# BradMcDanel/term-quantization

Measured on NVIDIA B200. Metric: resnet18_tq_g8_a12_images_per_sec, higher is better.
Workload: dtype int term codes (TR encode) -> exact int32 accumulators on tcgen05 (kind::f16 with statically proven fp32 K-chunk accumulators summed in int32, or kind::i8 planes with s32 accumulators)

## Files before the change

include/tq_b200.h:

```cpp
#ifndef TQ_B200_H
#define TQ_B200_H

#include <stdint.h>

#ifdef __cplusplus
extern "C" {
#endif

#define TQ_VERSION 201

#define TQ_OK               0
#define TQ_ERR_INVALID      1
#define TQ_ERR_UNSUPPORTED  2
#define TQ_ERR_CUDA         3

#define TQ_F32   0
#define TQ_F64   1
#define TQ_BF16  2
#define TQ_F16   3

#define TQ_I8    0
#define TQ_I16   1
#define TQ_I32   2
#define TQ_U8    3
#define TQ_F16C  4

#define TQ_ENC_HESE    0
#define TQ_ENC_BINARY  1
#define TQ_ENC_BOOTH   2

#define TQ_FLAG_RELU       1u
#define TQ_FLAG_RECIP_DIV  2u

#define TQ_FLAG_EXACT_DIV  4u

#define TQ_MAX_GROUP   32
#define TQ_MAX_BITS    16

int         tq_version(void);
const char *tq_last_error(void);
uint64_t    tq_launch_count(void);

int tq_tr_encode(const void *in, void *out, int dtype,
                 int64_t B, int64_t C, int64_t WH,
                 float sf, int bits, int g, int alpha,
                 int encoding, unsigned flags, void *stream);

int tq_tr_encode_codes(const void *in, void *codes, int dtype, int code_dtype,
                       int64_t B, int64_t C, int64_t WH,
                       float sf, int bits, int g, int alpha,
                       int encoding, unsigned flags, int *overflow, void *stream);

int tq_hist_accumulate(const void *x, int dtype, int64_t n,
                       float *hist, uint32_t *counts_scratch ,
                       int nbins, float lo, float hi, void *stream);

int tq_mse_profile(const float *hist, const float *x, int nbins,
                   const float *sfs, int nsf, int bits, int terms,
                   double *errs, int *argmin, void *stream);

int tq_hese_term_count(const void *w, int dtype, int64_t n, float sf, unsigned flags,
                       unsigned long long *count, void *stream);

int tq_conv2d_codes_f16(const void *act, const void *wgt, const float *bias, float *out,
                        int N, int H, int W, int C, int Cout, int R, int S, int stride, int pad,
                        float scale, int acc_groups, void *stream);

int tq_conv2d_codes_fused(const void *act, const void *wgt, float *out_f32, void *out_codes,
                          const float *bias, const float *bn_a, const float *bn_b, const float *residual,
                          int N, int H, int W, int C, int Cout, int R, int S, int stride, int pad,
                          float scale, int relu, float next_sf, int next_bits, int next_terms,
                          int acc_groups, void *stream);

int tq_conv2d_planes_i8(const void *act_planes, const void *wgt_planes, int planes_a, int planes_w,
                        float *out_f32, void *out_codes, const float *bias, const float *bn_a,
                        const float *bn_b, const float *residual, int N, int H, int W, int C, int Cout,
                        int R, int S, int stride, int pad, float scale, int relu, float next_sf,
                        int next_bits, int next_terms, int act_max, int wgt_max, void *stream);

int tq_codes_to_planes(const void *codes_f16, void *planes_s8, int64_t n, int planes, int *overflow, void *stream);

int tq_conv_weight_l1(const void *wgt_f16, int RS, int Cout, int C, long long *pos, long long *neg, void *stream);

int tq_bn_relu_maxpool_encode(const float *x, const float *bn_a, const float *bn_b, float *out,
                              void *out_codes, int N, int H, int W, int C, int relu,
                              float next_sf, int next_bits, int next_terms, void *stream);

int tq_stem_conv7x7s2(const float *x, void *x2_scratch, const void *w2, float *out,
                      int N, int H, int W, int Cout, void *stream);
int tq_stem_conv7x7s2_dt(const void *x, int x_dtype, void *x2_scratch, const void *w2, float *out,
                         int N, int H, int W, int Cout, void *stream);

int tq_stem_conv7x7s2_u8(const void *x_u8, const float *mean3, const float *std3, void *x2_scratch, const void *w2,
                         float *out, int N, int H, int W, int Cout, void *stream);
int tq_stem_conv7x7s2_pool(const void *x, int x_dtype, void *x2_scratch, const void *w2,
                           const float *bn_a, const float *bn_b, int relu, float *out, void *out_codes,
                           int N, int H, int W, int Cout, float next_sf, int next_bits, int next_terms,
                           void *stream);

int tq_depthwise3x3_codes(const void *act_codes, const int32_t *wgt_codes, float *out_f32, void *out_codes,
                          const float *bias, const float *bn_a, const float *bn_b, int N, int H, int W, int C,
                          int stride, float scale, int relu, int act_unsigned, float next_sf, int next_bits,
                          int next_terms, void *stream);

int tq_bn_act_encode(const float *x, const float *bias, const float *bn_a, const float *bn_b, float *out_f32,
                     void *out_codes, int64_t npix, int C, int relu, float next_sf, int next_bits, int next_terms,
                     void *stream);

int tq_first_conv3x3_fused(const float *x, const float *wgt, const float *bias, const float *bn_a, const float *bn_b,
                           float *out_f32, void *out_codes, int N, int H, int W, int Cout, int stride, int relu,
                           float next_sf, int next_bits, int next_terms, void *stream);

int tq_maxpool2d_f16(const void *x_f16, void *y_f16, int N, int H, int W, int C, int k, int stride, int pad,
                     void *stream);

int tq_u8_normalize_bf16(const void *x_u8, void *y_bf16, int64_t npix, const float *mean3, const float *std3,
                         void *stream);

int tq_selftest_division(uint64_t n, uint32_t seed, unsigned long long *mismatch, void *stream);

#ifdef __cplusplus
}
#endif
#endif
```

term_quantization_b200/_lib.py:

```python
import ctypes as C
import os

_HERE = os.path.dirname(os.path.abspath(__file__))
LIB_PATH = os.environ.get("TQ_B200_LIB") or os.path.join(_HERE, "libtq_b200.so")

TQ_OK, TQ_ERR_INVALID, TQ_ERR_UNSUPPORTED, TQ_ERR_CUDA = 0, 1, 2, 3
TQ_F32, TQ_F64, TQ_BF16, TQ_F16 = 0, 1, 2, 3
TQ_I8, TQ_I16, TQ_I32, TQ_U8, TQ_F16C = 0, 1, 2, 3, 4
ENC_HESE, ENC_BINARY, ENC_BOOTH = 0, 1, 2
FLAG_RELU, FLAG_RECIP_DIV, FLAG_EXACT_DIV = 1, 2, 4

_i64, _i, _f, _p, _u = C.c_int64, C.c_int, C.c_float, C.c_void_p, C.c_uint
SYMBOLS = {
    "tq_version": (_i, []),
    "tq_last_error": (C.c_char_p, []),
    "tq_launch_count": (C.c_uint64, []),
    "tq_tr_encode": (_i, [_p, _p, _i, _i64, _i64, _i64, _f, _i, _i, _i, _i, _u, _p]),
    "tq_tr_encode_codes": (_i, [_p, _p, _i, _i, _i64, _i64, _i64, _f, _i, _i, _i, _i, _u, _p, _p]),
    "tq_hist_accumulate": (_i, [_p, _i, _i64, _p, _p, _i, _f, _f, _p]),
    "tq_mse_profile": (_i, [_p, _p, _i, _p, _i, _i, _i, _p, _p, _p]),
    "tq_hese_term_count": (_i, [_p, _i, _i64, _f, _u, _p, _p]),
    "tq_conv2d_codes_f16": (_i, [_p, _p, _p, _p] + [_i] * 9 + [_f, _i, _p]),
    "tq_conv2d_codes_fused": (_i, [_p] * 8 + [_i] * 9 + [_f, _i, _f, _i, _i, _i, _p]),
    "tq_conv2d_planes_i8": (_i, [_p, _p, _i, _i] + [_p] * 6 + [_i] * 9 + [_f, _i, _f, _i, _i, _i, _i, _p]),
    "tq_codes_to_planes": (_i, [_p, _p, _i64, _i, _p, _p]),
    "tq_conv_weight_l1": (_i, [_p, _i, _i, _i, _p, _p, _p]),
    "tq_depthwise3x3_codes": (_i, [_p] * 7 + [_i] * 5 + [_f, _i, _i, _f, _i, _i, _p]),
    "tq_bn_act_encode": (_i, [_p] * 6 + [_i64, _i, _i, _f, _i, _i, _p]),
    "tq_maxpool2d_f16": (_i, [_p, _p, _i, _i, _i, _i, _i, _i, _i, _p]),
    "tq_first_conv3x3_fused": (_i, [_p] * 7 + [_i, _i, _i, _i, _i, _i, _f, _i, _i, _p]),
    "tq_u8_normalize_bf16": (_i, [_p, _p, _i64, _p, _p, _p]),
    "tq_bn_relu_maxpool_encode": (_i, [_p] * 5 + [_i] * 5 + [_f, _i, _i, _p]),
    "tq_stem_conv7x7s2": (_i, [_p, _p, _p, _p, _i, _i, _i, _i, _p]),
    "tq_stem_conv7x7s2_dt": (_i, [_p, _i, _p, _p, _p, _i, _i, _i, _i, _p]),
    "tq_stem_conv7x7s2_u8": (_i, [_p, _p, _p, _p, _p, _p, _i, _i, _i, _i, _p]),
    "tq_stem_conv7x7s2_pool": (_i, [_p, _i, _p, _p, _p, _p, _i, _p, _p, _i, _i, _i, _i, _f, _i, _i, _p]),
    "tq_selftest_division": (_i, [C.c_uint64, C.c_uint32, _p, _p]),
}

_lib = None


class TQError(RuntimeError):
    pass


def build(verbose=False):
    import subprocess
    subprocess.run(["make", "-C", os.path.join(_HERE, "csrc"), "-j4", "--no-print-directory"],
                   check=True, stdout=None if verbose else subprocess.DEVNULL)


def lib():
    global _lib
    if _lib is None:
        if not os.path.exists(LIB_PATH):
            raise TQError(
                f"{LIB_PATH} is missing: build it with `python -c 'import __graft_entry__ as g; "
                "g.build()'` or `make -C term_quantization_b200/csrc`. There is no CPU fallback.")
        L = C.CDLL(LIB_PATH)
        for name, (res, args) in SYMBOLS.items():
            fn = getattr(L, name)
            fn.restype = res
            fn.argtypes = args
        _lib = L
    return _lib


def check(rc):
    if rc != TQ_OK:
        msg = lib().tq_last_error().decode("utf-8", "replace")
        if rc == TQ_ERR_INVALID:
            raise ValueError(f"tq_b200: {msg}")
        if rc == TQ_ERR_UNSUPPORTED:
            raise NotImplementedError(f"tq_b200: {msg}")
        raise TQError(f"tq_b200: {msg}")


def launch_count():
    return int(lib().tq_launch_count())
```

term_quantization_b200/conv_codes.py:

```python
import torch

from . import _lib
from . import tr_cuda


def pack_conv_weight(w, w_sf, weight_bits, group_size, num_terms):
    codes = tr_cuda.tr_codes(w.detach().contiguous(), w_sf, weight_bits, group_size, num_terms,
                             dtype=torch.int16)
    O, I, kh, kw = codes.shape
    return codes.permute(2, 3, 0, 1).reshape(kh * kw, O, I).to(torch.float16).contiguous()



EXACT_LIMIT = 1 << 24


def _relu_code(relu):
    if relu in ("relu6", 2):
        return 2
    return 1 if relu else 0


class WeightPlan:

    def __init__(self, engine, groups, bound, act_max, signed, wgt, planes=None, planes_w=0, wgt_max=0):
        self.engine, self.groups, self.bound, self.act_max, self.signed = engine, groups, bound, act_max, signed
        self.wgt, self.planes, self.planes_w, self.wgt_max = wgt, planes, planes_w, wgt_max

    def __repr__(self):
        return (f"WeightPlan({self.engine}, groups={self.groups}, bound={self.bound:.3e}, act_max={self.act_max}, "
                f"signed={self.signed}, planes_w={self.planes_w})")


def weight_l1(wgt):
    RS, Cout, C = wgt.shape
    kcb = (C + 63) // 64
    pos = torch.empty((Cout, kcb), dtype=torch.int64, device=wgt.device)
    neg = torch.empty_like(pos)
    with torch.cuda.device(wgt.device):
        rc = _lib.lib().tq_conv_weight_l1(wgt.data_ptr(), RS, Cout, C, pos.data_ptr(), neg.data_ptr(),
                                          torch.cuda.current_stream(wgt.device).cuda_stream)
    _lib.check(rc)
    return pos, neg


def codes_to_planes(codes, planes):
    if codes.dtype != torch.float16 or not codes.is_contiguous() or not codes.is_cuda:
        raise RuntimeError("codes_to_planes expects a contiguous fp16 CUDA tensor")
    out = torch.empty((planes,) + tuple(codes.shape), dtype=torch.int8, device=codes.device)
    ovf = torch.zeros(1, dtype=torch.int32, device=codes.device)
    with torch.cuda.device(codes.device):
        rc = _lib.lib().tq_codes_to_planes(codes.data_ptr(), out.data_ptr(), codes.numel(), planes, ovf.data_ptr(),
                                           torch.cuda.current_stream(codes.device).cuda_stream)
    _lib.check(rc)
    return out, ovf


def _planes_needed(max_abs_code):
    if max_abs_code <= 127:
        return 1
    if max_abs_code <= 2047:
        return 2
    raise NotImplementedError(f"codes up to {max_abs_code} do not fit two signed 8-bit planes")


def plan_weight(wgt, act_max, signed_act=False, engine="auto"):
    if wgt.dtype != torch.float16 or wgt.dim() != 3 or not wgt.is_contiguous():
        raise RuntimeError("plan_weight expects a contiguous fp16 [R*S, Cout, C] code tensor")
    RS, Cout, C = wgt.shape
    bound = float("inf")
    if engine in ("auto", "f16"):
        pos, neg = weight_l1(wgt)
        kcb = pos.shape[1]
        block_n = 64 if Cout <= 64 else 128
        for groups in (1, 2, 4, 8):
            if kcb % groups or groups * block_n > (512 if block_n == 128 else 256):
                continue
            p = pos.view(Cout, groups, kcb // groups).sum(2)
            n = neg.view(Cout, groups, kcb // groups).sum(2)
            worst = (p + n) if signed_act else torch.maximum(p, n)
            b = float(act_max) * float(worst.max().item())
            bound = min(bound, b)
            if b < EXACT_LIMIT:
                return WeightPlan("f16", groups, b, act_max, signed_act, wgt)
        if engine == "f16":
            raise NotImplementedError(
                f"kind::f16 conv: cannot prove exact fp32 accumulation for this weight (best bound {bound:.3e} >= 2^24 "
                f"with act_max = {act_max}); use the kind::i8 plane engine (engine='i8' / 'auto')")
    if C % 16:
        raise NotImplementedError("kind::i8 plane engine needs C % 16 == 0")
    wmax = int(wgt.abs().max().item())
    pw = _planes_needed(wmax)
    planes, ovf = codes_to_planes(wgt, pw)
    if int(ovf.item()):
        raise RuntimeError("weight codes do not fit their planes")
    return WeightPlan("i8", 1, bound, act_max, signed_act, wgt, planes=planes, planes_w=pw, wgt_max=max(wmax, 1))


_PLANS = {}


def _cached_plan(wgt, act_max, signed_act, engine):
    key = (wgt.data_ptr(), wgt._version, tuple(wgt.shape), int(act_max), bool(signed_act), engine)
    plan = _PLANS.get(key)
    if plan is None or plan.wgt is not wgt:
        if len(_PLANS) > 256:
            _PLANS.clear()
        plan = _PLANS[key] = plan_weight(wgt, act_max, signed_act, engine)
    return plan


def _run_conv(act, plan, out, codes, bias, bn, residual, N, H, W, C, Cout, R, S, stride, pad, scale, relu, sf, bits,
              terms, act_planes=None):
    ptr = lambda t: t.data_ptr() if t is not None else None
    L = _lib.lib()
    stream = torch.cuda.current_stream(act.device).cuda_stream
    with torch.cuda.device(act.device):
        if plan.engine == "f16":
            rc = L.tq_conv2d_codes_fused(
                act.data_ptr(), plan.wgt.data_ptr(), ptr(out), ptr(codes), ptr(bias),
                ptr(bn[0]) if bn else None, ptr(bn[1]) if bn else None, ptr(residual),
                N, H, W, C, Cout, R, S, stride, pad, float(scale), _relu_code(relu), float(sf), int(bits),
                int(terms), int(plan.groups), stream)
        else:
            if act_planes is None:
                pa = _planes_needed(plan.act_max)
                act_planes, _ = codes_to_planes(act, pa)
            rc = L.tq_conv2d_planes_i8(
                act_planes.data_ptr(), plan.planes.data_ptr(), act_planes.shape[0], plan.planes_w, ptr(out), ptr(codes),
                ptr(bias), ptr(bn[0]) if bn else None, ptr(bn[1]) if bn else None, ptr(residual),
                N, H, W, C, Cout, R, S, stride, pad, float(scale), _relu_code(relu), float(sf), int(bits), int(terms),
                int(plan.act_max), int(plan.wgt_max), stream)
    _lib.check(rc)


def conv2d_codes(act, wgt, bias, kernel_size, stride, pad, scale, out=None, *, act_max=512, signed_act=False,
                 engine="auto", plan=None):
    if not (act.is_cuda and wgt.is_cuda and act.dtype == torch.float16 and wgt.dtype == torch.float16):
        raise RuntimeError("conv2d_codes expects fp16 CUDA code tensors")
    if not (act.is_contiguous() and wgt.is_contiguous()):
        raise RuntimeError("conv2d_codes expects contiguous NHWC activations and packed weights")
    N, H, W, C = act.shape
    R, S = kernel_size
    RS, Cout, C2 = wgt.shape
    if RS != R * S or C2 != C:
        raise RuntimeError("weight / activation shape mismatch")
    Ho = (H + 2 * pad - R) // stride + 1
    Wo = (W + 2 * pad - S) // stride + 1
    if out is None:
        out = torch.empty((N, Ho, Wo, Cout), dtype=torch.float32, device=act.device)
    if plan is None:
        plan = _cached_plan(wgt, act_max, signed_act, engine)
    _run_conv(act, plan, out, None, bias, None, None, N, H, W, C, Cout, R, S, stride, pad, scale, False, 1.0, 1, 0)
    return out


def conv2d_codes_fused(act, wgt, kernel_size, stride, pad, scale, *, bias=None, bn=None, residual=None,
                       relu=False, want_f32=True, next_quant=None, act_max=512, signed_act=False, engine="auto",
                       plan=None):
    N, H, W, C = act.shape
    R, S = kernel_size
    RS, Cout, C2 = wgt.shape
    if act.dtype != torch.float16 or wgt.dtype != torch.float16 or RS != R * S or C2 != C:
        raise RuntimeError("conv2d_codes_fused: bad operands")
    Ho = (H + 2 * pad - R) // stride + 1
    Wo = (W + 2 * pad - S) // stride + 1
    out = torch.empty((N, Ho, Wo, Cout), dtype=torch.float32, device=act.device) if want_f32 else None
    codes = torch.empty((N, Ho, Wo, Cout), dtype=torch.float16, device=act.device) if next_quant else None
    if residual is not None and (residual.shape != (N, Ho, Wo, Cout) or not residual.is_contiguous()
                                 or residual.dtype != torch.float32):
        raise RuntimeError("residual must be a contiguous fp32 [N, Ho, Wo, Cout] tensor")
    sf, bits, terms = next_quant if next_quant else (1.0, 1, 0)
    if plan is None:
        plan = _cached_plan(wgt, act_max, signed_act, engine)
    _run_conv(act, plan, out, codes, bias, bn, residual, N, H, W, C, Cout, R, S, stride, pad, scale, relu, sf, bits, terms)
    return out, codes


def pack_linear_weight(w, w_sf):
    sf32 = torch.tensor(w_sf, dtype=torch.float32).item()
    codes = torch.round(w.detach() / sf32)
    if not torch.equal(codes * sf32, w.detach()):
        raise RuntimeError("weight is not an integer multiple of w_sf any more")
    O, I = codes.shape
    Op, Ip = (O + 3) // 4 * 4, (I + 15) // 16 * 16
    packed = torch.zeros((1, Op, Ip), dtype=torch.float16, device=w.device)
    packed[0, :O, :I] = codes.to(torch.float16)
    return packed, sf32


def linear_codes(x_codes, wgt, scale, *, bias=None, out_features=None, plan=None, act_max=512, signed_act=True,
                 engine="auto"):
    if x_codes.dtype != torch.float16 or x_codes.dim() != 2:
        raise RuntimeError("linear_codes expects fp16 [M, K] codes")
    M, K = x_codes.shape
    _, Op, Kp = wgt.shape
    if K > Kp:
        raise RuntimeError("weight / activation shape mismatch")
    if K != Kp:
        xp = torch.zeros((M, Kp), dtype=torch.float16, device=x_codes.device)
        xp[:, :K] = x_codes
        x_codes = xp
    bias_p = bias
    if bias is not None and bias.numel() != Op:
        bias_p = torch.zeros(Op, dtype=torch.float32, device=wgt.device)
        bias_p[:bias.numel()] = bias.detach().float()
    out = conv2d_codes(x_codes.contiguous().view(1, 1, M, Kp), wgt, bias_p, (1, 1), 1, 0, scale, plan=plan, act_max=act_max,
                       signed_act=signed_act, engine=engine).view(M, Op)
    n = out_features if out_features is not None else Op
    return out if n == Op else out[:, :n]


def pack_depthwise_weight(w, w_sf):
    if w.dim() != 4 or w.shape[1] != 1 or tuple(w.shape[2:]) != (3, 3):
        raise NotImplementedError("depthwise packing expects a (C, 1, 3, 3) weight")
    sf32 = torch.tensor(w_sf, dtype=torch.float32).item()
    codes = torch.round(w.detach() / sf32)
    if not torch.equal(codes * sf32, w.detach()):
        raise RuntimeError("depthwise weight is not an integer multiple of w_sf any more")
    return codes.view(w.shape[0], 9).t().contiguous().to(torch.int32), sf32


def depthwise3x3_codes(act, wgt, stride, scale, *, bias=None, bn=None, relu=False, want_f32=False, next_quant=None,
                       act_unsigned=False):
    if act.dtype != torch.float16 or not act.is_contiguous() or wgt.dtype != torch.int32 or not wgt.is_contiguous():
        raise RuntimeError("depthwise3x3_codes expects contiguous fp16 NHWC codes and int32 [9, C] weights")
    N, H, W, C = act.shape
    if tuple(wgt.shape) != (9, C):
        raise RuntimeError("weight / activation shape mismatch")
    Ho, Wo = (H - 1) // stride + 1, (W - 1) // stride + 1
    out = torch.empty((N, Ho, Wo, C), dtype=torch.float32, device=act.device) if want_f32 else None
    codes = torch.empty((N, Ho, Wo, C), dtype=torch.float16, device=act.device) if next_quant else None
    sf, bits, terms = next_quant if next_quant else (1.0, 1, 0)
    ptr = lambda t: t.data_ptr() if t is not None else None
    with torch.cuda.device(act.device):
        rc = _lib.lib().tq_depthwise3x3_codes(
            act.data_ptr(), wgt.data_ptr(), ptr(out), ptr(codes), ptr(bias), ptr(bn[0]) if bn else None,
            ptr(bn[1]) if bn else None, N, H, W, C, stride, float(scale), _relu_code(relu), int(bool(act_unsigned)),
            float(sf), int(bits), int(terms), torch.cuda.current_stream(act.device).cuda_stream)
    _lib.check(rc)
    return out, codes


def pack_first_conv_weight(w_oihw):
    if w_oihw.dim() != 4 or w_oihw.shape[1:] != (3, 3, 3):
        raise RuntimeError("pack_first_conv_weight expects a (Cout, 3, 3, 3) weight")
    return w_oihw.detach().float().permute(2, 3, 1, 0).contiguous()


def first_conv3x3_fused(x_nhwc, w_packed, stride=1, bias=None, bn=None, relu=False, want_f32=False, next_quant=None):
    if x_nhwc.dtype != torch.float32 or not x_nhwc.is_contiguous() or not x_nhwc.is_cuda or x_nhwc.shape[-1] != 3:
        raise RuntimeError("first_conv3x3_fused expects a contiguous fp32 CUDA [N, H, W, 3] tensor")
    N, H, W, _ = x_nhwc.shape
    Cout = w_packed.shape[-1]
    Ho, Wo = (H - 1) // stride + 1, (W - 1) // stride + 1
    out = torch.empty((N, Ho, Wo, Cout), dtype=torch.float32, device=x_nhwc.device) if want_f32 else None
    codes = torch.empty((N, Ho, Wo, Cout), dtype=torch.float16, device=x_nhwc.device) if next_quant else None
    if out is None and codes is None:
        raise RuntimeError("first_conv3x3_fused: nothing to compute (want_f32 or next_quant)")
    sf, bits, terms = next_quant if next_quant else (1.0, 1, 0)
    ptr = lambda t: t.data_ptr() if t is not None else None
    for t in (bias, bn[0] if bn else None, bn[1] if bn else None):
        if t is not None and (t.dtype != torch.float32 or t.numel() != Cout or not t.is_contiguous() or t.device != x_nhwc.device):
            raise RuntimeError("first_conv3x3_fused: bias / bn must be contiguous fp32 [Cout] tensors on the input's device")
    with torch.cuda.device(x_nhwc.device):
        rc = _lib.lib().tq_first_conv3x3_fused(
            x_nhwc.data_ptr(), w_packed.data_ptr(), ptr(bias), ptr(bn[0]) if bn else None, ptr(bn[1]) if bn else None,
            ptr(out), ptr(codes), N, H, W, Cout, int(stride), _relu_code(relu), float(sf), int(bits), int(terms),
            torch.cuda.current_stream(x_nhwc.device).cuda_stream)
    _lib.check(rc)
    return out, codes


def maxpool_codes(codes_nhwc, kernel_size, stride=None, padding=0):
    k = kernel_size if isinstance(kernel_size, int) else kernel_size[0]
    st = k if stride is None else (stride if isinstance(stride, int) else stride[0])
    pd = padding if isinstance(padding, int) else padding[0]
    if codes_nhwc.dtype != torch.float16 or not codes_nhwc.is_contiguous() or not codes_nhwc.is_cuda:
        raise RuntimeError("maxpool_codes expects a contiguous fp16 CUDA [N, H, W, C] tensor")
    N, H, W, C = codes_nhwc.shape
    Ho, Wo = (H + 2 * pd - k) // st + 1, (W + 2 * pd - k) // st + 1
    out = torch.empty((N, Ho, Wo, C), dtype=torch.float16, device=codes_nhwc.device)
    with torch.cuda.device(codes_nhwc.device):
        rc = _lib.lib().tq_maxpool2d_f16(codes_nhwc.data_ptr(), out.data_ptr(), N, H, W, C, k, st, pd,
                                         torch.cuda.current_stream(codes_nhwc.device).cuda_stream)
    _lib.check(rc)
    return out


def bn_act_encode(x_nhwc, bn=None, relu=False, want_f32=False, next_quant=None, bias=None):
    if x_nhwc.dtype != torch.float32 or not x_nhwc.is_contiguous() or not x_nhwc.is_cuda:
        raise RuntimeError("bn_act_encode expects a contiguous fp32 CUDA tensor with channels last")
    C = x_nhwc.shape[-1]
    out = torch.empty_like(x_nhwc) if want_f32 else None
    codes = torch.empty(x_nhwc.shape, dtype=torch.float16, device=x_nhwc.device) if next_quant else None
    sf, bits, terms = next_quant if next_quant else (1.0, 1, 0)
    ptr = lambda t: t.data_ptr() if t is not None else None
    with torch.cuda.device(x_nhwc.device):
        if bias is not None and (bias.dtype != torch.float32 or bias.numel() != C or not bias.is_contiguous() or bias.device != x_nhwc.device):
            raise RuntimeError("bn_act_encode: bias must be a contiguous fp32 [C] tensor on the input's device")
        rc = _lib.lib().tq_bn_act_encode(
            x_nhwc.data_ptr(), ptr(bias), ptr(bn[0]) if bn else None, ptr(bn[1]) if bn else None, ptr(out), ptr(codes),
            x_nhwc.numel() // C, C, _relu_code(relu), float(sf), int(bits), int(terms),
            torch.cuda.current_stream(x_nhwc.device).cuda_stream)
    _lib.check(rc)
    return out, codes


def bn_relu_maxpool_encode(x_nhwc, bn, relu=True, next_quant=None):
    if x_nhwc.dtype != torch.float32 or not x_nhwc.is_contiguous() or not x_nhwc.is_cuda:
        raise RuntimeError("bn_relu_maxpool_encode expects a contiguous fp32 CUDA [N, H, W, C] tensor")
    N, H, W, C = x_nhwc.shape
    Ho, Wo = (H - 1) // 2 + 1, (W - 1) // 2 + 1
    out = torch.empty((N, Ho, Wo, C), dtype=torch.float32, device=x_nhwc.device)
    codes = torch.empty((N, Ho, Wo, C), dtype=torch.float16, device=x_nhwc.device) if next_quant else None
    sf, bits, terms = next_quant if next_quant else (1.0, 1, 0)
    with torch.cuda.device(x_nhwc.device):
        rc = _lib.lib().tq_bn_relu_maxpool_encode(
            x_nhwc.data_ptr(), bn[0].data_ptr(), bn[1].data_ptr(), out.data_ptr(),
            codes.data_ptr() if codes is not None else None, N, H, W, C, int(bool(relu)),
            float(sf), int(bits), int(terms), torch.cuda.current_stream(x_nhwc.device).cuda_stream)
    _lib.check(rc)
    return out, codes


def pack_stem_weight(w, channel_sign=None):
    Cout, Cin, kh, kw = w.shape
    if (Cin, kh, kw) != (3, 7, 7) or Cout > 64:
        raise NotImplementedError("stem conv packing expects a (Cout <= 64, 3, 7, 7) weight")
    w8 = torch.zeros(Cout, 4, 8, 8, dtype=torch.float32, device=w.device)
    w8[:, :3, :7, :7] = w.detach().float()
    if channel_sign is not None:
        w8 = w8 * channel_sign.view(-1, 1, 1, 1).to(w8)
    w2 = w8.view(Cout, 4, 4, 2, 4, 2).permute(2, 0, 4, 3, 5, 1).reshape(4, Cout, 64)
    hi = w2.half()
    lo = (w2 - hi.float()).half()
    out = torch.zeros(4, 128, 64, dtype=torch.float16, device=w.device)
    out[:, :Cout] = hi
    out[:, 64:64 + Cout] = lo
    return out.contiguous()


_STEM_DTYPES = {torch.float32: _lib.TQ_F32, torch.bfloat16: _lib.TQ_BF16, torch.float16: _lib.TQ_F16}


def stem_conv7x7s2(x_nhwc, w2, scratch=None, cout=None):
    if x_nhwc.dtype not in _STEM_DTYPES or not x_nhwc.is_contiguous() or x_nhwc.shape[-1] != 3:
        raise RuntimeError("stem_conv7x7s2 expects a contiguous fp32 / bf16 / fp16 [N, H, W, 3] tensor")
    N, H, W, _ = x_nhwc.shape
    Cout = cout if cout is not None else 64
    need = (2 if x_nhwc.dtype == torch.float32 else 1) * N * (H // 2 + 3) * (W // 2 + 3) * 16
    if scratch is None or scratch.numel() < need:
        scratch = torch.empty(need, dtype=torch.float16, device=x_nhwc.device)
    out = torch.empty((N, H // 2, W // 2, Cout), dtype=torch.float32, device=x_nhwc.device)
    with torch.cuda.device(x_nhwc.device):
        rc = _lib.lib().tq_stem_conv7x7s2_dt(x_nhwc.data_ptr(), _STEM_DTYPES[x_nhwc.dtype], scratch.data_ptr(),
                                             w2.data_ptr(), out.data_ptr(), N, H, W, Cout,
                                             torch.cuda.current_stream(x_nhwc.device).cuda_stream)
    _lib.check(rc)
    return out, scratch


def stem_conv7x7s2_u8(x_u8_nhwc, mean, std, w2, scratch=None, cout=None):
    import ctypes
    if x_u8_nhwc.dtype != torch.uint8 or not x_u8_nhwc.is_contiguous() or not x_u8_nhwc.is_cuda or x_u8_nhwc.shape[-1] != 3:
        raise RuntimeError("stem_conv7x7s2_u8 expects a contiguous uint8 CUDA [N, H, W, 3] tensor")
    N, H, W, _ = x_u8_nhwc.shape
    Cout = cout if cout is not None else 64
    need = N * (H // 2 + 3) * (W // 2 + 3) * 16
    if scratch is None or scratch.numel() < need:
        scratch = torch.empty(need, dtype=torch.float16, device=x_u8_nhwc.device)
    out = torch.empty((N, H // 2, W // 2, Cout), dtype=torch.float32, device=x_u8_nhwc.device)
    m = (ctypes.c_float * 3)(*mean)
    s = (ctypes.c_float * 3)(*std)
    with torch.cuda.device(x_u8_nhwc.device):
        rc = _lib.lib().tq_stem_conv7x7s2_u8(x_u8_nhwc.data_ptr(), ctypes.cast(m, ctypes.c_void_p), ctypes.cast(s, ctypes.c_void_p),
                                             scratch.data_ptr(), w2.data_ptr(), out.data_ptr(), N, H, W, Cout,
                                             torch.cuda.current_stream(x_u8_nhwc.device).cuda_stream)
    _lib.check(rc)
    return out, scratch


def stem_pool_operands(w, bn):
    a, b = bn
    sign = torch.where(a < 0, -torch.ones_like(a), torch.ones_like(a))
    return pack_stem_weight(w, sign), (a.abs().contiguous(), b.contiguous())


def stem_conv_pool(x_nhwc, w2, bn, relu=True, next_quant=None, scratch=None):
    if x_nhwc.dtype not in _STEM_DTYPES or not x_nhwc.is_contiguous() or x_nhwc.shape[-1] != 3:
        raise RuntimeError("stem_conv_pool expects a contiguous fp32 / bf16 / fp16 [N, H, W, 3] tensor")
    N, H, W, _ = x_nhwc.shape
    Cout = bn[0].numel()
    need = (2 if x_nhwc.dtype == torch.float32 else 1) * N * (H // 2 + 3) * (W // 2 + 3) * 16
    if scratch is None or scratch.numel() < need:
        scratch = torch.empty(need, dtype=torch.float16, device=x_nhwc.device)
    Hp, Wp = (H // 2 - 1) // 2 + 1, (W // 2 - 1) // 2 + 1
    out = torch.empty((N, Hp, Wp, Cout), dtype=torch.float32, device=x_nhwc.device)
    codes = torch.empty((N, Hp, Wp, Cout), dtype=torch.float16, device=x_nhwc.device) if next_quant else None
    sf, bits, terms = next_quant if next_quant else (1.0, 1, 0)
    with torch.cuda.device(x_nhwc.device):
        rc = _lib.lib().tq_stem_conv7x7s2_pool(
            x_nhwc.data_ptr(), _STEM_DTYPES[x_nhwc.dtype], scratch.data_ptr(), w2.data_ptr(),
            bn[0].data_ptr(), bn[1].data_ptr(), int(bool(relu)), out.data_ptr(),
            codes.data_ptr() if codes is not None else None, N, H, W, Cout, float(sf), int(bits), int(terms),
            torch.cuda.current_stream(x_nhwc.device).cuda_stream)
    _lib.check(rc)
    return out, codes, scratch
```

term_quantization_b200/csrc/tq_gemm.cu:

```cuda
#ifdef TQ_CONV_TRACE
#include <cstdio>
#endif
#include <cuda.h>

#include <cstdlib>
#include <cstring>
#include <mutex>
#include <type_traits>
#include <vector>

#include "tq_common.cuh"

namespace tq {

constexpr int GM_BLOCK_M = 128;
constexpr int GM_ROW_BYTES = 128;
constexpr int GM_BLOCK_K = 64;
constexpr int GM_THREADS = 640;
constexpr int GM_A_BYTES = GM_BLOCK_M * GM_ROW_BYTES;
constexpr int GM_I8_SHIFT = 4;

struct ConvGeom {
    int N, H, W, C, Cout, R, S, stride, pad, Ho, Wo;
    int wbox, hbox, nbox;
    int hw;
    int step_w, step_h, off_w, off_h;
    int pool, pool_p, pool_q;
    int halo, halo_baseoff;
    int img_h1;
    int pair;
    int tiles_w, tiles_h, tiles_n;
    int m_tiles, n_tiles, kc_blocks;
    int a_tx_bytes;
    float scale;
    int a_stages, a_stage_bytes;
    int stages, stage_bytes, ring_off, bstat_off, epi_off, epi_group_bytes, epi_codes_off, lut_off, bar_off, smem_total;
    int prog_steps, nb_tiles, n_groups;
    int kcpg, acc_int, planes_a, planes_w, kblk;
    int b_rows;
    int dbg_skip_epilogue;
    int dbg_skip_mma, dbg_skip_tma;
    uint32_t prog_mma[16];
    const float *bias, *bn_a, *bn_b, *residual;
    int relu, relu6, write_f32, write_codes;
    float next_sf;
    int next_bits, next_terms, next_fastdiv;
};

__device__ __forceinline__ uint32_t smem_u32(const void *p) { return (uint32_t)__cvta_generic_to_shared(p); }

__device__ __forceinline__ void mbar_init(uint64_t *bar, uint32_t count)
{
    asm volatile("mbarrier.init.shared::cta.b64 [%0], %1;" ::"r"(smem_u32(bar)), "r"(count));
}
__device__ __forceinline__ void mbar_expect_tx(uint64_t *bar, uint32_t bytes)
{
    asm volatile("mbarrier.arrive.expect_tx.shared::cta.b64 _, [%0], %1;" ::"r"(smem_u32(bar)), "r"(bytes) : "memory");
}
__device__ __forceinline__ void mbar_arrive(uint64_t *bar)
{
    asm volatile("mbarrier.arrive.shared::cta.b64 _, [%0];" ::"r"(smem_u32(bar)) : "memory");
}
__device__ __forceinline__ void mbar_wait(uint64_t *bar, uint32_t parity)
{
    asm volatile(
        "{\n\t"
        ".reg .pred P1;\n\t"
        "WAIT_LOOP:\n\t"
        "mbarrier.try_wait.parity.shared::cta.b64 P1, [%0], %1;\n\t"
        "@P1 bra DONE;\n\t"
        "bra WAIT_LOOP;\n\t"
        "DONE:\n\t"
        "}" ::"r"(smem_u32(bar)), "r"(parity) : "memory");
}
__device__ __forceinline__ void tma_load_4d(const CUtensorMap *map, uint64_t *bar, void *dst, int c0, int c1, int c2, int c3)
{
    asm volatile(
        "cp.async.bulk.tensor.4d.shared::cluster.global.mbarrier::complete_tx::bytes [%0], [%1, {%3, %4, %5, %6}], [%2];"
        ::"r"(smem_u32(dst)), "l"(map), "r"(smem_u32(bar)), "r"(c0), "r"(c1), "r"(c2), "r"(c3) : "memory");
}
__device__ __forceinline__ void tma_load_3d(const CUtensorMap *map, uint64_t *bar, void *dst, int c0, int c1, int c2)
{
    asm volatile(
        "cp.async.bulk.tensor.3d.shared::cluster.global.mbarrier::complete_tx::bytes [%0], [%1, {%3, %4, %5}], [%2];"
        ::"r"(smem_u32(dst)), "l"(map), "r"(smem_u32(bar)), "r"(c0), "r"(c1), "r"(c2) : "memory");
}
__device__ __forceinline__ bool elect_one()
{
    uint32_t pred = 0;
    asm volatile(
        "{\n\t"
        ".reg .pred P;\n\t"
        "elect.sync _|P, 0xFFFFFFFF;\n\t"
        "selp.u32 %0, 1, 0, P;\n\t"
        "}" : "=r"(pred));
    return pred != 0;
}
__device__ __forceinline__ void tc_fence_before() { asm volatile("tcgen05.fence::before_thread_sync;" ::: "memory"); }
__device__ __forceinline__ void tc_fence_after() { asm volatile("tcgen05.fence::after_thread_sync;" ::: "memory"); }
__device__ __forceinline__ void umma_f16(uint32_t tmem_d, uint64_t desc_a, uint64_t desc_b, uint32_t idesc, uint32_t accumulate)
{
    asm volatile(
        "{\n\t"
        ".reg .pred p;\n\t"
        "setp.ne.b32 p, %4, 0;\n\t"
        "tcgen05.mma.cta_group::1.kind::f16 [%0], %1, %2, %3, p;\n\t"
        "}" ::"r"(tmem_d), "l"(desc_a), "l"(desc_b), "r"(idesc), "r"(accumulate) : "memory");
}
__device__ __forceinline__ void umma_i8(uint32_t tmem_d, uint64_t desc_a, uint64_t desc_b, uint32_t idesc, uint32_t accumulate)
{
    asm volatile(
        "{\n\t"
        ".reg .pred p;\n\t"
        "setp.ne.b32 p, %4, 0;\n\t"
        "tcgen05.mma.cta_group::1.kind::i8 [%0], %1, %2, %3, p;\n\t"
        "}" ::"r"(tmem_d), "l"(desc_a), "l"(desc_b), "r"(idesc), "r"(accumulate) : "memory");
}
template <int KIND>
__device__ __forceinline__ void umma(uint32_t tmem_d, uint64_t desc_a, uint64_t desc_b, uint32_t idesc, uint32_t accumulate)
{
    if constexpr (KIND == 1) umma_i8(tmem_d, desc_a, desc_b, idesc, accumulate);
    else umma_f16(tmem_d, desc_a, desc_b, idesc, accumulate);
}
__device__ __forceinline__ uint32_t cluster_ctarank()
{
    uint32_t r;
    asm volatile("mov.u32 %0, %%cluster_ctarank;" : "=r"(r));
    return r;
}
__device__ __forceinline__ void cluster_sync_all()
{
    asm volatile("barrier.cluster.arrive.release.aligned;\n\tbarrier.cluster.wait.acquire.aligned;" ::: "memory");
}
__device__ __forceinline__ uint32_t mapa_u32(uint32_t addr, uint32_t rank)
{
    uint32_t r;
    asm volatile("mapa.shared::cluster.u32 %0, %1, %2;" : "=r"(r) : "r"(addr), "r"(rank));
    return r;
}
__device__ __forceinline__ void mbar_arrive_cluster(uint32_t cluster_addr)
{
    asm volatile("mbarrier.arrive.shared::cluster.b64 _, [%0];" ::"r"(cluster_addr) : "memory");
}
__device__ __forceinline__ void tma_load_4d_pair(const CUtensorMap *map, uint32_t bar_cluster, void *dst, int c0, int c1, int c2, int c3)
{
    asm volatile(
        "cp.async.bulk.tensor.4d.cta_group::2.shared::cluster.global.mbarrier::complete_tx::bytes [%0], [%1, {%3, %4, %5, %6}], [%2];"
        ::"r"(smem_u32(dst)), "l"(map), "r"(bar_cluster), "r"(c0), "r"(c1), "r"(c2), "r"(c3) : "memory");
}
__device__ __forceinline__ void tma_load_3d_pair(const CUtensorMap *map, uint32_t bar_cluster, void *dst, int c0, int c1, int c2)
{
    asm volatile(
        "cp.async.bulk.tensor.3d.cta_group::2.shared::cluster.global.mbarrier::complete_tx::bytes [%0], [%1, {%3, %4, %5}], [%2];"
        ::"r"(smem_u32(dst)), "l"(map), "r"(bar_cluster), "r"(c0), "r"(c1), "r"(c2) : "memory");
}
__device__ __forceinline__ void umma_f16_pair(uint32_t tmem_d, uint64_t desc_a, uint64_t desc_b, uint32_t idesc, uint32_t accumulate)
{
    asm volatile(
        "{\n\t"
        ".reg .pred p;\n\t"
        "setp.ne.b32 p, %4, 0;\n\t"
        "tcgen05.mma.cta_group::2.kind::f16 [%0], %1, %2, %3, p;\n\t"
        "}" ::"r"(tmem_d), "l"(desc_a), "l"(desc_b), "r"(idesc), "r"(accumulate) : "memory");
}
__device__ __forceinline__ void umma_commit_pair(uint64_t *bar)
{
    asm volatile("tcgen05.commit.cta_group::2.mbarrier::arrive::one.shared::cluster.multicast::cluster.b64 [%0], %1;"
                 ::"r"(smem_u32(bar)), "h"((uint16_t)3) : "memory");
}
__device__ __forceinline__ void umma_commit(uint64_t *bar)
{
    asm volatile("tcgen05.commit.cta_group::1.mbarrier::arrive::one.shared::cluster.b64 [%0];" ::"r"(smem_u32(bar)) : "memory");
}
#ifdef TQ_CONV_TRACE
#define TR_DECL(n) long long trc[n] = {}
#define TR(slot, ...) do { const long long _t = clock64(); __VA_ARGS__; trc[slot] += clock64() - _t; } while (0)
#define TR_T0(name) const long long name = clock64()
#define TR_SINCE(slot, name) trc[slot] += clock64() - name
#else
#define TR_DECL(n)
#define TR(slot, ...) do { __VA_ARGS__; } while (0)
#define TR_T0(name)
#define TR_SINCE(slot, name)
#endif

__device__ __forceinline__ void tmem_ld_32x32b_x32(uint32_t taddr, uint32_t (&r)[32])
{
    asm volatile(
        "tcgen05.ld.sync.aligned.32x32b.x32.b32 "
        "{%0, %1, %2, %3, %4, %5, %6, %7, %8, %9, %10, %11, %12, %13, %14, %15, "
        "%16, %17, %18, %19, %20, %21, %22, %23, %24, %25, %26, %27, %28, %29, %30, %31}, [%32];"
        : "=r"(r[0]), "=r"(r[1]), "=r"(r[2]), "=r"(r[3]), "=r"(r[4]), "=r"(r[5]), "=r"(r[6]), "=r"(r[7]),
          "=r"(r[8]), "=r"(r[9]), "=r"(r[10]), "=r"(r[11]), "=r"(r[12]), "=r"(r[13]), "=r"(r[14]), "=r"(r[15]),
          "=r"(r[16]), "=r"(r[17]), "=r"(r[18]), "=r"(r[19]), "=r"(r[20]), "=r"(r[21]), "=r"(r[22]), "=r"(r[23]),
          "=r"(r[24]), "=r"(r[25]), "=r"(r[26]), "=r"(r[27]), "=r"(r[28]), "=r"(r[29]), "=r"(r[30]), "=r"(r[31])
        : "r"(taddr));
    asm volatile("tcgen05.wait::ld.sync.aligned;" ::: "memory");
}

__device__ __forceinline__ void tmem_ld_32x32b_x16(uint32_t taddr, uint32_t (&r)[16])
{
    asm volatile(
        "tcgen05.ld.sync.aligned.32x32b.x16.b32 "
        "{%0, %1, %2, %3, %4, %5, %6, %7, %8, %9, %10, %11, %12, %13, %14, %15}, [%16];"
        : "=r"(r[0]), "=r"(r[1]), "=r"(r[2]), "=r"(r[3]), "=r"(r[4]), "=r"(r[5]), "=r"(r[6]), "=r"(r[7]),
          "=r"(r[8]), "=r"(r[9]), "=r"(r[10]), "=r"(r[11]), "=r"(r[12]), "=r"(r[13]), "=r"(r[14]), "=r"(r[15])
        : "r"(taddr));
    asm volatile("tcgen05.wait::ld.sync.aligned;" ::: "memory");
}

__device__ __forceinline__ void tma_store_4d(const CUtensorMap *map, const void *src, int c0, int c1, int c2, int c3)
{
    asm volatile("cp.async.bulk.tensor.4d.global.shared::cta.bulk_group [%0, {%2, %3, %4, %5}], [%1];"
                 ::"l"(map), "r"(smem_u32(src)), "r"(c0), "r"(c1), "r"(c2), "r"(c3) : "memory");
}
__device__ __forceinline__ void bulk_commit() { asm volatile("cp.async.bulk.commit_group;" ::: "memory"); }
__device__ __forceinline__ void bulk_wait_read0() { asm volatile("cp.async.bulk.wait_group.read 0;" ::: "memory"); }
__device__ __forceinline__ void bulk_wait0() { asm volatile("cp.async.bulk.wait_group 0;" ::: "memory"); }
__device__ __forceinline__ void fence_proxy_async() { asm volatile("fence.proxy.async.shared::cta;" ::: "memory"); }
__device__ __forceinline__ void epi_bar_sync(int id) { asm volatile("bar.sync %0, 128;" ::"r"(id) : "memory"); }
__device__ __forceinline__ void cp_async16(void *dst, const void *src)
{
    asm volatile("cp.async.ca.shared.global [%0], [%1], 16;" ::"r"(smem_u32(dst)), "l"(src) : "memory");
}
__device__ __forceinline__ void cp_async_wait_all() { asm volatile("cp.async.wait_all;" ::: "memory"); }

__device__ __forceinline__ uint64_t smem_desc_sw128(uint32_t saddr)
{
    return (uint64_t)((saddr & 0x3FFFFu) >> 4) | (1ull << 16) | ((uint64_t)(1024 >> 4) << 32) | (1ull << 46) | (2ull << 61);
}

constexpr int GM_LUT_MAX_BITS = 10;
constexpr int GM_MAX_STAGES = 8;
constexpr int GM_EPI_GROUPS = 4;
constexpr int GM_EPI_F32_BYTES = 16384;
constexpr int GM_EPI_CODE_BYTES = 8192;
constexpr int GM_SMEM_BUDGET = 227 * 1024;

template <bool FULL>
__device__ __forceinline__ void epi_affine(float (&t)[32], const ConvGeom &g, int c0)
{
    if (g.bias) {
        const float4 *bp = reinterpret_cast<const float4 *>(g.bias + c0);
#pragma unroll
        for (int j = 0; j < 32; j += 4) {
            if (FULL || c0 + j < g.Cout) {
                const float4 b = __ldg(bp + (j >> 2));
                t[j] = __fadd_rn(t[j], b.x); t[j + 1] = __fadd_rn(t[j + 1], b.y);
                t[j + 2] = __fadd_rn(t[j + 2], b.z); t[j + 3] = __fadd_rn(t[j + 3], b.w);
            }
        }
    }
    if (g.bn_a) {
        const float4 *ap = reinterpret_cast<const float4 *>(g.bn_a + c0);
        const float4 *bp = reinterpret_cast<const float4 *>(g.bn_b + c0);
#pragma unroll
        for (int j = 0; j < 32; j += 4) {
            if (FULL || c0 + j < g.Cout) {
                const float4 a = __ldg(ap + (j >> 2));
                const float4 b = __ldg(bp + (j >> 2));
                t[j] = __fmaf_rn(t[j], a.x, b.x); t[j + 1] = __fmaf_rn(t[j + 1], a.y, b.y);
                t[j + 2] = __fmaf_rn(t[j + 2], a.z, b.z); t[j + 3] = __fmaf_rn(t[j + 3], a.w, b.w);
            }
        }
    }
}

__device__ __forceinline__ uint32_t lds_u16(uint32_t saddr)
{
    uint16_t v;
    asm("ld.shared.u16 %0, [%1];" : "=h"(v) : "r"(saddr));
    return v;
}

template <bool RELU>
__device__ __forceinline__ void epi_stage(float (&t)[32], const ConvGeom &g, uint8_t *st_f32, uint8_t *st_codes, int row,
                                          bool has_res, const __half *lut, const Quant &nq)
{
    const uint32_t sw128 = (uint32_t)(row & 7);
    const uint32_t sw64 = (uint32_t)((row >> 1) & 3);
    uint8_t *frow = st_f32 + row * 128, *crow = st_codes + row * 64;
    if (has_res) {
#pragma unroll
        for (int j = 0; j < 32; j += 4) {
            const float4 r = *reinterpret_cast<const float4 *>(frow + (((uint32_t)(j >> 2) ^ sw128) << 4));
            t[j] = __fadd_rn(t[j], r.x); t[j + 1] = __fadd_rn(t[j + 1], r.y);
            t[j + 2] = __fadd_rn(t[j + 2], r.z); t[j + 3] = __fadd_rn(t[j + 3], r.w);
        }
    }
    if (RELU) {
#pragma unroll
        for (int j = 0; j < 32; ++j) t[j] = fmaxf(t[j], 0.0f);
        if (g.relu6) {
#pragma unroll
            for (int j = 0; j < 32; ++j) t[j] = fminf(t[j], 6.0f);
        }
    }
    if (g.write_f32) {
#pragma unroll
        for (int j = 0; j < 32; j += 4)
            *reinterpret_cast<float4 *>(frow + (((uint32_t)(j >> 2) ^ sw128) << 4)) = make_float4(t[j], t[j + 1], t[j + 2], t[j + 3]);
    }
    if (g.write_codes) {
        const uint32_t lut_s = smem_u32(lut) - 2u * 0x4B000000u;
        const uint32_t sign_off = 2u << g.next_bits;
#pragma unroll
        for (int j = 0; j < 32; j += 8) {
            uint32_t hc[8];
#pragma unroll
            for (int e = 0; e < 8; ++e) {
                const float x = t[j + e];
                float r;
                if (RELU) r = div_rn_nonneg<true>(x, nq);
                else r = div_rn_nonneg<true>(fmaxf(fabsf(x), 0.0f), nq);
                r = fminf(r, nq.maxv);
                float q = __fadd_rd(r, 0.5f);
                q = __fadd_rd(q, 8388608.0f);
                uint32_t addr = __float_as_uint(q) * 2u + lut_s;
                if (!RELU) addr += (__float_as_uint(x) >> 31) * sign_off;
                hc[e] = lds_u16(addr);
            }
            *reinterpret_cast<uint4 *>(crow + (((uint32_t)(j >> 3) ^ sw64) << 4)) =
                make_uint4(hc[0] | (hc[1] << 16), hc[2] | (hc[3] << 16), hc[4] | (hc[5] << 16), hc[6] | (hc[7] << 16));
        }
    }
}

template <int BLOCK_N, int MODE, bool RELU, int KIND, int CG = 1>
__global__ void __launch_bounds__(GM_THREADS, 1)
conv_igemm_kernel(const __grid_constant__ CUtensorMap tmA, const __grid_constant__ CUtensorMap tmB,
                      const __grid_constant__ CUtensorMap tmC, const __grid_constant__ CUtensorMap tmD,
                      const __grid_constant__ CUtensorMap tmR, const __grid_constant__ ConvGeom g)
{
    static_assert(KIND == 0 || MODE == 0, "the s8-plane engine streams both operands (MODE 0)");
    static_assert(CG == 1 || ((MODE == 4 || MODE == 3) && KIND == 0), "the CTA pair runs the halo modes");
    constexpr int MMA_N = MODE == 2 ? 2 * BLOCK_N : BLOCK_N;
    constexpr int B_BYTES = MMA_N * GM_ROW_BYTES;
    const int STAGES = g.stages;
    extern __shared__ uint8_t smem_raw[];
    uint8_t *smem = reinterpret_cast<uint8_t *>((reinterpret_cast<uintptr_t>(smem_raw) + 1023) & ~uintptr_t(1023));
    uint8_t *ring = smem + g.ring_off;
    uint8_t *bstat = smem + g.bstat_off;
    uint64_t *full_bar = reinterpret_cast<uint64_t *>(smem + g.bar_off);
    uint64_t *empty_bar = full_bar + GM_MAX_STAGES;
    uint64_t *tfull_bar = empty_bar + GM_MAX_STAGES;
    uint64_t *tempty_bar = tfull_bar + 3;
    uint64_t *bfull_bar = tempty_bar + 3;
    uint64_t *res_bar = bfull_bar + 1;
    uint64_t *afull_bar = res_bar + GM_EPI_GROUPS;
    uint64_t *aempty_bar = afull_bar + 4;
    uint32_t *tmem_slot = reinterpret_cast<uint32_t *>(aempty_bar + 4);
    constexpr bool prog = MODE >= 1 && MODE <= 3;
    const int acc_cols = g.n_groups * BLOCK_N;

    const int warp = threadIdx.x >> 5, lane = threadIdx.x & 31;
    const uint32_t cta_rank = CG == 2 ? cluster_ctarank() : 0u;
    const int tile_first = CG == 2 ? (int)(blockIdx.x >> 1) : (int)blockIdx.x;
    const int tile_step = CG == 2 ? (int)(gridDim.x >> 1) : (int)gridDim.x;
    const int total_tiles = CG == 2 ? ((g.m_tiles + 1) / 2) * g.n_tiles : g.m_tiles * g.n_tiles;
    auto m_tile_of = [&](int tile) { return CG == 2 ? 2 * (tile / g.n_tiles) + (int)cta_rank : tile / g.n_tiles; };
    const int kblocks = g.R * g.S * g.kc_blocks * (KIND == 1 ? g.planes_a * g.planes_w : 1);
    const int ACC_STAGES = 3 * acc_cols <= 512 ? 3 : (2 * acc_cols <= 512 ? 2 : 1);
    uint32_t TMEM_COLS = 32;
    while (TMEM_COLS < (uint32_t)(ACC_STAGES * acc_cols)) TMEM_COLS <<= 1;

    if (warp == 0 && lane == 0) {
        asm volatile("prefetch.tensormap [%0];" ::"l"(&tmA) : "memory");
        asm volatile("prefetch.tensormap [%0];" ::"l"(&tmB) : "memory");
        if (g.write_f32) asm volatile("prefetch.tensormap [%0];" ::"l"(&tmC) : "memory");
        if (g.write_codes) asm volatile("prefetch.tensormap [%0];" ::"l"(&tmD) : "memory");
        if (g.residual) asm volatile("prefetch.tensormap [%0];" ::"l"(&tmR) : "memory");
    }
    __half *lut = reinterpret_cast<__half *>(smem + g.lut_off);
    if (g.write_codes) {
        for (uint32_t i = threadIdx.x; i < (2u << g.next_bits); i += GM_THREADS) {
            int code = elem_code(i & ((1u << g.next_bits) - 1u), TQ_ENC_HESE, g.next_terms);
            lut[i] = __int2half_rn((i >> g.next_bits) ? -code : code);
        }
    }
    if (MODE == 4 && g.img_h1) {
        const int tail = g.a_stage_bytes - g.a_tx_bytes;
        for (int i = threadIdx.x * 16; i < g.a_stages * tail; i += GM_THREADS * 16)
            *reinterpret_cast<uint4 *>(bstat + (i / tail) * g.a_stage_bytes + g.a_tx_bytes + (i % tail)) = make_uint4(0u, 0u, 0u, 0u);
        fence_proxy_async();
    }
    if (warp == 1 && lane == 0) {
        for (int i = 0; i < STAGES; ++i) { mbar_init(&full_bar[i], 1); mbar_init(&empty_bar[i], 1); }
        mbar_init(bfull_bar, 1);
        for (int i = 0; i < 3; ++i) { mbar_init(&tfull_bar[i], 1); mbar_init(&tempty_bar[i], (ACC_STAGES == 1 ? 512 : 256) * CG); }
        for (int i = 0; i < GM_EPI_GROUPS; ++i) mbar_init(&res_bar[i], 1);
        for (int i = 0; i < 4; ++i) { mbar_init(&afull_bar[i], 1); mbar_init(&aempty_bar[i], 1); }
        asm volatile("fence.mbarrier_init.release.cluster;" ::: "memory");
    }
    if (warp == 2) {
        if constexpr (CG == 2) {
            asm volatile("tcgen05.alloc.cta_group::2.sync.aligned.shared::cta.b32 [%0], %1;" ::"r"(smem_u32(tmem_slot)), "r"(TMEM_COLS) : "memory");
            asm volatile("tcgen05.relinquish_alloc_permit.cta_group::2.sync.aligned;" ::: "memory");
        } else {
            asm volatile("tcgen05.alloc.cta_group::1.sync.aligned.shared::cta.b32 [%0], %1;" ::"r"(smem_u32(tmem_slot)), "r"(TMEM_COLS) : "memory");
            asm volatile("tcgen05.relinquish_alloc_permit.cta_group::1.sync.aligned;" ::: "memory");
        }
    }
    tc_fence_before();
    if constexpr (CG == 2) cluster_sync_all();
    else __syncthreads();
    tc_fence_after();
    const uint32_t tmem_base = *tmem_slot;

    if (warp == 0) {
        if (elect_one()) {
            int stage = 0;
            uint32_t phase = 0;
            uint8_t *sdst = ring;
            if constexpr (prog && CG == 2) {
                const uint32_t bfull0 = mapa_u32(smem_u32(bfull_bar), 0);
                if (cta_rank == 0) mbar_expect_tx(bfull_bar, (uint32_t)(g.nb_tiles * B_BYTES));
                for (int t = 0; t < g.nb_tiles; ++t)
                    tma_load_3d_pair(&tmB, bfull0, bstat + t * (B_BYTES / 2), 0, (int)cta_rank * (BLOCK_N / 2), t);
            } else if constexpr (prog) {
                mbar_expect_tx(bfull_bar, (uint32_t)(g.nb_tiles * B_BYTES));
                for (int t = 0; t < g.nb_tiles; ++t) tma_load_3d(&tmB, bfull_bar, bstat + t * B_BYTES, 0, 0, t);
            }
            if constexpr (MODE == 4 && CG == 2) {
                constexpr uint32_t B_HALF = (uint32_t)B_BYTES / 2;
                const int kcb = g.kc_blocks, taps = g.R * g.S, a_stages = g.a_stages;
                const uint32_t full0 = mapa_u32(smem_u32(full_bar), 0), afull0 = mapa_u32(smem_u32(afull_bar), 0);
                int as = 0, bs = 0;
                uint32_t aph = 0, bph = 0;
                TR_DECL(4);
                TR_T0(tp0);
                auto load_halo = [&](int tile, int kc) {
                    const int m_tile = m_tile_of(tile);
                    const int tw = m_tile % g.tiles_w, th = (m_tile / g.tiles_w) % g.tiles_h, tn = m_tile / (g.tiles_w * g.tiles_h);
                    TR(0, mbar_wait(&aempty_bar[as], aph ^ 1u));
                    if (cta_rank == 0) mbar_expect_tx(&afull_bar[as], 2u * (uint32_t)g.a_tx_bytes);
                    tma_load_4d_pair(&tmA, afull0 + 8u * (uint32_t)as, bstat + as * g.a_stage_bytes, kc * GM_BLOCK_K,
                                     tw * g.step_w - g.pad, th * g.step_h - g.pad, tn * g.nbox);
                    if (++as == a_stages) { as = 0; aph ^= 1u; }
                };
                const bool ahead = a_stages >= 3;
                if (ahead && tile_first < total_tiles) load_halo(tile_first, 0);
                for (int tile = tile_first; tile < total_tiles; tile += tile_step) {
                    const int n_tile = tile % g.n_tiles;
                    const int nb0 = n_tile * BLOCK_N + (int)cta_rank * (BLOCK_N / 2);
                    for (int kc = 0; kc < kcb; ++kc) {
                        if (!ahead) load_halo(tile, kc);
                        else if (kc + 1 < kcb) load_halo(tile, kc + 1);
                        else if (tile + tile_step < total_tiles) load_halo(tile + tile_step, 0);
                        for (int tap = 0; tap < taps; tap += 2) {
                            const int nt = taps - tap >= 2 ? 2 : 1;
                            TR(1, mbar_wait(&empty_bar[bs], bph ^ 1u));
                            if (cta_rank == 0) mbar_expect_tx(&full_bar[bs], 2u * (uint32_t)nt * B_HALF);
                            for (int j = 0; j < nt; ++j)
                                tma_load_3d_pair(&tmB, full0 + 8u * (uint32_t)bs, ring + bs * g.stage_bytes + j * (int)B_HALF,
                                                 kc * GM_BLOCK_K, nb0, tap + j);
                            if (++bs == STAGES) { bs = 0; bph ^= 1u; }
                        }
                    }
                }
#ifdef TQ_CONV_TRACE
                TR_SINCE(2, tp0);
                if (blockIdx.x == 0 || blockIdx.x == 101)
                    printf("cta %3d producer (pair): total %lld, wait halo-empty %lld, wait weight-empty %lld\n", blockIdx.x, trc[2], trc[0], trc[1]);
#endif
            } else if constexpr (MODE == 4) {
                const int kcb = g.kc_blocks, taps = g.R * g.S, a_stages = g.a_stages;
                int as = 0, bs = 0;
                uint32_t aph = 0, bph = 0;
                TR_DECL(4);
                TR_T0(tp0);
                for (int tile = tile_first; tile < total_tiles; tile += tile_step) {
                    const int n_tile = tile % g.n_tiles, m_tile = m_tile_of(tile);
                    const int tw = m_tile % g.tiles_w, th = (m_tile / g.tiles_w) % g.tiles_h, tn = m_tile / (g.tiles_w * g.tiles_h);
                    const int w_in0 = tw * g.step_w - g.pad, h_in0 = th * g.step_h - g.pad;
                    const int nb0 = n_tile * BLOCK_N;
                    for (int kc = 0; kc < kcb; ++kc) {
                        TR(0, mbar_wait(&aempty_bar[as], aph ^ 1u));
                        if (g.dbg_skip_tma == 4) {
                            mbar_arrive(&afull_bar[as]);
                        } else {
                        mbar_expect_tx(&afull_bar[as], (uint32_t)g.a_tx_bytes);
                        tma_load_4d(&tmA, &afull_bar[as], bstat + as * g.a_stage_bytes, kc * GM_BLOCK_K, w_in0, h_in0, tn * g.nbox);
                        }
                        if (++as == a_stages) { as = 0; aph ^= 1u; }
                        for (int tap = 0; tap < taps; ++tap) {
                            TR(1, mbar_wait(&empty_bar[bs], bph ^ 1u));
                            if (g.dbg_skip_tma == 2) {
                                mbar_arrive(&full_bar[bs]);
                            } else {
                            mbar_expect_tx(&full_bar[bs], (uint32_t)B_BYTES);
                            tma_load_3d(&tmB, &full_bar[bs], ring + bs * B_BYTES, kc * GM_BLOCK_K, nb0, tap);
                            }
                            if (++bs == STAGES) { bs = 0; bph ^= 1u; }
                        }
                    }
                }
#ifdef TQ_CONV_TRACE
                TR_SINCE(2, tp0);
                if (blockIdx.x == 0 || blockIdx.x == 100)
                    printf("cta %3d producer: total %lld, wait halo-empty %lld, wait weight-empty %lld\n", blockIdx.x, trc[2], trc[0], trc[1]);
#endif
            } else if constexpr (MODE == 3 && CG == 2) {
                const uint32_t full0 = mapa_u32(smem_u32(full_bar), 0);
                for (int tile = tile_first; tile < total_tiles; tile += tile_step) {
                    const int m_tile = m_tile_of(tile);
                    const int tw = m_tile % g.tiles_w, th = (m_tile / g.tiles_w) % g.tiles_h, tn = m_tile / (g.tiles_w * g.tiles_h);
                    mbar_wait(&empty_bar[stage], phase ^ 1u);
                    if (cta_rank == 0) mbar_expect_tx(&full_bar[stage], 2u * (uint32_t)g.a_tx_bytes);
                    tma_load_4d_pair(&tmA, full0 + 8u * (uint32_t)stage, sdst, 0, tw * g.step_w - g.pad, th * g.step_h - g.pad, tn * g.nbox);
                    sdst += g.stage_bytes;
                    if (++stage == STAGES) { stage = 0; phase ^= 1u; sdst = ring; }
                }
            } else {
            const int steps = MODE == 3 ? g.kc_blocks : (MODE == 2 ? g.prog_steps / g.R : (prog ? g.prog_steps : kblocks));
            const int S = MODE == 3 ? 1 : g.S, kc_blocks = g.kc_blocks, stage_bytes = g.stage_bytes;
            const uint32_t tx_bytes = (uint32_t)g.a_tx_bytes + (prog ? 0u : (uint32_t)B_BYTES);
            const bool skip_tma = g.dbg_skip_tma != 0;
            for (int tile = tile_first; tile < total_tiles; tile += tile_step) {
                const int n_tile = tile % g.n_tiles, m_tile = m_tile_of(tile);
                const int tw = m_tile % g.tiles_w, th = (m_tile / g.tiles_w) % g.tiles_h, tn = m_tile / (g.tiles_w * g.tiles_h);
                const int w_in0 = (tw * g.step_w + g.off_w) * g.stride - g.pad, h_in0 = (th * g.step_h + g.off_h) * g.stride - g.pad, n0 = tn * g.nbox;
                const int nb0 = n_tile * BLOCK_N;
                int r = 0, sx = 0, kc = 0;
                int pa = 0, pw = 0;
                const int kblk = g.kblk, taps_all = g.R * g.S;
                for (int st = 0; st < steps; ++st) {
                    int cc, cw, ch, cn, bt;
                    if constexpr (MODE == 2) {
                        cw = w_in0; ch = h_in0; cc = 0; cn = n0 + st * g.N;
                        bt = 0;
                    } else {
                        cw = w_in0 + sx; ch = h_in0 + r; cc = kc * kblk; cn = n0; bt = r * S + sx;
                        if constexpr (KIND == 1) { cn += pa * g.N; bt += pw * taps_all; }
                    }
                    mbar_wait(&empty_bar[stage], phase ^ 1u);
                    if (skip_tma) mbar_arrive(&full_bar[stage]);
                    else {
                        mbar_expect_tx(&full_bar[stage], tx_bytes);
                        tma_load_4d(&tmA, &full_bar[stage], sdst, cc, cw, ch, cn);
                        if constexpr (!prog) tma_load_3d(&tmB, &full_bar[stage], sdst + GM_A_BYTES, cc, nb0, bt);
                    }
                    sdst += stage_bytes;
                    if (++stage == STAGES) { stage = 0; phase ^= 1u; sdst = ring; }
                    if (++kc == kc_blocks) {
                        kc = 0;
                        if constexpr (KIND == 1) {
                            if (++pw == g.planes_w) { pw = 0; if (++pa == g.planes_a) { pa = 0; if (++sx == S) { sx = 0; ++r; } } }
                        } else {
                            if (++sx == S) { sx = 0; ++r; }
                        }
                    }
                }
            }
            }
        }
        __syncwarp();
    } else if (warp == 1) {
        constexpr uint32_t IDESC = (KIND == 1 ? ((2u << 4) | (1u << 7) | (1u << 10)) : (1u << 4)) |
                                   ((uint32_t)(MMA_N >> 3) << 17) | ((uint32_t)(GM_BLOCK_M >> 4) << 24);
        constexpr uint64_t DESC_HI = ((uint64_t)(1024 >> 4) << 32) | (1ull << 46) | (2ull << 61);
        if (elect_one() && cta_rank == 0) {
            int stage = 0;
            uint32_t phase = 0;
            int acc = 0;
            uint32_t acc_phase = 0;
            const uint32_t a_lo0 = ((smem_u32(ring) & 0x3FFFFu) >> 4) | (1u << 16);
            const uint32_t b_lo0 = ((smem_u32(bstat) & 0x3FFFFu) >> 4) | (1u << 16);
            const uint32_t a_step = (uint32_t)g.stage_bytes >> 4;
            uint32_t a_lo = a_lo0;
            const int steps = prog ? g.prog_steps : kblocks;
            const bool skip_mma = g.dbg_skip_mma != 0;
            uint32_t pw = MODE == 2 ? g.prog_mma[0] : 0u;
            int as4 = 0;
            uint32_t aph4 = 0;
            if constexpr (prog) {
                mbar_wait(bfull_bar, 0);
                tc_fence_after();
            }
            TR_DECL(6);
            TR_T0(ti0);
            for (int tile = tile_first; tile < total_tiles; tile += tile_step) {
                TR(0, mbar_wait(&tempty_bar[acc], acc_phase ^ 1u));
                tc_fence_after();
                const uint32_t tmem_d = tmem_base + (uint32_t)(acc * acc_cols);
                if constexpr (MODE == 4 && CG == 2) {
                    constexpr uint32_t IDESC2 = (1u << 4) | ((uint32_t)(MMA_N >> 3) << 17) | ((uint32_t)(256 >> 4) << 24);
                    constexpr uint32_t B_HALF16 = (uint32_t)(B_BYTES / 2) >> 4;
                    const int taps = g.R * g.S, S = g.S, kcb = g.kc_blocks;
                    const uint32_t row_step = (uint32_t)g.hw * 8u;
                    int kin = 0;
                    uint32_t td = tmem_d;
                    for (int kc = 0; kc < kcb; ++kc) {
                        TR(1, mbar_wait(&afull_bar[as4], aph4));
                        tc_fence_after();
                        uint32_t a_row = b_lo0 + (uint32_t)as4 * ((uint32_t)g.a_stage_bytes >> 4);
                        int sx = 0;
                        for (int tap = 0; tap < taps; tap += 2) {
                            const int nt = taps - tap >= 2 ? 2 : 1;
                            TR(2, mbar_wait(&full_bar[stage], phase));
                            tc_fence_after();
                            for (int j = 0; j < nt; ++j) {
                                const uint64_t da = DESC_HI | (a_row + (uint32_t)sx * 8u);
                                const uint64_t db = DESC_HI | (a_lo + (uint32_t)j * B_HALF16);
#pragma unroll
                                for (int k = 0; k < GM_ROW_BYTES / 32; ++k)
                                    umma_f16_pair(td, da + (uint64_t)(2 * k), db + (uint64_t)(2 * k), IDESC2, (kin | (tap + j) | k) != 0 ? 1u : 0u);
                                if (++sx == S) { sx = 0; a_row += row_step; }
                            }
                            umma_commit_pair(&empty_bar[stage]);
                            a_lo += a_step;
                            if (++stage == STAGES) { stage = 0; phase ^= 1u; a_lo = a_lo0; }
                        }
                        umma_commit_pair(&aempty_bar[as4]);
                        if (++as4 == g.a_stages) { as4 = 0; aph4 ^= 1u; }
                        if (++kin == g.kcpg) { kin = 0; td += BLOCK_N; }
                    }
                } else if constexpr (MODE == 4) {
                    const int taps = g.R * g.S, S = g.S, kcb = g.kc_blocks;
                    const uint32_t row_step = (uint32_t)g.hw * 8u;
                    int kin = 0;
                    uint32_t td = tmem_d;
                    for (int kc = 0; kc < kcb; ++kc) {
                        TR(1, mbar_wait(&afull_bar[as4], aph4));
                        tc_fence_after();
                        uint32_t a_row = b_lo0 + (uint32_t)as4 * ((uint32_t)g.a_stage_bytes >> 4);
                        int sx = 0;
                        for (int tap = 0; tap < taps; ++tap) {
                            TR(2, mbar_wait(&full_bar[stage], phase));
                            tc_fence_after();
                            const uint64_t da = DESC_HI | (a_row + (uint32_t)sx * 8u);
                            const uint64_t db = DESC_HI | a_lo;
                            if (!skip_mma) {
#pragma unroll
                                for (int k = 0; k < GM_ROW_BYTES / 32; ++k)
                                    umma<KIND>(td, da + (uint64_t)(2 * k), db + (uint64_t)(2 * k), IDESC, (kin | tap | k) != 0 ? 1u : 0u);
                            }
                            umma_commit(&empty_bar[stage]);
                            a_lo += a_step;
                            if (++stage == STAGES) { stage = 0; phase ^= 1u; a_lo = a_lo0; }
                            if (++sx == S) { sx = 0; a_row += row_step; }
                        }
                        umma_commit(&aempty_bar[as4]);
                        if (++as4 == g.a_stages) { as4 = 0; aph4 ^= 1u; }
                        if (++kin == g.kcpg) { kin = 0; td += BLOCK_N; }
                    }
                } else if constexpr (MODE == 3 && CG == 2) {
                    constexpr uint32_t IDESC2 = (1u << 4) | ((uint32_t)(MMA_N >> 3) << 17) | ((uint32_t)(256 >> 4) << 24);
                    const int taps = g.R * g.S, S = g.S;
                    const uint32_t row_step = (uint32_t)g.hw * 8u;
                    TR(2, mbar_wait(&full_bar[stage], phase));
                    tc_fence_after();
                    uint32_t a_row = a_lo, b_lo = b_lo0;
                    int s = 0;
                    for (int tap = 0; tap < taps; ++tap) {
                        const uint64_t da = DESC_HI | (a_row + (uint32_t)s * 8u);
                        const uint64_t db = DESC_HI | b_lo;
#pragma unroll
                        for (int k = 0; k < GM_ROW_BYTES / 32; ++k)
                            umma_f16_pair(tmem_d, da + (uint64_t)(2 * k), db + (uint64_t)(2 * k), IDESC2, (tap | k) != 0 ? 1u : 0u);
                        b_lo += (uint32_t)(B_BYTES / 2) >> 4;
                        if (++s == S) { s = 0; a_row += row_step; }
                    }
                    umma_commit_pair(&empty_bar[stage]);
                    a_lo += a_step;
                    if (++stage == STAGES) { stage = 0; phase ^= 1u; a_lo = a_lo0; }
                } else if constexpr (MODE == 3) {
                    const int taps = g.R * g.S, S = g.S, kcb = g.kc_blocks;
                    const uint32_t row_step = (uint32_t)g.hw * 8u;
                    for (int kc = 0; kc < kcb; ++kc) {
                        TR(2, mbar_wait(&full_bar[stage], phase));
                        tc_fence_after();
                        uint32_t a_row = a_lo, b_lo = b_lo0 + (uint32_t)kc * (uint32_t)(B_BYTES >> 4);
                        int s = 0;
                        for (int tap = 0; tap < taps; ++tap) {
                            const uint32_t a_tap = a_row + (uint32_t)s * 8u;
                            uint64_t da = DESC_HI | a_tap;
                            if (g.halo_baseoff) da |= (uint64_t)((a_tap >> 3) & 7u) << 49;
                            const uint64_t db = DESC_HI | b_lo;
                            if (!skip_mma) {
#pragma unroll
                                for (int k = 0; k < GM_ROW_BYTES / 32; ++k)
                                    umma<KIND>(tmem_d, da + (uint64_t)(2 * k), db + (uint64_t)(2 * k), IDESC, (kc | tap | k) != 0 ? 1u : 0u);
                            }
                            b_lo += (uint32_t)kcb * (uint32_t)(B_BYTES >> 4);
                            if (++s == S) { s = 0; a_row += row_step; }
                        }
                        umma_commit(&empty_bar[stage]);
                        a_lo += a_step;
                        if (++stage == STAGES) { stage = 0; phase ^= 1u; a_lo = a_lo0; }
                    }
                } else if constexpr (MODE != 2) {
                    uint32_t b_lo = b_lo0;
                    int kc = 0, kin = 0, tap0 = 1, pa = 0, pw = 0;
                    uint32_t grp = 0;
                    for (int st = 0; st < steps; ++st) {
                        TR(2, mbar_wait(&full_bar[stage], phase));
                        tc_fence_after();
                        const uint64_t da = DESC_HI | a_lo;
                        const uint64_t db = DESC_HI | (MODE == 1 ? b_lo : a_lo + (uint32_t)(GM_A_BYTES >> 4));
                        uint32_t fresh;
                        if constexpr (KIND == 1) {
                            grp = (uint32_t)(pa + pw);
                            fresh = (tap0 && kc == 0 && (pa == 0 || pw == g.planes_w - 1)) ? 1u : 0u;
                        } else {
                            fresh = (tap0 && kin == 0) ? 1u : 0u;
                        }
                        const uint32_t td = tmem_d + grp * BLOCK_N;
                        if (!skip_mma) {
#pragma unroll
                            for (int k = 0; k < GM_ROW_BYTES / 32; ++k)
                                umma<KIND>(td, da + (uint64_t)(2 * k), db + (uint64_t)(2 * k), IDESC, (k != 0 || !fresh) ? 1u : 0u);
                        }
                        umma_commit(&empty_bar[stage]);
                        a_lo += a_step;
                        b_lo += (uint32_t)(B_BYTES >> 4);
                        if (++stage == STAGES) { stage = 0; phase ^= 1u; a_lo = a_lo0; }
                        if constexpr (KIND == 1) {
                            if (++kc == g.kc_blocks) {
                                kc = 0;
                                if (++pw == g.planes_w) { pw = 0; if (++pa == g.planes_a) { pa = 0; tap0 = 0; } }
                            }
                        } else {
                            ++kin; ++kc;
                            if (kin == g.kcpg) { kin = 0; ++grp; }
                            if (kc == g.kc_blocks) { kc = 0; kin = 0; grp = 0; tap0 = 0; }
                        }
                    }
                } else {
                    uint32_t started = 0;
                    const int R = g.R, planes = steps / R;
                    const uint32_t row_step = (uint32_t)g.hw * 8u;
                    int st = 0;
                    for (int pl = 0; pl < planes; ++pl) {
                        TR(2, mbar_wait(&full_bar[stage], phase));
                        tc_fence_after();
                        uint32_t a_row = a_lo;
                        for (int r = 0; r < R; ++r, ++st, a_row += row_step) {
                            const uint32_t cur = pw;
                            pw = g.prog_mma[st + 1 < steps ? st + 1 : 0];
                            const uint64_t da = DESC_HI | a_row;
                            const uint32_t g0 = (cur >> 8) & 0xFu;
                            const uint64_t db = DESC_HI | (b_lo0 + ((cur >> 4) & 0xFu) * (uint32_t)(B_BYTES >> 4));
                            const uint32_t first = ((started >> g0) & 1u) ^ 1u;
                            started |= 1u << g0;
                            if (!skip_mma) {
#pragma unroll
                                for (int k = 0; k < GM_BLOCK_K / 16; ++k)
                                    umma_f16(tmem_d + g0 * BLOCK_N, da + (uint64_t)(2 * k), db + (uint64_t)(2 * k), IDESC,
                                             (k != 0 || !first) ? 1u : 0u);
                            }
                            if ((cur & 0xFu) == 2u) {
                                const uint32_t g1 = (cur >> 16) & 0xFu;
                                const uint64_t db1 = DESC_HI | (b_lo0 + ((cur >> 12) & 0xFu) * (uint32_t)(B_BYTES >> 4));
                                const uint32_t first1 = ((started >> g1) & 1u) ^ 1u;
                                started |= 1u << g1;
                                if (!skip_mma) {
#pragma unroll
                                    for (int k = 0; k < GM_BLOCK_K / 16; ++k)
                                        umma_f16(tmem_d + g1 * BLOCK_N, da + (uint64_t)(2 * k), db1 + (uint64_t)(2 * k), IDESC,
                                                 (k != 0 || !first1) ? 1u : 0u);
                                }
                            }
                        }
                        umma_commit(&empty_bar[stage]);
                        a_lo += a_step;
                        if (++stage == STAGES) { stage = 0; phase ^= 1u; a_lo = a_lo0; }
                    }
                }
                if constexpr (CG == 2) umma_commit_pair(&tfull_bar[acc]);
                else umma_commit(&tfull_bar[acc]);
                if (++acc == ACC_STAGES) { acc = 0; acc_phase ^= 1u; }
            }
#ifdef TQ_CONV_TRACE
            TR_SINCE(3, ti0);
            if (blockIdx.x == 0 || blockIdx.x == 100)
                printf("cta %3d issuer: total %lld, wait acc-empty %lld, wait halo-full %lld, wait stage-full %lld\n", blockIdx.x, trc[3], trc[0], trc[1], trc[2]);
#endif
        }
        __syncwarp();
    } else if (warp >= 4) {
        const int grp = (warp - 4) >> 2;
        const int pair = grp >> 1, half = grp & 1;
        const int ew = warp & 3;
        const int mrow = ew * 32 + lane;
        const int my = mrow / g.hw, mx = mrow % g.hw;
        const int row = g.img_h1 ? (my / g.img_h1) * (g.wbox * g.hbox) + (my % g.img_h1) * g.wbox + mx : my * g.wbox + mx;
        const bool row_live = g.img_h1 ? (mx < g.wbox && (my % g.img_h1) < g.hbox && (my / g.img_h1) < g.nbox) : (mx < g.wbox && row < 128);
        const bool store_thread = (ew == 0 && lane == 0);
        uint8_t *st_f32 = smem + g.epi_off + grp * g.epi_group_bytes;
        uint8_t *st_codes = st_f32 + g.epi_codes_off;
        const Quant nq = make_quant(g.write_codes ? g.next_sf : 1.0f, (float)((1u << g.next_bits) - 1u));
        const bool has_res = g.residual != nullptr;
        const bool single = ACC_STAGES == 1;
        const int CHUNKS = single ? BLOCK_N / 128 : BLOCK_N / 64;
        const uint32_t res_bytes = (uint32_t)(g.wbox * g.hbox * g.nbox) * 128u;
        uint32_t res_phase = 0;
        int it = 0;
        const uint32_t tempty0 = CG == 2 ? mapa_u32(smem_u32(tempty_bar), 0) : 0u;
        auto release_acc = [&](int a) {
            if (CG == 2 && cta_rank != 0) mbar_arrive_cluster(tempty0 + 8u * (uint32_t)a);
            else mbar_arrive(&tempty_bar[a]);
        };
        TR_DECL(8);
        TR_T0(te0);
        const int n_tiles = g.n_tiles, tiles_w = g.tiles_w, tiles_h = g.tiles_h;
        int n_tile = tile_first % n_tiles;
        int tw, th, tn;
        {
            const int m0 = m_tile_of(tile_first);
            tw = m0 % tiles_w; th = (m0 / tiles_w) % tiles_h; tn = m0 / (tiles_w * tiles_h);
        }
        const int step_n = tile_step % n_tiles, step_m = (tile_step / n_tiles) * CG;
        const int s_w = step_m % tiles_w, s_h = (step_m / tiles_w) % tiles_h, s_n = step_m / (tiles_w * tiles_h);
        const int u_w = CG % tiles_w, u_h = (CG / tiles_w) % tiles_h, u_n = CG / (tiles_w * tiles_h);
        auto add_m = [&](int dw, int dh, int dn) {
            tw += dw;
            int c = tw >= tiles_w ? 1 : 0;
            tw -= c ? tiles_w : 0;
            th += dh + c;
            c = th >= tiles_h ? 1 : 0;
            th -= c ? tiles_h : 0;
            tn += dn + c;
        };
        int acc = 0;
        uint32_t acc_phase = 0;
        auto next_tile = [&]() {
            n_tile += step_n;
            const bool carry = n_tile >= n_tiles;
            n_tile -= carry ? n_tiles : 0;
            add_m(s_w, s_h, s_n);
            if (carry) add_m(u_w, u_h, u_n);
            if (++acc == ACC_STAGES) { acc = 0; acc_phase ^= 1u; }
        };
        for (int tile = tile_first; tile < total_tiles; tile += tile_step, ++it, next_tile()) {
            if (!single && (it & 1) != pair) continue;
            const int w0 = tw * g.wbox, h0 = th * g.hbox, n0 = tn * g.nbox;

            if (g.dbg_skip_epilogue) {
                mbar_wait(&tfull_bar[acc], acc_phase);
                tc_fence_after();
                tc_fence_before();
                release_acc(acc);
                continue;
            }
#pragma unroll 1
            for (int cc = 0; cc < CHUNKS; ++cc) {
                const int col0 = (single ? grp * (BLOCK_N / 4) : half * (BLOCK_N / 2)) + cc * 32;
                const int c0 = n_tile * BLOCK_N + col0;
                const bool chunk_live = c0 < g.Cout;
                if (has_res && store_thread && chunk_live) {
                    bulk_wait_read0();
                    mbar_expect_tx(&res_bar[grp], res_bytes);
                    tma_load_4d(&tmR, &res_bar[grp], st_f32, c0, w0, h0, n0);
                }
                if (cc == 0) {
                    TR(0, mbar_wait(&tfull_bar[acc], acc_phase));
                    tc_fence_after();
                }
                if (!chunk_live) {
                    if (cc == CHUNKS - 1) {
                        tc_fence_before();
                        release_acc(acc);
                    }
                    continue;
                }
                float t[32];
                TR_T0(tl0);
#pragma unroll
                for (int hh = 0; hh < 2; ++hh) {
                    uint32_t v[16];
                    const uint32_t tcol = tmem_base + ((uint32_t)(ew * 32) << 16) + (uint32_t)(acc * acc_cols + col0 + hh * 16);
                    tmem_ld_32x32b_x16(tcol, v);
                    const bool as_int = KIND == 1 || g.acc_int != 0;
                    if (g.n_groups > 1) {
                        if (KIND == 0 && as_int) {
#pragma unroll
                            for (int e = 0; e < 16; ++e) v[e] = (uint32_t)__float2int_rn(__uint_as_float(v[e]));
                        }
                        for (int gi = 1; gi < g.n_groups; ++gi) {
                            uint32_t u[16];
                            tmem_ld_32x32b_x16(tcol + (uint32_t)(gi * BLOCK_N), u);
#pragma unroll
                            for (int e = 0; e < 16; ++e) {
                                if (KIND == 1) v[e] = (v[e] << GM_I8_SHIFT) + u[e];
                                else if (as_int) v[e] += (uint32_t)__float2int_rn(__uint_as_float(u[e]));
                                else v[e] = __float_as_uint(__fadd_rn(__uint_as_float(v[e]), __uint_as_float(u[e])));
                            }
                        }
                    }
                    if (KIND == 1 || (as_int && g.n_groups > 1)) {
#pragma unroll
                        for (int e = 0; e < 16; ++e) v[e] = __float_as_uint(__int2float_rn((int)v[e]));
                    }
#pragma unroll
                    for (int e = 0; e < 16; ++e) t[hh * 16 + e] = __fmul_rn(__uint_as_float(v[e]), g.scale);
                }
                if (cc == CHUNKS - 1) {
                    tc_fence_before();
                    release_acc(acc);
                }
                TR_SINCE(1, tl0);
                TR_T0(tq0);
                if constexpr (MODE == 2) {
                    if (g.pool) {
                        {
                            uint8_t *frow = st_f32 + mrow * 128;
                            const uint32_t sw = (uint32_t)(mrow & 7);
#pragma unroll
                            for (int j = 0; j < 32; j += 4)
                                *reinterpret_cast<float4 *>(frow + (((uint32_t)(j >> 2) ^ sw) << 4)) =
                                    make_float4(t[j], t[j + 1], t[j + 2], t[j + 3]);
                        }
                        epi_bar_sync(1 + grp);
                        TR_SINCE(2, tq0);
                        TR_T0(tq1);
                        uint8_t *st_pool = st_codes, *st_pcodes = st_codes + 4096;
                        const int pp = mrow >> 2, cb = mrow & 3;
                        float pv[8];
                        const bool pool_thread = pp < g.pool_p * g.pool_q;
                        if (pool_thread) {
                            const int pl = pp / g.pool_q, ql = pp % g.pool_q;
                            const int oh0 = 2 * (th * g.pool_p + pl) - 1, ow0 = 2 * (tw * g.pool_q + ql) - 1;
                            int rowoff[3], coloff[3];
#pragma unroll
                            for (int d = 0; d < 3; ++d) {
                                rowoff[d] = (2 * pl + (((unsigned)(oh0 + d) < (unsigned)g.Ho) ? d : 1)) * g.hw;
                                coloff[d] = 2 * ql + (((unsigned)(ow0 + d) < (unsigned)g.Wo) ? d : 1);
                            }
                            float4 m0 = make_float4(-INFINITY, -INFINITY, -INFINITY, -INFINITY), m1 = m0;
#pragma unroll
                            for (int dy = 0; dy < 3; ++dy)
#pragma unroll
                                for (int dx = 0; dx < 3; ++dx) {
                                    const int mm = rowoff[dy] + coloff[dx];
                                    const uint32_t sw = (uint32_t)(mm & 7);
                                    const float4 a = *reinterpret_cast<const float4 *>(st_f32 + mm * 128 + (((uint32_t)(2 * cb) ^ sw) << 4));
                                    const float4 b = *reinterpret_cast<const float4 *>(st_f32 + mm * 128 + (((uint32_t)(2 * cb + 1) ^ sw) << 4));
                                    m0.x = fmaxf(m0.x, a.x); m0.y = fmaxf(m0.y, a.y); m0.z = fmaxf(m0.z, a.z); m0.w = fmaxf(m0.w, a.w);
                                    m1.x = fmaxf(m1.x, b.x); m1.y = fmaxf(m1.y, b.y); m1.z = fmaxf(m1.z, b.z); m1.w = fmaxf(m1.w, b.w);
                                }
                            pv[0] = m0.x; pv[1] = m0.y; pv[2] = m0.z; pv[3] = m0.w; pv[4] = m1.x; pv[5] = m1.y; pv[6] = m1.z; pv[7] = m1.w;
                            const int c8 = c0 + 8 * cb;
                            if (c8 < g.Cout) {
                                const float4 a0 = __ldg(reinterpret_cast<const float4 *>(g.bn_a + c8));
                                const float4 a1 = __ldg(reinterpret_cast<const float4 *>(g.bn_a + c8 + 4));
                                const float4 b0 = __ldg(reinterpret_cast<const float4 *>(g.bn_b + c8));
                                const float4 b1 = __ldg(reinterpret_cast<const float4 *>(g.bn_b + c8 + 4));
                                const float av[8] = {a0.x, a0.y, a0.z, a0.w, a1.x, a1.y, a1.z, a1.w};
                                const float bv[8] = {b0.x, b0.y, b0.z, b0.w, b1.x, b1.y, b1.z, b1.w};
#pragma unroll
                                for (int e = 0; e < 8; ++e) {
                                    pv[e] = __fmaf_rn(pv[e], av[e], bv[e]);
                                    if (RELU) pv[e] = fmaxf(pv[e], 0.0f);
                                }
                            }
                        }
                        TR_SINCE(3, tq1);
                        TR_T0(tq2);
                        if (store_thread) bulk_wait_read0();
                        epi_bar_sync(1 + grp);
                        TR_SINCE(4, tq2);
                        TR_T0(tq3);
                        if (pool_thread) {
                            const uint32_t psw = (uint32_t)(pp & 7);
                            *reinterpret_cast<float4 *>(st_pool + pp * 128 + (((uint32_t)(2 * cb) ^ psw) << 4)) = make_float4(pv[0], pv[1], pv[2], pv[3]);
                            *reinterpret_cast<float4 *>(st_pool + pp * 128 + (((uint32_t)(2 * cb + 1) ^ psw) << 4)) = make_float4(pv[4], pv[5], pv[6], pv[7]);
                            if (g.write_codes) {
                                uint32_t hc[8];
#pragma unroll
                                for (int e = 0; e < 8; ++e) {
                                    uint32_t idx;
                                    if (RELU) idx = g.next_fastdiv ? quantize_f32_nonneg<true>(pv[e], nq) : quantize_f32_nonneg<false>(pv[e], nq);
                                    else idx = (g.next_fastdiv ? quantize_f32<true>(pv[e], nq) : quantize_f32<false>(pv[e], nq)) |
                                               ((__float_as_uint(pv[e]) >> 31) << g.next_bits);
                                    hc[e] = __half_as_ushort(lut[idx]);
                                }
                                *reinterpret_cast<uint4 *>(st_pcodes + pp * 64 + (((uint32_t)cb ^ (uint32_t)((pp >> 1) & 3)) << 4)) =
                                    make_uint4(hc[0] | (hc[1] << 16), hc[2] | (hc[3] << 16), hc[4] | (hc[5] << 16), hc[6] | (hc[7] << 16));
                            }
                        }
                        TR_SINCE(5, tq3);
                        fence_proxy_async();
                        epi_bar_sync(1 + grp);
                        if (store_thread) {
                            tma_store_4d(&tmC, st_pool, c0, tw * g.pool_q, th * g.pool_p, n0);
                            if (g.write_codes) tma_store_4d(&tmD, st_pcodes, c0, tw * g.pool_q, th * g.pool_p, n0);
                            bulk_commit();
                        }
                        TR_SINCE(6, tq0);
                        continue;
                    }
                }
                TR(2, if (c0 + 32 <= g.Cout) epi_affine<true>(t, g, c0); else epi_affine<false>(t, g, c0));
                TR_T0(tw0);
                if (has_res) {
                    mbar_wait(&res_bar[grp], res_phase);
                } else {
                    if (store_thread) bulk_wait_read0();
                    epi_bar_sync(1 + grp);
                }
                TR_SINCE(3, tw0);
                TR(4, if (row_live) epi_stage<RELU>(t, g, st_f32, st_codes, row, has_res, lut, nq));
                if (has_res) res_phase ^= 1u;
                TR_T0(ts0);
                fence_proxy_async();
                epi_bar_sync(1 + grp);
                if (store_thread) {
                    if (g.write_f32) tma_store_4d(&tmC, st_f32, c0, w0, h0, n0);
                    if (g.write_codes) tma_store_4d(&tmD, st_codes, c0, w0, h0, n0);
                    bulk_commit();
                }
                TR_SINCE(5, ts0);
            }
        }
#ifdef TQ_CONV_TRACE
        TR_SINCE(7, te0);
        if ((blockIdx.x == 0 || blockIdx.x == 100) && store_thread && grp < 2)
            printf("cta %3d epilogue group %d: total %lld, wait acc-full %lld, tmem+combine %lld, affine %lld, wait staging %lld, stage %lld, "
                   "sync+store %lld, pooled tail %lld  (pooled stem: the four middle slots are raw staging + sync, window max + affine, store wait + sync, "
                   "pooled tile + encode)\n", blockIdx.x, grp, trc[7], trc[0], trc[1], trc[2], trc[3], trc[4], trc[5], trc[6]);
#endif
        if (store_thread) bulk_wait0();
    }

    tc_fence_before();
    if constexpr (CG == 2) cluster_sync_all();
    else __syncthreads();
    if (warp == 2) {
        if constexpr (CG == 2) asm volatile("tcgen05.dealloc.cta_group::2.sync.aligned.b32 %0, %1;" ::"r"(tmem_base), "r"(TMEM_COLS) : "memory");
        else asm volatile("tcgen05.dealloc.cta_group::1.sync.aligned.b32 %0, %1;" ::"r"(tmem_base), "r"(TMEM_COLS) : "memory");
    }
}

typedef CUresult (*EncodeTiledFn)(CUtensorMap *, CUtensorMapDataType, cuuint32_t, void *, const cuuint64_t *,
                                  const cuuint64_t *, const cuuint32_t *, const cuuint32_t *, CUtensorMapInterleave,
                                  CUtensorMapSwizzle, CUtensorMapL2promotion, CUtensorMapFloatOOBfill);

EncodeTiledFn encode_tiled()
{
    static EncodeTiledFn fn = nullptr;
    static std::once_flag once;
    std::call_once(once, [] {
        void *p = nullptr;
        cudaDriverEntryPointQueryResult q;
        if (cudaGetDriverEntryPoint("cuTensorMapEncodeTiled", &p, cudaEnableDefault, &q) == cudaSuccess &&
            q == cudaDriverEntryPointSuccess)
            fn = (EncodeTiledFn)p;
    });
    return fn;
}

static void pick_box(ConvGeom &g)
{
    long best = -1;
    static const int force_w = getenv("TQ_CONV_WBOX") ? atoi(getenv("TQ_CONV_WBOX")) : 0;
    static const int force_h = getenv("TQ_CONV_HBOX") ? atoi(getenv("TQ_CONV_HBOX")) : 0;
    for (int wb = 1; wb <= g.Wo && wb <= 128; ++wb) {
        if (wb * g.stride > 256) break;
        if (force_w && wb != force_w && force_w <= g.Wo) continue;
        for (int hb = 1; hb <= g.Ho && wb * hb <= 128; ++hb) {
            if (hb * g.stride > 256) break;
            if (force_h && hb != force_h && force_h <= g.Ho && force_w * force_h <= 128) continue;
            int nb = 1;
            if (wb == g.Wo && hb == g.Ho) nb = 128 / (wb * hb) < g.N ? 128 / (wb * hb) : g.N;
            if (nb < 1) nb = 1;
            const long tiles = (long)((g.Wo + wb - 1) / wb) * ((g.Ho + hb - 1) / hb) * ((g.N + nb - 1) / nb);
            if (best < 0 || tiles < best || (tiles == best && wb > g.wbox)) {
                best = tiles;
                g.wbox = wb; g.hbox = hb; g.nbox = nb;
            }
        }
    }
    g.tiles_w = (g.Wo + g.wbox - 1) / g.wbox;
    g.tiles_h = (g.Ho + g.hbox - 1) / g.hbox;
    g.tiles_n = (g.N + g.nbox - 1) / g.nbox;
    g.m_tiles = g.tiles_w * g.tiles_h * g.tiles_n;
    g.a_tx_bytes = g.wbox * g.hbox * g.nbox * GM_ROW_BYTES;
}

static bool pick_box_halo(ConvGeom &g)
{
    long best = -1, best_halo = 0;
    int bw = 0, bh = 0;
    for (int wb = 1; wb <= g.Wo; ++wb) {
        const int hw = wb + g.S - 1;
        if (hw > 128 || hw > 256) break;
        int hb = 128 / hw;
        if (hb > g.Ho) hb = g.Ho;
        if (hb < 1 || hb + g.R - 1 > 256) continue;
        const long tiles = (long)((g.Wo + wb - 1) / wb) * ((g.Ho + hb - 1) / hb) * g.N;
        const long halo = (long)hw * (hb + g.R - 1);
        if (best < 0 || tiles < best || (tiles == best && halo < best_halo)) { best = tiles; best_halo = halo; bw = wb; bh = hb; }
    }
    if (best < 0) return false;
    g.wbox = bw; g.hbox = bh; g.nbox = 1;
    g.hw = bw + g.S - 1;
    g.tiles_w = (g.Wo + bw - 1) / bw;
    g.tiles_h = (g.Ho + bh - 1) / bh;
    g.tiles_n = g.N;
    g.m_tiles = g.tiles_w * g.tiles_h * g.tiles_n;
    g.a_tx_bytes = g.hw * (bh + g.R - 1) * GM_ROW_BYTES;
    return true;
}

static int plan_smem(ConvGeom &g, int block_n)
{
    const int b_bytes = (g.b_rows > 0 ? g.b_rows : block_n) * GM_ROW_BYTES;
    const bool prog = g.prog_steps > 0;
    g.stage_bytes = GM_A_BYTES + (prog ? 0 : b_bytes);
    if (g.halo) g.stage_bytes = (g.a_tx_bytes + 1023) & ~1023;
    g.bstat_off = 0;
    g.ring_off = prog ? g.nb_tiles * (g.pair ? b_bytes / 2 : b_bytes) : 0;
    if (g.halo && !prog) {
        g.a_stage_bytes = (g.a_tx_bytes + 1023) & ~1023;
        if (g.img_h1) g.a_stage_bytes = (g.a_tx_bytes + ((g.R - 1) * g.hw + g.S) * GM_ROW_BYTES + 1023) & ~1023;
        static const int a_stages_env = getenv("TQ_CONV_ASTAGES") ? atoi(getenv("TQ_CONV_ASTAGES")) : 0;
        g.a_stages = a_stages_env >= 2 && a_stages_env <= 4 ? a_stages_env : (g.pair ? 3 : 2);
        g.stage_bytes = b_bytes;
        g.ring_off = g.a_stages * g.a_stage_bytes;
    }
    g.epi_codes_off = (g.write_f32 || g.residual) ? GM_EPI_F32_BYTES : 0;
    g.epi_group_bytes = g.epi_codes_off + ((g.write_codes || g.pool) ? GM_EPI_CODE_BYTES : 0);
    const int epi_bytes = GM_EPI_GROUPS * g.epi_group_bytes;
    const int fixed = g.ring_off + epi_bytes + (2 << GM_LUT_MAX_BITS) * 2 + 1024  + 1024 ;
    int stages = (GM_SMEM_BUDGET - fixed) / g.stage_bytes;
    if (stages > GM_MAX_STAGES) stages = GM_MAX_STAGES;
    static const int cap = getenv("TQ_CONV_STAGES") ? atoi(getenv("TQ_CONV_STAGES")) : GM_MAX_STAGES;
    if (stages > cap && cap >= 2) stages = cap;
    if (stages < 2) return fail(TQ_ERR_UNSUPPORTED, "shared memory budget: %d resident weight tiles do not fit", g.nb_tiles);
    g.stages = stages;
    g.epi_off = g.ring_off + stages * g.stage_bytes;
    g.lut_off = g.epi_off + epi_bytes;
    g.bar_off = g.lut_off + (2 << GM_LUT_MAX_BITS) * 2;
    g.smem_total = g.bar_off + 1024 + 1024;
    return TQ_OK;
}

template <int BLOCK_N, int MODE, int KIND = 0, int CG = 1>
static int launch_conv_mode(const CUtensorMap &tmA, const CUtensorMap &tmB, const CUtensorMap &tmC,
                            const CUtensorMap &tmD, const CUtensorMap &tmR, ConvGeom &g, cudaStream_t s)
{
    static const bool skip_epi = getenv("TQ_CONV_SKIP_EPI") != nullptr;
    g.dbg_skip_epilogue = skip_epi ? 1 : 0;
    static const bool skip_mma = getenv("TQ_CONV_SKIP_MMA") != nullptr;
    static const int skip_tma = getenv("TQ_CONV_SKIP_TMA") ? atoi(getenv("TQ_CONV_SKIP_TMA")) : 0;
    g.dbg_skip_mma = skip_mma ? 1 : 0;
    g.dbg_skip_tma = skip_tma;
    auto kern = g.relu ? conv_igemm_kernel<BLOCK_N, MODE, true, KIND, CG> : conv_igemm_kernel<BLOCK_N, MODE, false, KIND, CG>;
    static bool attr_set[2][64] = {{false}};
    int dev = 0;
    cudaGetDevice(&dev);
    if (dev >= 0 && dev < 64 && !attr_set[g.relu ? 1 : 0][dev]) {
        if (cudaFuncSetAttribute(kern, cudaFuncAttributeMaxDynamicSharedMemorySize, GM_SMEM_BUDGET) != cudaSuccess)
            return check_launch("cudaFuncSetAttribute(conv_igemm_kernel)");
        attr_set[g.relu ? 1 : 0][dev] = true;
    }
    if constexpr (CG == 2) {
        const int supers = ((g.m_tiles + 1) / 2) * g.n_tiles;
        cudaLaunchConfig_t cfg = {};
        cudaLaunchAttribute attr[1];
        attr[0].id = cudaLaunchAttributeClusterDimension;
        attr[0].val.clusterDim.x = 2; attr[0].val.clusterDim.y = 1; attr[0].val.clusterDim.z = 1;
        cfg.blockDim = dim3(GM_THREADS); cfg.dynamicSmemBytes = (size_t)g.smem_total; cfg.stream = s;
        cfg.attrs = attr; cfg.numAttrs = 1;
        static int max_pairs[2][64] = {{0}};
        int &mp = max_pairs[g.relu ? 1 : 0][dev >= 0 && dev < 64 ? dev : 0];
        if (mp == 0) {
            cfg.gridDim = dim3((unsigned)(num_sms() & ~1));
            int n = 0;
            if (cudaOccupancyMaxActiveClusters(&n, kern, &cfg) != cudaSuccess || n < 1) { (void)cudaGetLastError(); n = num_sms() / 2; }
            mp = n < num_sms() / 2 ? n : num_sms() / 2;
        }
        const int pairs = supers < mp ? supers : mp;
        cfg.gridDim = dim3((unsigned)(2 * pairs));
        cudaError_t e = cudaLaunchKernelEx(&cfg, kern, tmA, tmB, tmC, tmD, tmR, g);
        count_launch();
        if (e != cudaSuccess) return fail(TQ_ERR_CUDA, "conv_igemm_kernel (CTA pairs): %s", cudaGetErrorString(e));
        return check_launch("conv_igemm_kernel");
    } else {
        const int total = g.m_tiles * g.n_tiles;
        const int grid = total < num_sms() ? total : num_sms();
        kern<<<grid, GM_THREADS, g.smem_total, s>>>(tmA, tmB, tmC, tmD, tmR, g);
        count_launch();
        return check_launch("conv_igemm_kernel");
    }
}

enum ConvVariant { CV_NONE = 0, CV_64_M0, CV_64_M1, CV_64_M2, CV_64_M3, CV_64_M3_PAIR, CV_128_M0, CV_128_M4, CV_128_M4_PAIR, CV_256_M0, CV_I8_64, CV_I8_128 };

static int pick_variant(ConvGeom &g, int block_n, int kind, bool general_prog, ConvVariant &v)
{
    if (g.n_groups < 1) g.n_groups = 1;
    if (g.n_groups * block_n > 512) return fail(TQ_ERR_UNSUPPORTED, "accumulator groups exceed tensor memory");
    if (g.kcpg < 1) g.kcpg = g.kc_blocks;
    int rc = plan_smem(g, block_n);
    if (rc != TQ_OK) return rc;
    if (kind == 1) {
        if (g.prog_steps != 0 || g.halo || block_n == 256) return fail(TQ_ERR_UNSUPPORTED, "s8-plane engine: streaming mode only");
        v = block_n == 64 ? CV_I8_64 : CV_I8_128;
        return TQ_OK;
    }
    if (g.prog_steps == 0 && g.halo) {
        if (block_n != 128) return fail(TQ_ERR_UNSUPPORTED, "streamed-weight halo mode is built for BLOCK_N = 128 only");
        v = g.pair ? CV_128_M4_PAIR : CV_128_M4;
        return TQ_OK;
    }
    if (g.prog_steps == 0) { v = block_n == 64 ? CV_64_M0 : (block_n == 128 ? CV_128_M0 : CV_256_M0); return TQ_OK; }
    if (block_n != 64) return fail(TQ_ERR_UNSUPPORTED, "resident-weight mode is built for BLOCK_N = 64 only");
    v = general_prog ? CV_64_M2 : (g.halo ? (g.pair ? CV_64_M3_PAIR : CV_64_M3) : CV_64_M1);
    return TQ_OK;
}

static int launch_variant(ConvVariant v, const CUtensorMap &tmA, const CUtensorMap &tmB, const CUtensorMap &tmC,
                          const CUtensorMap &tmD, const CUtensorMap &tmR, ConvGeom &g, cudaStream_t s)
{
    switch (v) {
    case CV_64_M0: return launch_conv_mode<64, 0>(tmA, tmB, tmC, tmD, tmR, g, s);
    case CV_64_M1: return launch_conv_mode<64, 1>(tmA, tmB, tmC, tmD, tmR, g, s);
    case CV_64_M2: return launch_conv_mode<64, 2>(tmA, tmB, tmC, tmD, tmR, g, s);
    case CV_64_M3: return launch_conv_mode<64, 3>(tmA, tmB, tmC, tmD, tmR, g, s);
    case CV_64_M3_PAIR: return launch_conv_mode<64, 3, 0, 2>(tmA, tmB, tmC, tmD, tmR, g, s);
    case CV_128_M0: return launch_conv_mode<128, 0>(tmA, tmB, tmC, tmD, tmR, g, s);
    case CV_128_M4: return launch_conv_mode<128, 4>(tmA, tmB, tmC, tmD, tmR, g, s);
    case CV_128_M4_PAIR: return launch_conv_mode<128, 4, 0, 2>(tmA, tmB, tmC, tmD, tmR, g, s);
    case CV_256_M0: return launch_conv_mode<256, 0>(tmA, tmB, tmC, tmD, tmR, g, s);
    case CV_I8_64: return launch_conv_mode<64, 0, 1>(tmA, tmB, tmC, tmD, tmR, g, s);
    case CV_I8_128: return launch_conv_mode<128, 0, 1>(tmA, tmB, tmC, tmD, tmR, g, s);
    default: return fail(TQ_ERR_UNSUPPORTED, "no kernel variant");
    }
}

struct ConvArgs {
    const void *act, *wgt, *out_f32, *out_codes, *bias, *bn_a, *bn_b, *residual;
    int kind, N, H, W, C, Cout, R, S, stride, pad, relu, next_bits, next_terms, acc_groups, planes_a, planes_w, device;
    float scale, next_sf;
};
struct ConvPlan {
    ConvArgs key;
    ConvGeom g;
    CUtensorMap tmA, tmB, tmC, tmD, tmR;
    ConvVariant variant;
};
static std::mutex g_plan_mu;
static std::vector<ConvPlan> g_plans[64];
static size_t g_plan_count = 0;

static uint64_t hash_args(const ConvArgs &a)
{
    const unsigned char *p = reinterpret_cast<const unsigned char *>(&a);
    uint64_t h = 1469598103934665603ull;
    for (size_t i = 0; i < sizeof(ConvArgs); ++i) { h ^= p[i]; h *= 1099511628211ull; }
    return h;
}

static int encode_map(EncodeTiledFn enc, CUtensorMap *tm, CUtensorMapDataType dt, int esize, const void *base,
                      int rank, const cuuint64_t *dims, const cuuint32_t *box, const cuuint32_t *estr, const char *what,
                      CUtensorMapSwizzle swz = CU_TENSOR_MAP_SWIZZLE_128B)
{
    cuuint64_t strides[4];
    cuuint64_t acc = (cuuint64_t)esize;
    for (int i = 0; i < rank - 1; ++i) { acc *= dims[i]; strides[i] = acc; }
    CUresult r = enc(tm, dt, (cuuint32_t)rank, const_cast<void *>(base), dims, strides, box, estr,
                     CU_TENSOR_MAP_INTERLEAVE_NONE, swz, CU_TENSOR_MAP_L2_PROMOTION_L2_256B,
                     CU_TENSOR_MAP_FLOAT_OOB_FILL_NONE);
    if (r != CUDA_SUCCESS) return fail(TQ_ERR_CUDA, "cuTensorMapEncodeTiled(%s) failed: %d", what, (int)r);
    return TQ_OK;
}

static int plan_conv(const ConvArgs &a, ConvPlan &pl)
{
    const int N = a.N, H = a.H, W = a.W, C = a.C, Cout = a.Cout, R = a.R, S = a.S, stride = a.stride, pad = a.pad;
    const int kind = a.kind;
    EncodeTiledFn enc = encode_tiled();
    if (!enc) return fail(TQ_ERR_CUDA, "cuTensorMapEncodeTiled is not available from this driver");

    ConvGeom g{};
    g.N = N; g.H = H; g.W = W; g.C = C; g.Cout = Cout; g.R = R; g.S = S; g.stride = stride; g.pad = pad;
    g.Ho = (H + 2 * pad - R) / stride + 1;
    g.Wo = (W + 2 * pad - S) / stride + 1;
    if (g.Ho < 1 || g.Wo < 1) return fail(TQ_ERR_INVALID, "empty output");
    g.scale = a.scale;
    g.kblk = kind == 1 ? GM_ROW_BYTES : GM_BLOCK_K;
    g.kc_blocks = (C + g.kblk - 1) / g.kblk;
    g.planes_a = kind == 1 ? a.planes_a : 1;
    g.planes_w = kind == 1 ? a.planes_w : 1;
    pick_box(g);
    g.hw = g.wbox;
    static const int n256 = getenv("TQ_CONV_N256") ? atoi(getenv("TQ_CONV_N256")) : 0;
    const int block_n = Cout <= 64 ? 64 : ((n256 && kind == 0 && a.acc_groups == 1 && Cout % 256 == 0) ? 256 : 128);
    g.n_tiles = (Cout + block_n - 1) / block_n;
    g.bias = (const float *)a.bias; g.bn_a = (const float *)a.bn_a; g.bn_b = (const float *)a.bn_b;
    g.residual = (const float *)a.residual;
    g.relu = a.relu ? 1 : 0;
    g.relu6 = a.relu == 2 ? 1 : 0;
    g.write_f32 = a.out_f32 ? 1 : 0;
    g.write_codes = a.out_codes ? 1 : 0;
    g.next_sf = a.out_codes ? a.next_sf : 1.0f;
    g.next_bits = a.out_codes ? a.next_bits : 1;
    g.next_terms = a.next_terms;
    g.next_fastdiv = (g.next_sf >= 9.313225746154785e-10f && g.next_sf <= 1073741824.0f) ? 1 : 0;
    if (kind == 1) {
        g.n_groups = g.planes_a + g.planes_w - 1;
        g.kcpg = g.kc_blocks;
        g.acc_int = 1;
    } else {
        if (a.acc_groups < 1 || g.kc_blocks % a.acc_groups != 0)
            return fail(TQ_ERR_INVALID, "acc_groups = %d must divide the %d 64-channel blocks of C", a.acc_groups, g.kc_blocks);
        g.n_groups = a.acc_groups;
        g.kcpg = g.kc_blocks / a.acc_groups;
        g.acc_int = a.acc_groups > 1 ? 1 : 0;
    }
    if (g.n_groups * block_n > 512 || (2 * g.n_groups * block_n > 512 && block_n != 128))
        return fail(TQ_ERR_UNSUPPORTED, "%d accumulator groups of %d columns exceed tensor memory", g.n_groups, block_n);
    const int taps = R * S * g.kc_blocks;
    static const bool no_prog = getenv("TQ_CONV_NO_PROG") != nullptr;
    if (kind == 0 && g.n_groups == 1 && !no_prog && Cout <= 64 && taps <= 12) {
        g.prog_steps = taps;
        g.nb_tiles = taps;
        static const bool no_halo = getenv("TQ_CONV_NO_HALO") != nullptr;
        static const bool halo_baseoff = getenv("TQ_CONV_HALO_BASEOFF") ? atoi(getenv("TQ_CONV_HALO_BASEOFF")) != 0 : false;
        if (!no_halo && g.kc_blocks == 1 && stride == 1 && R * S > 1) {
            ConvGeom h = g;
            static const int slack = getenv("TQ_CONV_HALO_SLACK") ? atoi(getenv("TQ_CONV_HALO_SLACK")) : 16;
            if (pick_box_halo(h) && (long)h.m_tiles * 100 <= (long)g.m_tiles * (100 + slack)) {
                g = h;
                g.halo = 1;
                g.halo_baseoff = halo_baseoff ? 1 : 0;
                static const int pair3_env = getenv("TQ_CONV_PAIR3") ? atoi(getenv("TQ_CONV_PAIR3")) : 0;
                static const int pair_env3 = getenv("TQ_CONV_PAIR") ? atoi(getenv("TQ_CONV_PAIR")) : 1;
                if (pair3_env && pair_env3 && !g.halo_baseoff && Cout % 16 == 0 && ((g.m_tiles + 1) / 2) * g.n_tiles >= num_sms() / 2) g.pair = 1;
            }
        }
    }

    g.step_w = g.wbox; g.step_h = g.hbox; g.off_w = 0; g.off_h = 0;
    static const bool no_halo4 = getenv("TQ_CONV_NO_HALO4") != nullptr;
    static const bool no_packed = getenv("TQ_CONV_NO_PACKED") != nullptr;
    if (kind == 0 && !no_halo4 && !no_packed && g.prog_steps == 0 && !g.halo && block_n == 128 && stride == 1 && R == 3 && S == 3 &&
        pad == 1 && N >= 2 && 2 * (W + 1) * (H + 1) <= 128) {
        const int per = (W + 1) * (H + 1);
        g.wbox = W; g.hbox = H; g.nbox = 128 / per < N ? 128 / per : N;
        g.hw = W + 1; g.img_h1 = H + 1;
        g.tiles_w = g.tiles_h = 1; g.tiles_n = (N + g.nbox - 1) / g.nbox; g.m_tiles = g.tiles_n;
        g.a_tx_bytes = g.nbox * per * GM_ROW_BYTES;
        g.step_w = g.wbox; g.step_h = g.hbox;
        g.halo = 1;
        static const int pair_env = getenv("TQ_CONV_PAIR") ? atoi(getenv("TQ_CONV_PAIR")) : 1;
        if (pair_env && ((g.m_tiles + 1) / 2) * g.n_tiles >= num_sms() / 2) g.pair = 1;
    }
    if (kind == 0 && !no_halo4 && g.prog_steps == 0 && !g.halo && block_n == 128 && stride == 1 && R * S > 1) {
        ConvGeom h = g;
        static const int slack4 = getenv("TQ_CONV_HALO_SLACK") ? atoi(getenv("TQ_CONV_HALO_SLACK")) : 16;
        if (pick_box_halo(h) && (long)h.m_tiles * 100 <= (long)g.m_tiles * (100 + slack4)) {
            h.step_w = h.wbox; h.step_h = h.hbox;
            g = h;
            g.halo = 1;
            static const int pair_env = getenv("TQ_CONV_PAIR") ? atoi(getenv("TQ_CONV_PAIR")) : 1;
            if (pair_env && ((g.m_tiles + 1) / 2) * g.n_tiles >= num_sms() / 2) g.pair = 1;
        }
    }
    const CUtensorMapDataType op_dt = kind == 1 ? CU_TENSOR_MAP_DATA_TYPE_UINT8 : CU_TENSOR_MAP_DATA_TYPE_FLOAT16;
    const int op_es = kind == 1 ? 1 : 2;
    int rc;
    {
        cuuint64_t dims[4] = {(cuuint64_t)C, (cuuint64_t)W, (cuuint64_t)H, (cuuint64_t)(g.planes_a * N)};
        cuuint32_t box[4] = {(cuuint32_t)g.kblk, (cuuint32_t)(g.wbox * stride), (cuuint32_t)(g.hbox * stride), (cuuint32_t)g.nbox};
        if (g.halo) { box[1] = (cuuint32_t)g.hw; box[2] = (cuuint32_t)(g.hbox + R - 1); }
        if (g.img_h1) { box[2] = (cuuint32_t)g.img_h1; box[3] = (cuuint32_t)g.nbox; }
        cuuint32_t estr[4] = {1, (cuuint32_t)stride, (cuuint32_t)stride, 1};
        if ((rc = encode_map(enc, &pl.tmA, op_dt, op_es, a.act, 4, dims, box, estr, "activations")) != TQ_OK) return rc;
    }
    {
        if (g.prog_steps > 0 && g.kc_blocks != 1) { g.halo = 0; g.pair = 0; g.prog_steps = 0; g.nb_tiles = 0; }
        cuuint64_t dims[3] = {(cuuint64_t)C, (cuuint64_t)Cout, (cuuint64_t)(g.planes_w * R * S)};
        cuuint32_t box[3] = {(cuuint32_t)g.kblk, (cuuint32_t)(g.pair ? block_n / 2 : block_n), 1};
        cuuint32_t estr[3] = {1, 1, 1};
        if ((rc = encode_map(enc, &pl.tmB, op_dt, op_es, a.wgt, 3, dims, box, estr, "weights")) != TQ_OK) return rc;
    }
    cuuint64_t odims[4] = {(cuuint64_t)Cout, (cuuint64_t)g.Wo, (cuuint64_t)g.Ho, (cuuint64_t)N};
    cuuint32_t one[4] = {1, 1, 1, 1};
    cuuint32_t obox[4] = {32, (cuuint32_t)g.wbox, (cuuint32_t)g.hbox, (cuuint32_t)g.nbox};
    pl.tmC = pl.tmA; pl.tmD = pl.tmA; pl.tmR = pl.tmA;
    if (a.out_f32 && (rc = encode_map(enc, &pl.tmC, CU_TENSOR_MAP_DATA_TYPE_FLOAT32, 4, a.out_f32, 4, odims, obox, one, "fp32 output")) != TQ_OK) return rc;
    if (a.out_codes && (rc = encode_map(enc, &pl.tmD, CU_TENSOR_MAP_DATA_TYPE_FLOAT16, 2, a.out_codes, 4, odims, obox, one, "code output",
                                        CU_TENSOR_MAP_SWIZZLE_64B)) != TQ_OK) return rc;
    if (a.residual && (rc = encode_map(enc, &pl.tmR, CU_TENSOR_MAP_DATA_TYPE_FLOAT32, 4, a.residual, 4, odims, obox, one, "residual")) != TQ_OK) return rc;
    if ((rc = pick_variant(g, block_n, kind, false, pl.variant)) != TQ_OK) return rc;
    pl.g = g;
    pl.key = a;
    return TQ_OK;
}

static int run_conv(ConvArgs &a, cudaStream_t s)
{
    int dev = 0;
    cudaGetDevice(&dev);
    a.device = dev;
    const uint64_t h = hash_args(a);
    static const bool no_cache = getenv("TQ_CONV_NO_PLAN_CACHE") != nullptr;
    ConvPlan pl;
    bool hit = false;
    if (!no_cache) {
        std::lock_guard<std::mutex> lk(g_plan_mu);
        for (const ConvPlan &c : g_plans[h & 63])
            if (memcmp(&c.key, &a, sizeof(ConvArgs)) == 0) { pl = c; hit = true; break; }
    }
    if (!hit) {
        int rc = plan_conv(a, pl);
        if (rc != TQ_OK) return rc;
        if (!no_cache) {
            std::lock_guard<std::mutex> lk(g_plan_mu);
            if (g_plan_count >= 4096) { for (auto &b : g_plans) b.clear(); g_plan_count = 0; }
            g_plans[h & 63].push_back(pl);
            ++g_plan_count;
        }
    }
    return launch_variant(pl.variant, pl.tmA, pl.tmB, pl.tmC, pl.tmD, pl.tmR, pl.g, s);
}

static int check_conv_args(const void *act, const void *wgt, const void *out_f32, const void *out_codes, const void *bias,
                           const void *bn_a, const void *bn_b, const void *residual, int N, int H, int W, int C, int Cout,
                           int R, int S, int stride, int pad, float next_sf, int next_bits, int next_terms, int c_align)
{
    if (!act || !wgt || (!out_f32 && !out_codes)) return fail(TQ_ERR_INVALID, "NULL pointer");
    if (N < 1 || H < 1 || W < 1 || C < 1 || Cout < 1 || R < 1 || S < 1 || stride < 1 || pad < 0)
        return fail(TQ_ERR_INVALID, "bad convolution geometry");
    if (C % c_align != 0) return fail(TQ_ERR_UNSUPPORTED, "input channels must be a multiple of %d (16-byte TMA rows), got %d", c_align, C);
    if (Cout % 4 != 0) return fail(TQ_ERR_UNSUPPORTED, "output channels must be a multiple of 4, got %d", Cout);
    if (out_codes && Cout % 8 != 0) return fail(TQ_ERR_UNSUPPORTED, "code output needs Cout %% 8 == 0, got %d", Cout);
    if ((bn_a == nullptr) != (bn_b == nullptr)) return fail(TQ_ERR_INVALID, "bn_a and bn_b go together");
    if ((((uintptr_t)act | (uintptr_t)wgt | (uintptr_t)out_f32 | (uintptr_t)out_codes | (uintptr_t)bias |
          (uintptr_t)bn_a | (uintptr_t)bn_b | (uintptr_t)residual) & 15u) != 0)
        return fail(TQ_ERR_INVALID, "pointers must be 16-byte aligned");
    if (out_codes) {
        if (!(next_sf > 0.0f) || !(next_sf < INFINITY)) return fail(TQ_ERR_INVALID, "next_sf must be positive and finite");
        if (next_bits < 1 || next_bits > GM_LUT_MAX_BITS) return fail(TQ_ERR_UNSUPPORTED, "fused encode supports 1..%d bits", GM_LUT_MAX_BITS);
        if (next_terms < 0) return fail(TQ_ERR_INVALID, "next_terms must be >= 0");
        if (!(next_sf >= 9.313225746154785e-10f && next_sf <= 1073741824.0f))
            return fail(TQ_ERR_UNSUPPORTED, "fused encode needs 2^-30 <= next_sf <= 2^30 (got %g): encode with tq_tr_encode_codes instead", (double)next_sf);
    }
    return TQ_OK;
}

}

using namespace tq;

extern "C" int tq_conv2d_codes_fused(const void *act, const void *wgt, float *out_f32, void *out_codes,
                                     const float *bias, const float *bn_a, const float *bn_b,
                                     const float *residual, int N, int H, int W, int C, int Cout, int R, int S,
                                     int stride, int pad, float scale, int relu, float next_sf, int next_bits,
                                     int next_terms, int acc_groups, void *stream)
{
    int rc = check_conv_args(act, wgt, out_f32, out_codes, bias, bn_a, bn_b, residual, N, H, W, C, Cout, R, S, stride, pad,
                             next_sf, next_bits, next_terms, 8);
    if (rc != TQ_OK) return rc;
    ConvArgs a;
    memset(&a, 0, sizeof(a));
    a.act = act; a.wgt = wgt; a.out_f32 = out_f32; a.out_codes = out_codes; a.bias = bias; a.bn_a = bn_a; a.bn_b = bn_b;
    a.residual = residual;
    a.kind = 0; a.N = N; a.H = H; a.W = W; a.C = C; a.Cout = Cout; a.R = R; a.S = S; a.stride = stride; a.pad = pad;
    a.relu = relu == 2 ? 2 : (relu ? 1 : 0); a.next_bits = out_codes ? next_bits : 1; a.next_terms = next_terms;
    a.acc_groups = acc_groups < 1 ? 1 : acc_groups; a.planes_a = 1; a.planes_w = 1;
    a.scale = scale; a.next_sf = out_codes ? next_sf : 1.0f;
    return run_conv(a, (cudaStream_t)stream);
}

extern "C" int tq_conv2d_codes_f16(const void *act, const void *wgt, const float *bias, float *out,
                                   int N, int H, int W, int C, int Cout, int R, int S, int stride, int pad,
                                   float scale, int acc_groups, void *stream)
{
    if (!out) return fail(TQ_ERR_INVALID, "NULL pointer");
    return tq_conv2d_codes_fused(act, wgt, out, nullptr, bias, nullptr, nullptr, nullptr, N, H, W, C, Cout, R, S,
                                 stride, pad, scale, 0, 1.0f, 1, 0, acc_groups, stream);
}

extern "C" int tq_conv2d_planes_i8(const void *act_planes, const void *wgt_planes, int planes_a, int planes_w,
                                   float *out_f32, void *out_codes, const float *bias, const float *bn_a,
                                   const float *bn_b, const float *residual, int N, int H, int W, int C, int Cout,
                                   int R, int S, int stride, int pad, float scale, int relu, float next_sf,
                                   int next_bits, int next_terms, int act_max, int wgt_max, void *stream)
{
    int rc = check_conv_args(act_planes, wgt_planes, out_f32, out_codes, bias, bn_a, bn_b, residual, N, H, W, C, Cout, R, S,
                             stride, pad, next_sf, next_bits, next_terms, 16);
    if (rc != TQ_OK) return rc;
    if (planes_a < 1 || planes_a > 2 || planes_w < 1 || planes_w > 2) return fail(TQ_ERR_INVALID, "1 or 2 planes per operand");
    const int acap = planes_a == 2 ? 2047 : 127, wcap = planes_w == 2 ? 2047 : 127;
    if (act_max < 1 || act_max > acap || wgt_max < 1 || wgt_max > wcap)
        return fail(TQ_ERR_INVALID, "act_max / wgt_max must lie in 1..%d / 1..%d for %d / %d planes", acap, wcap, planes_a, planes_w);
    if ((double)C * R * S * (double)act_max * (double)wgt_max >= 2147483648.0)
        return fail(TQ_ERR_UNSUPPORTED, "K = %d with |a| <= %d, |w| <= %d can overflow an int32 accumulator", C * R * S, act_max, wgt_max);
    ConvArgs a;
    memset(&a, 0, sizeof(a));
    a.act = act_planes; a.wgt = wgt_planes; a.out_f32 = out_f32; a.out_codes = out_codes; a.bias = bias; a.bn_a = bn_a;
    a.bn_b = bn_b; a.residual = residual;
    a.kind = 1; a.N = N; a.H = H; a.W = W; a.C = C; a.Cout = Cout; a.R = R; a.S = S; a.stride = stride; a.pad = pad;
    a.relu = relu == 2 ? 2 : (relu ? 1 : 0); a.next_bits = out_codes ? next_bits : 1; a.next_terms = next_terms;
    a.acc_groups = 1; a.planes_a = planes_a; a.planes_w = planes_w;
    a.scale = scale; a.next_sf = out_codes ? next_sf : 1.0f;
    return run_conv(a, (cudaStream_t)stream);
}

namespace tq {

__global__ void __launch_bounds__(256)
codes_to_planes_kernel(const __half *__restrict__ codes, int8_t *__restrict__ planes, int64_t n8, int64_t plane_stride,
                       int nplanes, int *__restrict__ overflow)
{
    bool ovf = false;
    for (int64_t i = (int64_t)blockIdx.x * blockDim.x + threadIdx.x; i < n8; i += (int64_t)gridDim.x * blockDim.x) {
        const uint4 v = __ldg(reinterpret_cast<const uint4 *>(codes) + i);
        const uint32_t w[4] = {v.x, v.y, v.z, v.w};
        uint32_t hi[2] = {0u, 0u}, lo[2] = {0u, 0u};
#pragma unroll
        for (int e = 0; e < 8; ++e) {
            const int c = __half2int_rn(__ushort_as_half((unsigned short)(w[e >> 1] >> (16 * (e & 1)))));
            int h, l;
            if (nplanes == 2) { h = c >> GM_I8_SHIFT; l = c & ((1 << GM_I8_SHIFT) - 1); }
            else { h = c; l = 0; }
            ovf |= (h < -128 || h > 127);
            hi[e >> 2] |= (uint32_t)(h & 0xFF) << (8 * (e & 3));
            lo[e >> 2] |= (uint32_t)(l & 0xFF) << (8 * (e & 3));
        }
        reinterpret_cast<uint2 *>(planes)[i] = make_uint2(hi[0], hi[1]);
        if (nplanes == 2) reinterpret_cast<uint2 *>(planes + plane_stride)[i] = make_uint2(lo[0], lo[1]);
    }
    if (ovf && overflow) atomicExch(overflow, 1);
}

__global__ void __launch_bounds__(128)
weight_l1_kernel(const __half *__restrict__ wgt, int RS, int Cout, int C, int kcb, long long *__restrict__ pos, long long *__restrict__ neg)
{
    const int co = blockIdx.x, kb = blockIdx.y;
    long long p = 0, m = 0;
    const int c0 = kb * GM_BLOCK_K, c1 = min(C, c0 + GM_BLOCK_K);
    for (int t = threadIdx.x; t < RS * (c1 - c0); t += blockDim.x) {
        const int tap = t / (c1 - c0), c = c0 + t % (c1 - c0);
        const int v = __half2int_rn(wgt[((int64_t)tap * Cout + co) * C + c]);
        if (v > 0) p += v; else m -= v;
    }
    __shared__ long long sp[128], sm[128];
    sp[threadIdx.x] = p; sm[threadIdx.x] = m;
    __syncthreads();
    for (int o = 64; o > 0; o >>= 1) {
        if ((int)threadIdx.x < o) { sp[threadIdx.x] += sp[threadIdx.x + o]; sm[threadIdx.x] += sm[threadIdx.x + o]; }
        __syncthreads();
    }
    if (threadIdx.x == 0) { pos[(int64_t)co * kcb + kb] = sp[0]; neg[(int64_t)co * kcb + kb] = sm[0]; }
}

}

extern "C" int tq_codes_to_planes(const void *codes_f16, void *planes_s8, int64_t n, int planes, int *overflow, void *stream)
{
    if (!codes_f16 || !planes_s8) return fail(TQ_ERR_INVALID, "NULL pointer");
    if (n < 0 || n % 8 != 0) return fail(TQ_ERR_INVALID, "element count must be a multiple of 8");
    if (planes != 1 && planes != 2) return fail(TQ_ERR_INVALID, "1 or 2 planes");
    if ((((uintptr_t)codes_f16 | (uintptr_t)planes_s8) & 15u) != 0) return fail(TQ_ERR_INVALID, "pointers must be 16-byte aligned");
    if (n == 0) return TQ_OK;
    int64_t blocks = (n / 8 + 255) / 256;
    if (blocks > (int64_t)num_sms() * 16) blocks = (int64_t)num_sms() * 16;
    codes_to_planes_kernel<<<(int)blocks, 256, 0, (cudaStream_t)stream>>>((const __half *)codes_f16, (int8_t *)planes_s8, n / 8, n,
                                                                        planes, overflow);
    count_launch();
    return check_launch("codes_to_planes_kernel");
}

extern "C" int tq_conv_weight_l1(const void *wgt_f16, int RS, int Cout, int C, long long *pos, long long *neg, void *stream)
{
    if (!wgt_f16 || !pos || !neg) return fail(TQ_ERR_INVALID, "NULL pointer");
    if (RS < 1 || Cout < 1 || C < 1) return fail(TQ_ERR_INVALID, "bad weight shape");
    const int kcb = (C + GM_BLOCK_K - 1) / GM_BLOCK_K;
    weight_l1_kernel<<<dim3((unsigned)Cout, (unsigned)kcb), 128, 0, (cudaStream_t)stream>>>((const __half *)wgt_f16, RS, Cout, C, kcb, pos, neg);
    count_launch();
    return check_launch("weight_l1_kernel");
}


namespace tq {

struct StemNorm { float mean[3], sd[3]; };
__device__ __forceinline__ float stem_pixel(uint8_t v, int c, const StemNorm &nm)
{
    const float t = __fdiv_rn((float)v, 255.0f);
    return __bfloat162float(__float2bfloat16_rn(__fdiv_rn(__fsub_rn(t, nm.mean[c]), nm.sd[c])));
}
template <typename T> __device__ __forceinline__ float stem_pixel(T v, int, const StemNorm &) { return Elem<T>::to_f32(v); }

template <typename Tin, bool LO>
__global__ void __launch_bounds__(256)
stem_prepare_kernel(const Tin *__restrict__ x, __half *__restrict__ x2, int N, int H, int W, int Hs, int Ws, StemNorm nm)
{
    __shared__ __half norm_lut[std::is_same<Tin, uint8_t>::value ? 768 : 1];
    if constexpr (std::is_same<Tin, uint8_t>::value) {
        for (int i = threadIdx.x; i < 768; i += blockDim.x) norm_lut[i] = __float2half_rn(stem_pixel((uint8_t)(i & 255), i >> 8, nm));
        __syncthreads();
    }
    const int64_t total = (int64_t)N * Hs * Ws;
    const int64_t plane = total * 16;
    for (int64_t t = (int64_t)blockIdx.x * blockDim.x + threadIdx.x; t < total; t += (int64_t)gridDim.x * blockDim.x) {
        const int ws = (int)(t % Ws), hs = (int)((t / Ws) % Hs), n = (int)(t / ((int64_t)Ws * Hs));
        __align__(16) __half hi[16], lo[16];
#pragma unroll
        for (int d = 0; d < 4; ++d) {
            const int h = 2 * hs + (d >> 1) - 3, w = 2 * ws + (d & 1) - 3;
            const bool in = h >= 0 && h < H && w >= 0 && w < W;
#pragma unroll
            for (int c = 0; c < 4; ++c) {
                if constexpr (std::is_same<Tin, uint8_t>::value) {
                    hi[d * 4 + c] = (in && c < 3) ? norm_lut[c * 256 + (int)x[(((int64_t)n * H + h) * W + w) * 3 + c]] : __float2half_rn(0.0f);
                } else {
                    float v = 0.0f;
                    if (in && c < 3) v = stem_pixel(x[(((int64_t)n * H + h) * W + w) * 3 + c], c, nm);
                    const __half vh = __float2half_rn(v);
                    hi[d * 4 + c] = vh;
                    if (LO) lo[d * 4 + c] = __float2half_rn(v - __half2float(vh));
                }
            }
        }
        uint4 *dh = reinterpret_cast<uint4 *>(x2 + t * 16);
        dh[0] = reinterpret_cast<const uint4 *>(hi)[0]; dh[1] = reinterpret_cast<const uint4 *>(hi)[1];
        if constexpr (LO) {
            uint4 *dl = reinterpret_cast<uint4 *>(x2 + plane + t * 16);
            dl[0] = reinterpret_cast<const uint4 *>(lo)[0]; dl[1] = reinterpret_cast<const uint4 *>(lo)[1];
        }
    }
}

}

constexpr int STEM_U8 = 100;

static int stem_impl(const void *x, int x_dtype, void *x2_scratch, const void *w2, float *out, void *out_codes,
                     const float *bn_a, const float *bn_b, int relu, int pool, float next_sf, int next_bits,
                     int next_terms, int N, int H, int W, int Cout, void *stream, const float *mean3 = nullptr,
                     const float *std3 = nullptr)
{
    if (!x || !x2_scratch || !w2 || !out) return fail(TQ_ERR_INVALID, "NULL pointer");
    if (x_dtype != TQ_F32 && x_dtype != TQ_BF16 && x_dtype != TQ_F16 && x_dtype != STEM_U8)
        return fail(TQ_ERR_UNSUPPORTED, "stem conv input must be fp32, bf16, fp16 or uint8");
    StemNorm nm{};
    if (x_dtype == STEM_U8) {
        if (!mean3 || !std3) return fail(TQ_ERR_INVALID, "uint8 images need mean3 / std3");
        for (int c = 0; c < 3; ++c) {
            if (!(std3[c] > 0.0f)) return fail(TQ_ERR_INVALID, "std must be positive");
            nm.mean[c] = mean3[c]; nm.sd[c] = std3[c];
        }
    }
    const bool lo_plane = x_dtype == TQ_F32;
    if (N < 1 || H < 2 || W < 2 || (H & 1) || (W & 1)) return fail(TQ_ERR_INVALID, "H and W must be even");
    if (Cout < 4 || Cout % 4) return fail(TQ_ERR_UNSUPPORTED, "Cout must be a multiple of 4");
    if ((((uintptr_t)x2_scratch | (uintptr_t)w2 | (uintptr_t)out) & 15u) != 0)
        return fail(TQ_ERR_INVALID, "pointers must be 16-byte aligned");
    EncodeTiledFn enc = encode_tiled();
    if (!enc) return fail(TQ_ERR_CUDA, "cuTensorMapEncodeTiled is not available from this driver");
    cudaStream_t s = (cudaStream_t)stream;
    const int Ho = H / 2, Wo = W / 2, Hs = Ho + 3, Ws = Wo + 3;

    {
        const int64_t total = (int64_t)N * Hs * Ws;
        int64_t blocks = (total + 255) / 256;
        if (blocks > (int64_t)num_sms() * 16) blocks = (int64_t)num_sms() * 16;
        if (x_dtype == TQ_F32)
            stem_prepare_kernel<float, true><<<(int)blocks, 256, 0, s>>>((const float *)x, (__half *)x2_scratch, N, H, W, Hs, Ws, nm);
        else if (x_dtype == TQ_BF16)
            stem_prepare_kernel<__nv_bfloat16, false><<<(int)blocks, 256, 0, s>>>((const __nv_bfloat16 *)x, (__half *)x2_scratch, N, H, W, Hs, Ws, nm);
        else if (x_dtype == STEM_U8)
            stem_prepare_kernel<uint8_t, false><<<(int)blocks, 256, 0, s>>>((const uint8_t *)x, (__half *)x2_scratch, N, H, W, Hs, Ws, nm);
        else
            stem_prepare_kernel<__half, false><<<(int)blocks, 256, 0, s>>>((const __half *)x, (__half *)x2_scratch, N, H, W, Hs, Ws, nm);
        count_launch();
        int rc = check_launch("stem_prepare_kernel");
        if (rc != TQ_OK) return rc;
    }

    ConvGeom g{};
    g.N = N; g.H = Hs; g.W = Wo; g.C = 64; g.Cout = Cout; g.R = 4; g.S = 1; g.stride = 1; g.pad = 0;
    g.Ho = Ho; g.Wo = Wo;
    g.scale = 1.0f;
    g.kc_blocks = 1;
    int Hp = 0, Wp = 0;
    if (!pool) {
        if (!pick_box_halo(g)) return fail(TQ_ERR_UNSUPPORTED, "stem conv: no tile shape");
        g.step_w = g.wbox; g.step_h = g.hbox;
    } else {
        Hp = (Ho + 2 - 3) / 2 + 1; Wp = (Wo + 2 - 3) / 2 + 1;
        long best = -1;
        for (int P = 1; P <= Hp && 2 * P + 1 <= 128; ++P)
            for (int Q = 1; Q <= Wp && (2 * P + 1) * (2 * Q + 1) <= 128; ++Q) {
                const long tiles = (long)((Hp + P - 1) / P) * ((Wp + Q - 1) / Q);
                if (best < 0 || tiles < best || (tiles == best && Q > g.pool_q)) { best = tiles; g.pool_p = P; g.pool_q = Q; }
            }
        g.pool = 1;
        g.wbox = 2 * g.pool_q + 1; g.hbox = 2 * g.pool_p + 1; g.nbox = 1;
        g.step_w = 2 * g.pool_q; g.step_h = 2 * g.pool_p; g.off_w = -1; g.off_h = -1;
        g.tiles_w = (Wp + g.pool_q - 1) / g.pool_q; g.tiles_h = (Hp + g.pool_p - 1) / g.pool_p; g.tiles_n = N;
        g.m_tiles = g.tiles_w * g.tiles_h * g.tiles_n;
        g.a_tx_bytes = g.wbox * g.hbox * GM_BLOCK_K * 2;
        if (g.pool_p * g.pool_q > 32) return fail(TQ_ERR_UNSUPPORTED, "pooled tile too large");
        g.bn_a = bn_a; g.bn_b = bn_b; g.relu = relu ? 1 : 0;
        g.write_codes = out_codes ? 1 : 0;
        if (out_codes) {
            if (!(next_sf > 0.0f) || !(next_sf < INFINITY)) return fail(TQ_ERR_INVALID, "next_sf must be positive and finite");
            if (next_bits < 1 || next_bits > GM_LUT_MAX_BITS || next_terms < 0) return fail(TQ_ERR_UNSUPPORTED, "fused encode supports 1..%d bits", GM_LUT_MAX_BITS);
        }
    }
    g.hw = g.wbox;
    const int block_n = Cout <= 64 ? 64 : 128;
    g.n_tiles = (Cout + block_n - 1) / block_n;
    g.write_f32 = 1;
    g.next_sf = out_codes ? next_sf : 1.0f; g.next_bits = out_codes ? next_bits : 1; g.next_terms = next_terms;
    g.next_fastdiv = (g.next_sf >= 9.313225746154785e-10f && g.next_sf <= 1073741824.0f) ? 1 : 0;
    static const int split_rows = getenv("TQ_STEM_SPLIT") ? atoi(getenv("TQ_STEM_SPLIT")) : 1;
    g.prog_steps = lo_plane ? 8 : 4; g.nb_tiles = 4; g.n_groups = split_rows ? 4 : 2; g.b_rows = 128;
    for (uint32_t R = 0; R < 4; ++R) {
        g.prog_mma[R] = 1u | (R << 4) | (((R < 2 || !split_rows) ? 0u : 2u) << 8);
        g.prog_mma[4 + R] = g.prog_mma[R];
    }

    CUtensorMap tmA, tmB, tmC, tmD;
    int rc;
    {
        cuuint64_t dims[4] = {64, (cuuint64_t)Wo, (cuuint64_t)Hs, (cuuint64_t)((lo_plane ? 2 : 1) * N)};
        cuuint64_t strides[3] = {32, (cuuint64_t)Ws * 32, (cuuint64_t)Hs * Ws * 32};
        cuuint32_t box[4] = {64, (cuuint32_t)g.wbox, (cuuint32_t)(g.hbox + g.R - 1), 1};
        cuuint32_t one[4] = {1, 1, 1, 1};
        g.a_tx_bytes = g.wbox * (g.hbox + g.R - 1) * GM_BLOCK_K * 2;
        g.halo = 1;
        CUresult r = enc(&tmA, CU_TENSOR_MAP_DATA_TYPE_FLOAT16, 4, x2_scratch, dims, strides, box, one,
                         CU_TENSOR_MAP_INTERLEAVE_NONE, CU_TENSOR_MAP_SWIZZLE_128B, CU_TENSOR_MAP_L2_PROMOTION_L2_256B,
                         CU_TENSOR_MAP_FLOAT_OOB_FILL_NONE);
        if (r != CUDA_SUCCESS) return fail(TQ_ERR_CUDA, "cuTensorMapEncodeTiled(stem windows) failed: %d", (int)r);
    }
    {
        cuuint64_t dims[3] = {64, 128, 4};
        cuuint32_t box[3] = {64, 128, 1};
        cuuint32_t one[3] = {1, 1, 1};
        if ((rc = encode_map(enc, &tmB, CU_TENSOR_MAP_DATA_TYPE_FLOAT16, 2, w2, 3, dims, box, one, "stem weights")) != TQ_OK) return rc;
    }
    tmD = tmA;
    if (!pool) {
        cuuint64_t odims[4] = {(cuuint64_t)Cout, (cuuint64_t)Wo, (cuuint64_t)Ho, (cuuint64_t)N};
        cuuint32_t box[4] = {32, (cuuint32_t)g.wbox, (cuuint32_t)g.hbox, (cuuint32_t)g.nbox};
        cuuint32_t one[4] = {1, 1, 1, 1};
        if ((rc = encode_map(enc, &tmC, CU_TENSOR_MAP_DATA_TYPE_FLOAT32, 4, out, 4, odims, box, one, "stem output")) != TQ_OK) return rc;
    } else {
        cuuint64_t odims[4] = {(cuuint64_t)Cout, (cuuint64_t)Wp, (cuuint64_t)Hp, (cuuint64_t)N};
        cuuint32_t box[4] = {32, (cuuint32_t)g.pool_q, (cuuint32_t)g.pool_p, 1};
        cuuint32_t one[4] = {1, 1, 1, 1};
        if ((rc = encode_map(enc, &tmC, CU_TENSOR_MAP_DATA_TYPE_FLOAT32, 4, out, 4, odims, box, one, "pooled output")) != TQ_OK) return rc;
        if (out_codes && (rc = encode_map(enc, &tmD, CU_TENSOR_MAP_DATA_TYPE_FLOAT16, 2, out_codes, 4, odims, box, one,
                                          "pooled codes", CU_TENSOR_MAP_SWIZZLE_64B)) != TQ_OK) return rc;
    }
    if (g.nbox != 1) return fail(TQ_ERR_UNSUPPORTED, "stem conv expects images of at least 128 output pixels");
    if (block_n != 64) return fail(TQ_ERR_UNSUPPORTED, "stem conv supports Cout <= 64");
    g.kblk = GM_BLOCK_K; g.kcpg = 1; g.planes_a = g.planes_w = 1; g.acc_int = 0;
    ConvVariant variant = CV_NONE;
    if ((rc = pick_variant(g, 64, 0, true, variant)) != TQ_OK) return rc;
    return launch_variant(variant, tmA, tmB, tmC, tmD, tmA, g, s);
}

extern "C" int tq_stem_conv7x7s2_dt(const void *x, int x_dtype, void *x2_scratch, const void *w2, float *out,
                                    int N, int H, int W, int Cout, void *stream)
{
    return stem_impl(x, x_dtype, x2_scratch, w2, out, nullptr, nullptr, nullptr, 0, 0, 1.0f, 1, 0, N, H, W, Cout, stream);
}

extern "C" int tq_stem_conv7x7s2_pool(const void *x, int x_dtype, void *x2_scratch, const void *w2,
                                      const float *bn_a, const float *bn_b, int relu, float *out, void *out_codes,
                                      int N, int H, int W, int Cout, float next_sf, int next_bits, int next_terms,
                                      void *stream)
{
    if (!bn_a || !bn_b) return fail(TQ_ERR_INVALID, "NULL pointer");
    if (Cout % 8) return fail(TQ_ERR_UNSUPPORTED, "Cout must be a multiple of 8");
    if ((((uintptr_t)bn_a | (uintptr_t)bn_b | (uintptr_t)out_codes) & 15u) != 0) return fail(TQ_ERR_INVALID, "pointers must be 16-byte aligned");
    return stem_impl(x, x_dtype, x2_scratch, w2, out, out_codes, bn_a, bn_b, relu, 1, next_sf, next_bits, next_terms,
                     N, H, W, Cout, stream);
}

extern "C" int tq_stem_conv7x7s2_u8(const void *x_u8, const float *mean3, const float *std3, void *x2_scratch, const void *w2,
                                    float *out, int N, int H, int W, int Cout, void *stream)
{
    return stem_impl(x_u8, STEM_U8, x2_scratch, w2, out, nullptr, nullptr, nullptr, 0, 0, 1.0f, 1, 0, N, H, W, Cout, stream,
                     mean3, std3);
}

extern "C" int tq_stem_conv7x7s2(const float *x, void *x2_scratch, const void *w2, float *out,
                                 int N, int H, int W, int Cout, void *stream)
{
    return tq_stem_conv7x7s2_dt(x, TQ_F32, x2_scratch, w2, out, N, H, W, Cout, stream);
}
```

term_quantization_b200/csrc/tq_pool.cu:

```cuda
#include <cuda.h>

#include "tq_common.cuh"

typedef CUresult (*EncodeTiledFn)(CUtensorMap *, CUtensorMapDataType, cuuint32_t, void *, const cuuint64_t *,
                                  const cuuint64_t *, const cuuint32_t *, const cuuint32_t *, CUtensorMapInterleave,
                                  CUtensorMapSwizzle, CUtensorMapL2promotion, CUtensorMapFloatOOBfill);
namespace tq {
EncodeTiledFn encode_tiled();
}

namespace tq {

struct PoolParams {
    int N, H, W, C, Ho, Wo;
    int relu;
    float next_sf;
    int next_bits, next_terms, next_fastdiv, write_codes;
};

__global__ void __launch_bounds__(256)
bn_relu_maxpool3x3s2_kernel(const float *__restrict__ x, const float *__restrict__ bn_a,
                            const float *__restrict__ bn_b, float *__restrict__ out,
                            __half *__restrict__ codes, PoolParams p)
{
    extern __shared__ __half lut[];
    if (p.write_codes) {
        for (uint32_t i = threadIdx.x; i < (2u << p.next_bits); i += blockDim.x) {
            const int code = elem_code(i & ((1u << p.next_bits) - 1u), TQ_ENC_HESE, p.next_terms);
            lut[i] = __int2half_rn((i >> p.next_bits) ? -code : code);
        }
        __syncthreads();
    }
    const Quant nq = make_quant(p.write_codes ? p.next_sf : 1.0f, (float)((1u << p.next_bits) - 1u));
    const int c4n = p.C >> 2;
    const int64_t total = (int64_t)p.N * p.Ho * p.Wo * c4n;
    for (int64_t t = (int64_t)blockIdx.x * blockDim.x + threadIdx.x; t < total; t += (int64_t)gridDim.x * blockDim.x) {
        const int c4 = (int)(t % c4n);
        const int64_t pix = t / c4n;
        const int wo = (int)(pix % p.Wo), ho = (int)((pix / p.Wo) % p.Ho), n = (int)(pix / ((int64_t)p.Wo * p.Ho));
        const float4 a = __ldg(reinterpret_cast<const float4 *>(bn_a) + c4);
        const float4 b = __ldg(reinterpret_cast<const float4 *>(bn_b) + c4);
        float4 m = make_float4(-INFINITY, -INFINITY, -INFINITY, -INFINITY);
#pragma unroll
        for (int dy = 0; dy < 3; ++dy) {
            const int h = ho * 2 - 1 + dy;
            if (h < 0 || h >= p.H) continue;
#pragma unroll
            for (int dx = 0; dx < 3; ++dx) {
                const int w = wo * 2 - 1 + dx;
                if (w < 0 || w >= p.W) continue;
                const float4 v = __ldg(reinterpret_cast<const float4 *>(x + (((int64_t)n * p.H + h) * p.W + w) * p.C) + c4);
                m.x = fmaxf(m.x, __fmaf_rn(v.x, a.x, b.x));
                m.y = fmaxf(m.y, __fmaf_rn(v.y, a.y, b.y));
                m.z = fmaxf(m.z, __fmaf_rn(v.z, a.z, b.z));
                m.w = fmaxf(m.w, __fmaf_rn(v.w, a.w, b.w));
            }
        }
        if (p.relu) { m.x = fmaxf(m.x, 0.f); m.y = fmaxf(m.y, 0.f); m.z = fmaxf(m.z, 0.f); m.w = fmaxf(m.w, 0.f); }
        reinterpret_cast<float4 *>(out)[t] = m;
        if (p.write_codes) {
            const float vv[4] = {m.x, m.y, m.z, m.w};
            uint32_t hc[4];
#pragma unroll
            for (int e = 0; e < 4; ++e) {
                const uint32_t neg = __float_as_uint(vv[e]) >> 31;
                const uint32_t q = p.next_fastdiv ? quantize_f32<true>(vv[e], nq) : quantize_f32<false>(vv[e], nq);
                hc[e] = __half_as_ushort(lut[q | (neg << p.next_bits)]);
            }
            reinterpret_cast<uint2 *>(codes)[t] = make_uint2(hc[0] | (hc[1] << 16), hc[2] | (hc[3] << 16));
        }
    }
}

constexpr int PT_PR = 4, PT_PC = 7, PT_CB = 64, PT_IH = 2 * PT_PR + 1, PT_IW = 2 * PT_PC + 1;
constexpr int PT_STAGE_BYTES = PT_IH * PT_IW * PT_CB * 4;
constexpr int PT_STAGES = 3;
constexpr int PT_THREADS = PT_PR * PT_PC * (PT_CB / 4);

__global__ void __launch_bounds__(PT_THREADS, 2)
bn_relu_maxpool3x3s2_tiled_kernel(const __grid_constant__ CUtensorMap tmIn, const float *__restrict__ bn_a,
                                  const float *__restrict__ bn_b, float *__restrict__ out,
                                  __half *__restrict__ codes, PoolParams p)
{
    extern __shared__ __align__(128) uint8_t pool_smem[];
    uint8_t *base = reinterpret_cast<uint8_t *>((reinterpret_cast<uintptr_t>(pool_smem) + 127) & ~uintptr_t(127));
    __half *lut = reinterpret_cast<__half *>(base + PT_STAGES * PT_STAGE_BYTES);
    uint64_t *full = reinterpret_cast<uint64_t *>(base + PT_STAGES * PT_STAGE_BYTES + (((size_t)(2u << p.next_bits) * 2 + 15) & ~(size_t)15));
    if (p.write_codes) {
        for (uint32_t i = threadIdx.x; i < (2u << p.next_bits); i += blockDim.x) {
            const int code = elem_code(i & ((1u << p.next_bits) - 1u), TQ_ENC_HESE, p.next_terms);
            lut[i] = __int2half_rn((i >> p.next_bits) ? -code : code);
        }
    }
    auto s32 = [](const void *q) { return (uint32_t)__cvta_generic_to_shared(q); };
    if (threadIdx.x == 0) {
        for (int i = 0; i < PT_STAGES; ++i) asm volatile("mbarrier.init.shared::cta.b64 [%0], 1;" ::"r"(s32(&full[i])));
        asm volatile("fence.mbarrier_init.release.cluster;" ::: "memory");
        asm volatile("prefetch.tensormap [%0];" ::"l"(&tmIn) : "memory");
    }
    __syncthreads();
    const Quant nq = make_quant(p.write_codes ? p.next_sf : 1.0f, (float)((1u << p.next_bits) - 1u));
    const int cblocks = p.C / PT_CB, tiles_w = (p.Wo + PT_PC - 1) / PT_PC, tiles_h = (p.Ho + PT_PR - 1) / PT_PR;
    const int64_t total = (int64_t)p.N * tiles_h * tiles_w * cblocks;
    const int C4 = p.C >> 2;
    constexpr int c4n = PT_CB / 4;
    auto issue = [&](int64_t t, int stage) {
        const int cb = (int)(t % cblocks);
        const int64_t r = t / cblocks;
        const int tw = (int)(r % tiles_w), th = (int)((r / tiles_w) % tiles_h), n = (int)(r / ((int64_t)tiles_w * tiles_h));
        const uint32_t bar = s32(&full[stage]);
        asm volatile("mbarrier.arrive.expect_tx.shared::cta.b64 _, [%0], %1;" ::"r"(bar), "r"((uint32_t)PT_STAGE_BYTES) : "memory");
        asm volatile(
            "cp.async.bulk.tensor.4d.shared::cluster.global.mbarrier::complete_tx::bytes [%0], [%1, {%3, %4, %5, %6}], [%2];"
            ::"r"(s32(base + stage * PT_STAGE_BYTES)), "l"(&tmIn), "r"(bar), "r"(cb * PT_CB), "r"(tw * PT_PC * 2 - 1),
              "r"(th * PT_PR * 2 - 1), "r"(n) : "memory");
    };
    int stage = 0;
    uint32_t phases = 0u;
    if (threadIdx.x == 0)
        for (int i = 0; i < PT_STAGES - 1; ++i)
            if ((int64_t)blockIdx.x + (int64_t)i * gridDim.x < total) issue(blockIdx.x + (int64_t)i * gridDim.x, i);
    for (int64_t t = blockIdx.x; t < total; t += gridDim.x) {
        const int64_t next = t + (int64_t)(PT_STAGES - 1) * gridDim.x;
        if (threadIdx.x == 0 && next < total) issue(next, (stage + PT_STAGES - 1) % PT_STAGES);
        {
            const uint32_t bar = s32(&full[stage]);
            asm volatile(
                "{\n\t"
                ".reg .pred P1;\n\t"
                "PT_WAIT:\n\t"
                "mbarrier.try_wait.parity.shared::cta.b64 P1, [%0], %1;\n\t"
                "@P1 bra PT_DONE;\n\t"
                "bra PT_WAIT;\n\t"
                "PT_DONE:\n\t"
                "}" ::"r"(bar), "r"((phases >> stage) & 1u) : "memory");
            phases ^= 1u << stage;
        }
        const int cb = (int)(t % cblocks);
        const int64_t r = t / cblocks;
        const int tw = (int)(r % tiles_w), th = (int)((r / tiles_w) % tiles_h), n = (int)(r / ((int64_t)tiles_w * tiles_h));
        const int h0 = th * PT_PR * 2 - 1, w0 = tw * PT_PC * 2 - 1;
        const float4 *tile = reinterpret_cast<const float4 *>(base + stage * PT_STAGE_BYTES);
        for (int o = threadIdx.x; o < PT_PR * PT_PC * c4n; o += blockDim.x) {
            const int c4 = o % c4n, pw = (o / c4n) % PT_PC, ph = o / (c4n * PT_PC);
            const int ho = th * PT_PR + ph, wo = tw * PT_PC + pw;
            if (ho >= p.Ho || wo >= p.Wo) continue;
            const int cg = cb * c4n + c4;
            const float4 a = __ldg(reinterpret_cast<const float4 *>(bn_a) + cg);
            const float4 b = __ldg(reinterpret_cast<const float4 *>(bn_b) + cg);
            const float ninf = -INFINITY;
            float4 m = make_float4(ninf, ninf, ninf, ninf);
#pragma unroll
            for (int dy = 0; dy < 3; ++dy) {
                const int h = h0 + 2 * ph + dy;
                if (h < 0 || h >= p.H) continue;
#pragma unroll
                for (int dx = 0; dx < 3; ++dx) {
                    const int w = w0 + 2 * pw + dx;
                    if (w < 0 || w >= p.W) continue;
                    const float4 v = tile[((2 * ph + dy) * PT_IW + 2 * pw + dx) * c4n + c4];
                    m.x = fmaxf(m.x, __fmaf_rn(v.x, a.x, b.x));
                    m.y = fmaxf(m.y, __fmaf_rn(v.y, a.y, b.y));
                    m.z = fmaxf(m.z, __fmaf_rn(v.z, a.z, b.z));
                    m.w = fmaxf(m.w, __fmaf_rn(v.w, a.w, b.w));
                }
            }
            if (p.relu) { m.x = fmaxf(m.x, 0.f); m.y = fmaxf(m.y, 0.f); m.z = fmaxf(m.z, 0.f); m.w = fmaxf(m.w, 0.f); }
            const int64_t oi = (((int64_t)n * p.Ho + ho) * p.Wo + wo) * C4 + cg;
            reinterpret_cast<float4 *>(out)[oi] = m;
            if (p.write_codes) {
                const float vv[4] = {m.x, m.y, m.z, m.w};
                uint32_t hc[4];
#pragma unroll
                for (int e = 0; e < 4; ++e) {
                    const uint32_t neg = __float_as_uint(vv[e]) >> 31;
                    const uint32_t q = p.next_fastdiv ? quantize_f32<true>(vv[e], nq) : quantize_f32<false>(vv[e], nq);
                    hc[e] = __half_as_ushort(lut[q | (neg << p.next_bits)]);
                }
                reinterpret_cast<uint2 *>(codes)[oi] = make_uint2(hc[0] | (hc[1] << 16), hc[2] | (hc[3] << 16));
            }
        }
        __syncthreads();
        stage = stage + 1 == PT_STAGES ? 0 : stage + 1;
    }
}

}

using namespace tq;

extern "C" int tq_bn_relu_maxpool_encode(const float *x, const float *bn_a, const float *bn_b, float *out,
                                         void *out_codes, int N, int H, int W, int C, int relu,
                                         float next_sf, int next_bits, int next_terms, void *stream)
{
    if (!x || !bn_a || !bn_b || !out) return fail(TQ_ERR_INVALID, "NULL pointer");
    if (N < 1 || H < 1 || W < 1 || C < 4 || C % 4) return fail(TQ_ERR_INVALID, "bad shape (C must be a multiple of 4)");
    if ((((uintptr_t)x | (uintptr_t)bn_a | (uintptr_t)bn_b | (uintptr_t)out | (uintptr_t)out_codes) & 15u) != 0)
        return fail(TQ_ERR_INVALID, "pointers must be 16-byte aligned");
    PoolParams p{};
    p.N = N; p.H = H; p.W = W; p.C = C;
    p.Ho = (H + 2 - 3) / 2 + 1;
    p.Wo = (W + 2 - 3) / 2 + 1;
    p.relu = relu ? 1 : 0;
    p.write_codes = out_codes ? 1 : 0;
    p.next_sf = out_codes ? next_sf : 1.0f;
    p.next_bits = out_codes ? next_bits : 1;
    p.next_terms = next_terms;
    if (out_codes) {
        if (!(next_sf > 0.0f) || !(next_sf < INFINITY)) return fail(TQ_ERR_INVALID, "next_sf must be positive and finite");
        if (next_bits < 1 || next_bits > 11 || next_terms < 0) return fail(TQ_ERR_UNSUPPORTED, "fused encode supports 1..11 bits");
    }
    p.next_fastdiv = (p.next_sf >= 9.313225746154785e-10f && p.next_sf <= 1073741824.0f) ? 1 : 0;
    static const int tiled_env = getenv("TQ_POOL_TILED") ? atoi(getenv("TQ_POOL_TILED")) : 1;
    if (tiled_env && C % PT_CB == 0 && p.Ho >= PT_PR && p.Wo >= PT_PC) {
        EncodeTiledFn enc = encode_tiled();
        if (enc) {
            CUtensorMap tm;
            cuuint64_t dims[4] = {(cuuint64_t)C, (cuuint64_t)W, (cuuint64_t)H, (cuuint64_t)N};
            cuuint64_t strides[3] = {(cuuint64_t)C * 4, (cuuint64_t)W * C * 4, (cuuint64_t)H * W * C * 4};
            cuuint32_t box[4] = {(cuuint32_t)PT_CB, (cuuint32_t)PT_IW, (cuuint32_t)PT_IH, 1};
            cuuint32_t one[4] = {1, 1, 1, 1};
            CUresult r = enc(&tm, CU_TENSOR_MAP_DATA_TYPE_FLOAT32, 4, const_cast<float *>(x), dims, strides, box, one,
                             CU_TENSOR_MAP_INTERLEAVE_NONE, CU_TENSOR_MAP_SWIZZLE_NONE, CU_TENSOR_MAP_L2_PROMOTION_L2_256B,
                             CU_TENSOR_MAP_FLOAT_OOB_FILL_NONE);
            if (r != CUDA_SUCCESS) return fail(TQ_ERR_CUDA, "cuTensorMapEncodeTiled(pool input) failed: %d", (int)r);
            const size_t smem_t = PT_STAGES * (size_t)PT_STAGE_BYTES + (((size_t)(2u << p.next_bits) * 2 + 15) & ~(size_t)15) + 64 + 128;
            static bool attr_done[64] = {false};
            int dev = 0;
            cudaGetDevice(&dev);
            if (dev >= 0 && dev < 64 && !attr_done[dev]) {
                if (cudaFuncSetAttribute(bn_relu_maxpool3x3s2_tiled_kernel, cudaFuncAttributeMaxDynamicSharedMemorySize, 112 * 1024) != cudaSuccess)
                    return check_launch("cudaFuncSetAttribute(bn_relu_maxpool3x3s2_tiled_kernel)");
                attr_done[dev] = true;
            }
            const int64_t tiles = (int64_t)N * ((p.Ho + PT_PR - 1) / PT_PR) * ((p.Wo + PT_PC - 1) / PT_PC) * (C / PT_CB);
            const int64_t capt = (int64_t)num_sms() * 2;
            bn_relu_maxpool3x3s2_tiled_kernel<<<(int)(tiles < capt ? tiles : capt), PT_THREADS, smem_t, (cudaStream_t)stream>>>(
                tm, bn_a, bn_b, out, (__half *)out_codes, p);
            count_launch();
            return check_launch("bn_relu_maxpool3x3s2_tiled_kernel");
        }
    }
    const int64_t total = (int64_t)N * p.Ho * p.Wo * (C / 4);
    int64_t blocks = (total + 255) / 256;
    const int64_t cap = (int64_t)num_sms() * 16;
    if (blocks > cap) blocks = cap;
    const size_t smem = out_codes ? (size_t)(2u << p.next_bits) * sizeof(__half) : 0;
    bn_relu_maxpool3x3s2_kernel<<<(int)blocks, 256, smem, (cudaStream_t)stream>>>(
        x, bn_a, bn_b, out, (__half *)out_codes, p);
    count_launch();
    return check_launch("bn_relu_maxpool3x3s2_kernel");
}


namespace tq {

__global__ void __launch_bounds__(256)
u8_normalize_bf16_kernel(const uint8_t *__restrict__ x, __nv_bfloat16 *__restrict__ y, int64_t npix4,
                         float m0, float m1, float m2, float s0, float s1, float s2)
{
    const float mean[3] = {m0, m1, m2}, sd[3] = {s0, s1, s2};
    for (int64_t t = (int64_t)blockIdx.x * blockDim.x + threadIdx.x; t < npix4; t += (int64_t)gridDim.x * blockDim.x) {
        const uint32_t *src = reinterpret_cast<const uint32_t *>(x) + t * 3;
        const uint32_t w[3] = {__ldg(src), __ldg(src + 1), __ldg(src + 2)};
        __align__(8) __nv_bfloat16 out[12];
#pragma unroll
        for (int k = 0; k < 12; ++k) {
            const float v = __fdiv_rn((float)((w[k >> 2] >> (8 * (k & 3))) & 0xFFu), 255.0f);
            out[k] = __float2bfloat16_rn(__fdiv_rn(__fsub_rn(v, mean[k % 3]), sd[k % 3]));
        }
        uint2 *dst = reinterpret_cast<uint2 *>(y + t * 12);
        dst[0] = reinterpret_cast<const uint2 *>(out)[0];
        dst[1] = reinterpret_cast<const uint2 *>(out)[1];
        dst[2] = reinterpret_cast<const uint2 *>(out)[2];
    }
}

}

extern "C" int tq_u8_normalize_bf16(const void *x_u8, void *y_bf16, int64_t npix, const float *mean3, const float *std3,
                                    void *stream)
{
    if (!x_u8 || !y_bf16 || !mean3 || !std3) return fail(TQ_ERR_INVALID, "NULL pointer");
    if (npix < 0 || npix % 4 != 0) return fail(TQ_ERR_INVALID, "pixel count must be a multiple of 4");
    if ((((uintptr_t)x_u8 & 3u) | ((uintptr_t)y_bf16 & 7u)) != 0) return fail(TQ_ERR_INVALID, "pointers must be 4 / 8-byte aligned");
    for (int c = 0; c < 3; ++c)
        if (!(std3[c] > 0.0f)) return fail(TQ_ERR_INVALID, "std must be positive");
    if (npix == 0) return TQ_OK;
    const int64_t n4 = npix / 4;
    int64_t blocks = (n4 + 255) / 256;
    const int64_t cap = (int64_t)num_sms() * 16;
    if (blocks > cap) blocks = cap;
    u8_normalize_bf16_kernel<<<(int)blocks, 256, 0, (cudaStream_t)stream>>>((const uint8_t *)x_u8, (__nv_bfloat16 *)y_bf16, n4,
                                                                          mean3[0], mean3[1], mean3[2], std3[0], std3[1], std3[2]);
    count_launch();
    return check_launch("u8_normalize_bf16_kernel");
}
```

term_quantization_b200/fused.py:

```python
import torch
import torch.nn as nn
import torch.nn.functional as F

from . import conv_codes, tr_cuda, tr_layer


def _bn_affine(bn):
    with torch.no_grad():
        a = bn.weight * torch.rsqrt(bn.running_var + bn.eps)
        b = torch.addcmul(bn.bias, -bn.running_mean, a)
    return a.float().contiguous(), b.float().contiguous()


def _quant_key(layer):
    q = layer.input_quant
    return (float(q.sf), int(q.data_bits), int(q.data_terms))


class _Conv:

    def __init__(self, layer, bn, post_relu=True, engine="auto"):
        why = layer.tensor_core_blocker()
        if why is not None:
            raise NotImplementedError(f"fused path: {why}")
        if layer.input_quant.tracking:
            raise RuntimeError("calibrate the model (set_tr_tracking(model, False)) before fusing")
        if layer._tc_weight is None or layer._tc_key != layer._weight_key():
            layer.use_tensor_cores(True, engine)
        self.layer = layer
        self.w = layer._tc_weight
        self.plan = conv_codes.plan_weight(self.w, 1 << int(layer.input_quant.data_bits), signed_act=not post_relu,
                                           engine=engine)
        self.quant = _quant_key(layer)
        sfx32 = torch.tensor(self.quant[0], dtype=torch.float32)
        self.scale = (sfx32 * torch.tensor(layer._tc_wsf32, dtype=torch.float32)).item()
        self.bias = layer.conv.bias
        self.bn = _bn_affine(bn) if bn is not None else None
        c = layer.conv
        self.ks, self.stride, self.pad = c.kernel_size, c.stride[0], c.padding[0]

    def check_fresh(self):
        layer = self.layer
        if layer._tc_weight is not self.w or layer._tc_key != layer._weight_key() or _quant_key(layer) != self.quant:
            raise RuntimeError("the wrapped model changed after fusing (weights, device or scale factors): "
                               "build the fused executor again")

    def __call__(self, codes, residual=None, relu=False, want_f32=True, next_quant=None):
        return conv_codes.conv2d_codes_fused(codes, self.w, self.ks, self.stride, self.pad, self.scale,
                                             bias=self.bias, bn=self.bn, residual=residual, relu=relu,
                                             want_f32=want_f32, next_quant=next_quant, plan=self.plan)


class FusedResNet(nn.Module):

    def __init__(self, model, stem="tcgen05", engine="auto"):
        super().__init__()
        if stem not in ("tcgen05", "tcgen05_pool", "cudnn"):
            raise ValueError("stem must be 'tcgen05', 'tcgen05_pool' or 'cudnn'")
        self.stem_mode = stem
        self.model = model.to(memory_format=torch.channels_last).eval()
        self.blocks = []
        for stage in (model.layer1, model.layer2, model.layer3, model.layer4):
            for blk in stage:
                if not (isinstance(blk.conv1, tr_layer.TRConv2dLayer) and isinstance(blk.conv2, tr_layer.TRConv2dLayer)
                        and hasattr(blk, "bn2") and not hasattr(blk, "conv3")):
                    raise NotImplementedError("FusedResNet expects TQ-converted BasicBlocks")
                down = None
                if blk.downsample is not None:
                    if not isinstance(blk.downsample[0], tr_layer.TRConv2dLayer):
                        raise NotImplementedError("downsample conv must be a TRConv2dLayer")
                    down = _Conv(blk.downsample[0], blk.downsample[1], engine=engine)
                self.blocks.append((_Conv(blk.conv1, blk.bn1, engine=engine), _Conv(blk.conv2, blk.bn2, engine=engine), down))
        mp = model.maxpool
        self.fuse_stem = (isinstance(mp, nn.MaxPool2d) and mp.kernel_size in (3, (3, 3)) and mp.stride in (2, (2, 2))
                          and mp.padding in (1, (1, 1)) and mp.dilation in (1, (1, 1)) and not mp.ceil_mode
                          and model.conv1.out_channels % 8 == 0 and self.blocks[0][0].quant[1] <= 10)
        self.stem_bn = _bn_affine(model.bn1)
        c1 = model.conv1
        self.stem_w = None
        if (stem != "cudnn" and self.fuse_stem and tuple(c1.weight.shape[1:]) == (3, 7, 7) and c1.stride == (2, 2)
                and c1.padding == (3, 3) and c1.dilation == (1, 1) and c1.groups == 1 and c1.bias is None
                and c1.out_channels <= 64):
            self.stem_w = conv_codes.pack_stem_weight(c1.weight)
            if stem == "tcgen05_pool":
                self.stem_w_pool, self.stem_bn_pool = conv_codes.stem_pool_operands(c1.weight, self.stem_bn)
        self._stem_scratch = None

    @staticmethod
    def _encode(x_nhwc, quant):
        sf, bits, terms = quant
        return tr_cuda.tr_codes(x_nhwc.view(1, -1, 1, 1), sf, bits, 1, terms,
                                dtype=torch.float16).view(x_nhwc.shape)

    def chain_description(self):
        def d(c):
            if c is None:
                return None
            return {"w": c.w.cpu().numpy().astype("int32"), "ks": tuple(c.ks), "stride": c.stride, "pad": c.pad,
                    "scale": c.scale, "bias": None if c.bias is None else c.bias.detach().float().cpu().numpy(),
                    "bn": None if c.bn is None else (c.bn[0].cpu().numpy(), c.bn[1].cpu().numpy()),
                    "quant": c.quant, "engine": c.plan.engine, "groups": c.plan.groups}
        return [(d(c1), d(c2), d(down)) for c1, c2, down in self.blocks]

    @torch.no_grad()
    def forward_u8(self, x_u8_nhwc, mean, std):
        H, W = x_u8_nhwc.shape[1], x_u8_nhwc.shape[2]
        if (self.fuse_stem and self.stem_w is not None and self.stem_mode != "tcgen05_pool" and H % 2 == 0 and W % 2 == 0
                and (H // 2) * (W // 2) >= 128):
            return self.forward(x_u8_nhwc, u8_norm=(tuple(mean), tuple(std)))
        from . import inference
        return self.forward(inference.normalize_u8(x_u8_nhwc, mean, std))

    def forward(self, x, capture=None, u8_norm=None):
        m = self.model
        if not torch.cuda.is_current_stream_capturing():
            for blk in self.blocks:
                for c in blk:
                    if c is not None:
                        c.check_fresh()
        if u8_norm is not None:
            q0 = self.blocks[0][0].quant
            y, self._stem_scratch = conv_codes.stem_conv7x7s2_u8(x, u8_norm[0], u8_norm[1], self.stem_w, self._stem_scratch,
                                                                 cout=m.conv1.out_channels)
            cur, c0 = conv_codes.bn_relu_maxpool_encode(y, self.stem_bn, relu=True, next_quant=q0)
            codes = {q0: c0}
        elif self.fuse_stem:
            x = x.contiguous(memory_format=torch.channels_last)
            q0 = self.blocks[0][0].quant
            if self.stem_w is not None and x.shape[2] % 2 == 0 and x.shape[3] % 2 == 0 \
                    and (x.shape[2] // 2) * (x.shape[3] // 2) >= 128:
                if self.stem_mode == "tcgen05_pool":
                    cur, c0, self._stem_scratch = conv_codes.stem_conv_pool(
                        x.permute(0, 2, 3, 1), self.stem_w_pool, self.stem_bn_pool, relu=True, next_quant=q0,
                        scratch=self._stem_scratch)
                else:
                    y, self._stem_scratch = conv_codes.stem_conv7x7s2(x.permute(0, 2, 3, 1), self.stem_w,
                                                                      self._stem_scratch, cout=m.conv1.out_channels)
                    cur, c0 = conv_codes.bn_relu_maxpool_encode(y, self.stem_bn, relu=True, next_quant=q0)
            else:
                y = m.conv1(x.float()).permute(0, 2, 3, 1)
                cur, c0 = conv_codes.bn_relu_maxpool_encode(y, self.stem_bn, relu=True, next_quant=q0)
            codes = {q0: c0}
        else:
            x = x.contiguous(memory_format=torch.channels_last)
            x = m.maxpool(m.relu(m.bn1(m.conv1(x.float()))))
            cur = x.permute(0, 2, 3, 1)
            codes = {}
        if capture is not None:
            capture["stem"] = cur
        for i, (c1, c2, down) in enumerate(self.blocks):
            def get(q):
                if q not in codes:
                    codes[q] = self._encode(cur, q)
                return codes[q]
            identity = cur if down is None else down(get(down.quant), want_f32=True)[0]
            _, mid = c1(get(c1.quant), relu=True, want_f32=False, next_quant=c2.quant)
            nxt = self.blocks[i + 1][0].quant if i + 1 < len(self.blocks) else None
            cur, out_codes = c2(mid, residual=identity, relu=True, want_f32=True, next_quant=nxt)
            codes = {nxt: out_codes} if nxt is not None else {}
        if capture is not None:
            capture["final"] = cur
        y = cur.permute(0, 3, 1, 2)
        return m.fc(torch.flatten(m.avgpool(y), 1))


def _first_conv_ok(c):
    return (c.in_channels == 3 and c.out_channels in (32, 64) and c.kernel_size == (3, 3) and c.padding == (1, 1)
            and c.stride in ((1, 1), (2, 2)) and c.dilation == (1, 1) and c.groups == 1 and c.weight.dtype == torch.float32)


def _square(pool):
    def one(v):
        return v if isinstance(v, int) else (v[0] if v[0] == v[1] else None)
    k, s, p = one(pool.kernel_size), one(pool.stride if pool.stride is not None else pool.kernel_size), one(pool.padding)
    return k is not None and s is not None and p is not None and k <= 7 and 2 * p <= k


class FusedVGG(nn.Module):

    def __init__(self, model):
        super().__init__()
        self.model = model.to(memory_format=torch.channels_last).eval()
        mods = list(model.features.children())
        if not isinstance(mods[0], nn.Conv2d) or isinstance(mods[0], tr_layer.TRConv2dLayer):
            raise NotImplementedError("FusedVGG expects an unwrapped first conv")
        self.stages = []
        i = 0
        post_relu = False
        while i < len(mods):
            m = mods[i]
            if isinstance(m, nn.ReLU):
                post_relu = True
            elif not isinstance(m, nn.MaxPool2d) and not isinstance(m, tr_layer.TRConv2dLayer):
                post_relu = False
            if isinstance(m, tr_layer.TRConv2dLayer):
                bn = None
                relu = False
                j = i + 1
                if j < len(mods) and isinstance(mods[j], nn.BatchNorm2d):
                    bn = mods[j]
                    j += 1
                if j < len(mods) and isinstance(mods[j], nn.ReLU):
                    relu = True
                    j += 1
                self.stages.append(("conv", (_Conv(m, bn, post_relu=post_relu), relu)))
                post_relu = relu
                i = j
            elif isinstance(m, nn.MaxPool2d):
                if m.dilation not in (1, (1, 1)) or m.ceil_mode:
                    raise NotImplementedError("FusedVGG: unsupported max-pool")
                self.stages.append(("pool", m))
                i += 1
            else:
                self.stages.append(("torch", m))
                i += 1
        self.first_tr = next(k for k, (kind, _) in enumerate(self.stages) if kind == "conv")
        if any(kind == "torch" for kind, _ in self.stages[self.first_tr:]):
            raise NotImplementedError("FusedVGG: unexpected module after the first wrapped conv")
        convs = [k for k, (kind, _) in enumerate(self.stages) if kind == "conv"]
        for k in convs[:-1]:
            if not self.stages[k][1][1]:
                raise NotImplementedError("FusedVGG: conv without ReLU before a quantiser")

    def chain_description(self):
        out = []
        for kind, payload in self.stages[self.first_tr:]:
            if kind == "conv":
                c, relu = payload
                out.append(("conv", {"w": c.w.cpu().numpy().astype("int32"), "ks": tuple(c.ks), "stride": c.stride, "pad": c.pad,
                                     "scale": c.scale, "bias": None if c.bias is None else c.bias.detach().float().cpu().numpy(),
                                     "bn": None if c.bn is None else (c.bn[0].cpu().numpy(), c.bn[1].cpu().numpy()),
                                     "quant": c.quant, "engine": c.plan.engine, "groups": c.plan.groups}, bool(relu)))
            else:
                one = lambda v: v if isinstance(v, int) else v[0]
                out.append(("pool", one(payload.kernel_size), one(payload.stride if payload.stride is not None else payload.kernel_size),
                            one(payload.padding)))
        return out

    @torch.no_grad()
    def forward(self, x, capture=None):
        m = self.model
        if not torch.cuda.is_current_stream_capturing():
            for kind, payload in self.stages:
                if kind == "conv":
                    payload[0].check_fresh()
        x = x.float().contiguous(memory_format=torch.channels_last)
        convs = [k for k, (kind, _) in enumerate(self.stages) if kind == "conv"]
        q0 = self.stages[convs[0]][1][0].quant
        stem = [mod for _, mod in self.stages[:self.first_tr]]
        if (len(stem) == 3 and isinstance(stem[0], nn.Conv2d) and isinstance(stem[1], nn.BatchNorm2d)
                and isinstance(stem[2], nn.ReLU) and stem[0].out_channels % 4 == 0):
            c0 = stem[0]
            if getattr(self, "_stem_bn", None) is None:
                self._stem_bn = _bn_affine(stem[1])
            bias0 = None if c0.bias is None else c0.bias.detach().float().contiguous()
            if _first_conv_ok(c0):
                if getattr(self, "_stem_w", None) is None:
                    self._stem_w = conv_codes.pack_first_conv_weight(c0.weight)
                _, codes = conv_codes.first_conv3x3_fused(x.permute(0, 2, 3, 1), self._stem_w, c0.stride[0], bias0, self._stem_bn,
                                                          relu=True, next_quant=q0)
            else:
                y = F.conv2d(x, c0.weight, None, c0.stride, c0.padding, c0.dilation, c0.groups).permute(0, 2, 3, 1).contiguous()
                _, codes = conv_codes.bn_act_encode(y, self._stem_bn, relu=True, next_quant=q0, bias=bias0)
        else:
            for mod in stem:
                x = mod(x)
            codes = FusedResNet._encode(x.permute(0, 2, 3, 1), q0)
        if capture is not None:
            capture["stem_codes"] = codes
        out = None
        for k in range(self.first_tr, len(self.stages)):
            kind, payload = self.stages[k]
            if kind == "conv":
                conv, relu = payload
                nxt = next((self.stages[j][1][0].quant for j in range(k + 1, len(self.stages))
                            if self.stages[j][0] == "conv"), None)
                if nxt is not None:
                    _, codes = conv(codes, relu=relu, want_f32=False, next_quant=nxt)
                else:
                    out, _ = conv(codes, relu=relu, want_f32=True)
                    codes = None
            else:
                if codes is not None and codes.shape[-1] % 8 == 0 and _square(payload):
                    codes = conv_codes.maxpool_codes(codes, payload.kernel_size, payload.stride, payload.padding)
                    continue
                t = codes if codes is not None else out
                t = payload(t.permute(0, 3, 1, 2)).permute(0, 2, 3, 1)
                if codes is not None:
                    codes = t.contiguous()
                else:
                    out = t.contiguous()
        if capture is not None:
            capture["final"] = out
        y = out.permute(0, 3, 1, 2)
        return m.classifier(torch.flatten(m.avgpool(y), 1))


class _Depthwise:

    def __init__(self, layer, bn):
        c = layer.conv
        if not (c.groups == c.in_channels == c.out_channels and c.kernel_size == (3, 3) and c.padding == (1, 1)
                and c.stride in ((1, 1), (2, 2)) and c.dilation == (1, 1) and c.in_channels % 8 == 0):
            raise NotImplementedError("fused depthwise path: 3x3 / pad 1 / stride 1 or 2 depthwise convs with C % 8 == 0")
        if layer.input_quant.tracking:
            raise RuntimeError("calibrate the model (set_tr_tracking(model, False)) before fusing")
        if layer.data_bits > 11 or layer.weight_bits > 16:
            raise NotImplementedError("fused depthwise path: int32 accumulator needs data_bits <= 11, weight_bits <= 16")
        self.layer = layer
        self.w, wsf32 = conv_codes.pack_depthwise_weight(c.weight, layer.w_sf)
        self.quant = _quant_key(layer)
        self.scale = (torch.tensor(self.quant[0], dtype=torch.float32) * torch.tensor(wsf32, dtype=torch.float32)).item()
        self.bias = c.bias
        self.bn = _bn_affine(bn) if bn is not None else None
        self.stride = c.stride[0]

    def __call__(self, codes, relu=False, want_f32=False, next_quant=None, post_relu=False):
        return conv_codes.depthwise3x3_codes(codes, self.w, self.stride, self.scale, bias=self.bias, bn=self.bn, relu=relu,
                                             want_f32=want_f32, next_quant=next_quant,
                                             act_unsigned=post_relu and self.quant[1] <= 9)


class FusedMobileNet(nn.Module):

    def __init__(self, model, engine="auto"):
        super().__init__()
        from torchvision.models.mobilenetv2 import InvertedResidual
        self.model = model.to(memory_format=torch.channels_last).eval()
        feats = list(model.features.children())
        stem = list(feats[0].children())
        if not (isinstance(stem[0], nn.Conv2d) and not isinstance(stem[0], tr_layer.TRConv2dLayer)
                and isinstance(stem[1], nn.BatchNorm2d) and isinstance(stem[2], nn.ReLU6)):
            raise NotImplementedError("FusedMobileNet expects an unwrapped conv-BN-ReLU6 stem")
        self.stem_conv, self.stem_bn = stem[0], _bn_affine(stem[1])
        self.blocks = []
        post_relu = True
        for blk in feats[1:-1]:
            if not isinstance(blk, InvertedResidual):
                raise NotImplementedError("FusedMobileNet expects InvertedResidual blocks")
            mods = list(blk.conv.children())
            expand = None
            if len(mods) == 4:
                e = list(mods[0].children())
                expand = _Conv(e[0], e[1], post_relu=post_relu, engine=engine)
                mods = mods[1:]
            d = list(mods[0].children())
            dw = _Depthwise(d[0], d[1])
            proj = _Conv(mods[1], mods[2], post_relu=True, engine=engine)
            self.blocks.append((expand, dw, proj, blk.use_res_connect))
            post_relu = False
        last = list(feats[-1].children())
        self.last = _Conv(last[0], last[1], post_relu=False, engine=engine)

    def chain_description(self):
        def conv(c):
            if c is None:
                return None
            return {"w": c.w.cpu().numpy().astype("int32"), "ks": tuple(c.ks), "stride": c.stride, "pad": c.pad,
                    "scale": c.scale, "bias": None if c.bias is None else c.bias.detach().float().cpu().numpy(),
                    "bn": None if c.bn is None else (c.bn[0].cpu().numpy(), c.bn[1].cpu().numpy()),
                    "quant": c.quant, "engine": c.plan.engine, "groups": c.plan.groups}

        def dwd(d):
            return {"w": d.w.cpu().numpy(), "stride": d.stride, "scale": d.scale,
                    "bias": None if d.bias is None else d.bias.detach().float().cpu().numpy(),
                    "bn": None if d.bn is None else (d.bn[0].cpu().numpy(), d.bn[1].cpu().numpy()), "quant": d.quant}
        return {"blocks": [(conv(e), dwd(d), conv(p), bool(r)) for e, d, p, r in self.blocks], "last": conv(self.last)}

    @torch.no_grad()
    def forward(self, x, capture=None):
        m = self.model
        if not torch.cuda.is_current_stream_capturing():
            for expand, dw, proj, _ in self.blocks:
                for c in (expand, proj):
                    if c is not None:
                        c.check_fresh()
                if _quant_key(dw.layer) != dw.quant:
                    raise RuntimeError("the wrapped model was re-calibrated after fusing: build the fused executor again")
            self.last.check_fresh()
        x = x.contiguous(memory_format=torch.channels_last)
        first = self.blocks[0][0] or self.blocks[0][1]
        c0 = self.stem_conv
        if _first_conv_ok(c0):
            if getattr(self, "_stem_w", None) is None:
                self._stem_w = conv_codes.pack_first_conv_weight(c0.weight)
            bias0 = None if c0.bias is None else c0.bias.detach().float().contiguous()
            _, codes = conv_codes.first_conv3x3_fused(x.float().permute(0, 2, 3, 1), self._stem_w, c0.stride[0], bias0,
                                                      self.stem_bn, relu="relu6", next_quant=first.quant)
        else:
            y = c0(x.float()).permute(0, 2, 3, 1)
            _, codes = conv_codes.bn_act_encode(y.contiguous(), self.stem_bn, relu="relu6", next_quant=first.quant)
        if capture is not None:
            capture["stem_codes"] = codes
        cur = None
        for i, (expand, dw, proj, use_res) in enumerate(self.blocks):
            h = codes
            if expand is not None:
                _, h = expand(h, relu="relu6", want_f32=False, next_quant=dw.quant)
            _, h = dw(h, relu="relu6", next_quant=proj.quant, post_relu=True)
            nxt = self.blocks[i + 1] if i + 1 < len(self.blocks) else None
            nq = ((nxt[0] or nxt[1]).quant if nxt is not None else self.last.quant)
            need_f32 = nxt is not None and nxt[3]
            cur, codes = proj(h, residual=cur if use_res else None, relu=False, want_f32=need_f32, next_quant=nq)
        out, _ = self.last(codes, relu="relu6", want_f32=True)
        if capture is not None:
            capture["final"] = out
        y = out.permute(0, 3, 1, 2)
        return m.classifier(torch.flatten(nn.functional.adaptive_avg_pool2d(y, (1, 1)), 1))
```

Before: 146,400.

## Split stem maxpool: horizontal row-max in stem epilogue, vertical pool kernel

The stem conv epilogue gains a pool==2 mode that takes the horizontal 3-wide stride-2 max across lanes with warp shuffles and stores only row maxima, halving the width of the stem output written to global memory. The BN/ReLU/maxpool kernel is templated on kernel width so a 1-wide variant can finish the vertical 3x1 max, BN and encode on that narrower tensor. This cuts stem-output write and reread traffic. The horizontal max now runs before BN, so the stem uses the pool-specific weights and BN operands (stem_pool_operands), presumably with the BN sign folded in so the max still commutes.

```diff
diff --git a/include/tq_b200.h b/include/tq_b200.h
--- a/include/tq_b200.h
+++ b/include/tq_b200.h
@@ -98,6 +98,14 @@
                            int N, int H, int W, int Cout, float next_sf, int next_bits, int next_terms,
                            void *stream);
 
+int tq_stem_conv7x7s2_rowmax(const void *x, int x_dtype, void *x2_scratch, const void *w2, float *out,
+                             int N, int H, int W, int Cout, void *stream);
+int tq_stem_conv7x7s2_u8_rowmax(const void *x_u8, const float *mean3, const float *std3, void *x2_scratch,
+                                const void *w2, float *out, int N, int H, int W, int Cout, void *stream);
+int tq_bn_relu_maxpool_encode_rowmax(const float *x, const float *bn_a, const float *bn_b, float *out,
+                                     void *out_codes, int N, int H, int W, int C, int relu,
+                                     float next_sf, int next_bits, int next_terms, void *stream);
+
 int tq_depthwise3x3_codes(const void *act_codes, const int32_t *wgt_codes, float *out_f32, void *out_codes,
                           const float *bias, const float *bn_a, const float *bn_b, int N, int H, int W, int C,
                           int stride, float scale, int relu, int act_unsigned, float next_sf, int next_bits,
diff --git a/term_quantization_b200/_lib.py b/term_quantization_b200/_lib.py
--- a/term_quantization_b200/_lib.py
+++ b/term_quantization_b200/_lib.py
@@ -35,6 +35,9 @@
     "tq_stem_conv7x7s2_dt": (_i, [_p, _i, _p, _p, _p, _i, _i, _i, _i, _p]),
     "tq_stem_conv7x7s2_u8": (_i, [_p, _p, _p, _p, _p, _p, _i, _i, _i, _i, _p]),
     "tq_stem_conv7x7s2_pool": (_i, [_p, _i, _p, _p, _p, _p, _i, _p, _p, _i, _i, _i, _i, _f, _i, _i, _p]),
+    "tq_stem_conv7x7s2_rowmax": (_i, [_p, _i, _p, _p, _p, _i, _i, _i, _i, _p]),
+    "tq_stem_conv7x7s2_u8_rowmax": (_i, [_p, _p, _p, _p, _p, _p, _i, _i, _i, _i, _p]),
+    "tq_bn_relu_maxpool_encode_rowmax": (_i, [_p] * 5 + [_i] * 5 + [_f, _i, _i, _p]),
     "tq_selftest_division": (_i, [C.c_uint64, C.c_uint32, _p, _p]),
 }
 
diff --git a/term_quantization_b200/conv_codes.py b/term_quantization_b200/conv_codes.py
--- a/term_quantization_b200/conv_codes.py
+++ b/term_quantization_b200/conv_codes.py
@@ -307,16 +307,17 @@
     return out, codes
 
 
-def bn_relu_maxpool_encode(x_nhwc, bn, relu=True, next_quant=None):
+def bn_relu_maxpool_encode(x_nhwc, bn, relu=True, next_quant=None, rowmax=False):
     if x_nhwc.dtype != torch.float32 or not x_nhwc.is_contiguous() or not x_nhwc.is_cuda:
         raise RuntimeError("bn_relu_maxpool_encode expects a contiguous fp32 CUDA [N, H, W, C] tensor")
     N, H, W, C = x_nhwc.shape
-    Ho, Wo = (H - 1) // 2 + 1, (W - 1) // 2 + 1
+    Ho, Wo = (H - 1) // 2 + 1, (W if rowmax else (W - 1) // 2 + 1)
     out = torch.empty((N, Ho, Wo, C), dtype=torch.float32, device=x_nhwc.device)
     codes = torch.empty((N, Ho, Wo, C), dtype=torch.float16, device=x_nhwc.device) if next_quant else None
     sf, bits, terms = next_quant if next_quant else (1.0, 1, 0)
+    fn = _lib.lib().tq_bn_relu_maxpool_encode_rowmax if rowmax else _lib.lib().tq_bn_relu_maxpool_encode
     with torch.cuda.device(x_nhwc.device):
-        rc = _lib.lib().tq_bn_relu_maxpool_encode(
+        rc = fn(
             x_nhwc.data_ptr(), bn[0].data_ptr(), bn[1].data_ptr(), out.data_ptr(),
             codes.data_ptr() if codes is not None else None, N, H, W, C, int(bool(relu)),
             float(sf), int(bits), int(terms), torch.cuda.current_stream(x_nhwc.device).cuda_stream)
@@ -344,7 +345,11 @@
 _STEM_DTYPES = {torch.float32: _lib.TQ_F32, torch.bfloat16: _lib.TQ_BF16, torch.float16: _lib.TQ_F16}
 
 
-def stem_conv7x7s2(x_nhwc, w2, scratch=None, cout=None):
+def _stem_out_w(W, rowmax):
+    return (W // 2 - 1) // 2 + 1 if rowmax else W // 2
+
+
+def stem_conv7x7s2(x_nhwc, w2, scratch=None, cout=None, rowmax=False):
     if x_nhwc.dtype not in _STEM_DTYPES or not x_nhwc.is_contiguous() or x_nhwc.shape[-1] != 3:
         raise RuntimeError("stem_conv7x7s2 expects a contiguous fp32 / bf16 / fp16 [N, H, W, 3] tensor")
     N, H, W, _ = x_nhwc.shape
@@ -352,16 +357,17 @@
     need = (2 if x_nhwc.dtype == torch.float32 else 1) * N * (H // 2 + 3) * (W // 2 + 3) * 16
     if scratch is None or scratch.numel() < need:
         scratch = torch.empty(need, dtype=torch.float16, device=x_nhwc.device)
-    out = torch.empty((N, H // 2, W // 2, Cout), dtype=torch.float32, device=x_nhwc.device)
+    out = torch.empty((N, H // 2, _stem_out_w(W, rowmax), Cout), dtype=torch.float32, device=x_nhwc.device)
+    fn = _lib.lib().tq_stem_conv7x7s2_rowmax if rowmax else _lib.lib().tq_stem_conv7x7s2_dt
     with torch.cuda.device(x_nhwc.device):
-        rc = _lib.lib().tq_stem_conv7x7s2_dt(x_nhwc.data_ptr(), _STEM_DTYPES[x_nhwc.dtype], scratch.data_ptr(),
+        rc = fn(x_nhwc.data_ptr(), _STEM_DTYPES[x_nhwc.dtype], scratch.data_ptr(),
                                              w2.data_ptr(), out.data_ptr(), N, H, W, Cout,
                                              torch.cuda.current_stream(x_nhwc.device).cuda_stream)
     _lib.check(rc)
     return out, scratch
 
 
-def stem_conv7x7s2_u8(x_u8_nhwc, mean, std, w2, scratch=None, cout=None):
+def stem_conv7x7s2_u8(x_u8_nhwc, mean, std, w2, scratch=None, cout=None, rowmax=False):
     import ctypes
     if x_u8_nhwc.dtype != torch.uint8 or not x_u8_nhwc.is_contiguous() or not x_u8_nhwc.is_cuda or x_u8_nhwc.shape[-1] != 3:
         raise RuntimeError("stem_conv7x7s2_u8 expects a contiguous uint8 CUDA [N, H, W, 3] tensor")
@@ -370,11 +376,12 @@
     need = N * (H // 2 + 3) * (W // 2 + 3) * 16
     if scratch is None or scratch.numel() < need:
         scratch = torch.empty(need, dtype=torch.float16, device=x_u8_nhwc.device)
-    out = torch.empty((N, H // 2, W // 2, Cout), dtype=torch.float32, device=x_u8_nhwc.device)
+    out = torch.empty((N, H // 2, _stem_out_w(W, rowmax), Cout), dtype=torch.float32, device=x_u8_nhwc.device)
     m = (ctypes.c_float * 3)(*mean)
     s = (ctypes.c_float * 3)(*std)
+    fn = _lib.lib().tq_stem_conv7x7s2_u8_rowmax if rowmax else _lib.lib().tq_stem_conv7x7s2_u8
     with torch.cuda.device(x_u8_nhwc.device):
-        rc = _lib.lib().tq_stem_conv7x7s2_u8(x_u8_nhwc.data_ptr(), ctypes.cast(m, ctypes.c_void_p), ctypes.cast(s, ctypes.c_void_p),
+        rc = fn(x_u8_nhwc.data_ptr(), ctypes.cast(m, ctypes.c_void_p), ctypes.cast(s, ctypes.c_void_p),
                                              scratch.data_ptr(), w2.data_ptr(), out.data_ptr(), N, H, W, Cout,
                                              torch.cuda.current_stream(x_u8_nhwc.device).cuda_stream)
     _lib.check(rc)
diff --git a/term_quantization_b200/csrc/tq_gemm.cu b/term_quantization_b200/csrc/tq_gemm.cu
--- a/term_quantization_b200/csrc/tq_gemm.cu
+++ b/term_quantization_b200/csrc/tq_gemm.cu
@@ -902,6 +902,41 @@
                 TR_SINCE(1, tl0);
                 TR_T0(tq0);
                 if constexpr (MODE == 2) {
+                    if (g.pool == 2) {
+                        const int Q = g.pool_q, ql = lane >> 1, q = tw * Q + ql;
+                        const bool left = q > 0, right = 2 * q + 1 < g.Wo;
+#pragma unroll
+                        for (int j = 0; j < 32; ++j) {
+                            const float c = __shfl_down_sync(0xFFFFFFFFu, t[j], 1);
+                            const float r = __shfl_down_sync(0xFFFFFFFFu, t[j], 2);
+                            const float m = right ? fmaxf(c, r) : c;
+                            t[j] = left ? fmaxf(t[j], m) : m;
+                        }
+                        TR_SINCE(2, tq0);
+                        TR_T0(tq2);
+                        if (store_thread) bulk_wait_read0();
+                        epi_bar_sync(1 + grp);
+                        TR_SINCE(4, tq2);
+                        TR_T0(tq3);
+                        if (!(lane & 1) && ql < Q) {
+                            const int o = ew * Q + ql;
+                            uint8_t *orow = st_f32 + o * 128;
+                            const uint32_t sw = (uint32_t)(o & 7);
+#pragma unroll
+                            for (int j = 0; j < 32; j += 4)
+                                *reinterpret_cast<float4 *>(orow + (((uint32_t)(j >> 2) ^ sw) << 4)) =
+                                    make_float4(t[j], t[j + 1], t[j + 2], t[j + 3]);
+                        }
+                        TR_SINCE(5, tq3);
+                        fence_proxy_async();
+                        epi_bar_sync(1 + grp);
+                        if (store_thread) {
+                            tma_store_4d(&tmC, st_f32, c0, tw * Q, th * g.hbox, n0);
+                            bulk_commit();
+                        }
+                        TR_SINCE(6, tq0);
+                        continue;
+                    }
                     if (g.pool) {
                         {
                             uint8_t *frow = st_f32 + mrow * 128;
@@ -1120,7 +1155,7 @@
         g.ring_off = g.a_stages * g.a_stage_bytes;
     }
     g.epi_codes_off = (g.write_f32 || g.residual) ? GM_EPI_F32_BYTES : 0;
-    g.epi_group_bytes = g.epi_codes_off + ((g.write_codes || g.pool) ? GM_EPI_CODE_BYTES : 0);
+    g.epi_group_bytes = g.epi_codes_off + ((g.write_codes || g.pool == 1) ? GM_EPI_CODE_BYTES : 0);
     const int epi_bytes = GM_EPI_GROUPS * g.epi_group_bytes;
     const int fixed = g.ring_off + epi_bytes + (2 << GM_LUT_MAX_BITS) * 2 + 1024  + 1024 ;
     int stages = (GM_SMEM_BUDGET - fixed) / g.stage_bytes;
@@ -1683,6 +1718,14 @@
     if (!pool) {
         if (!pick_box_halo(g)) return fail(TQ_ERR_UNSUPPORTED, "stem conv: no tile shape");
         g.step_w = g.wbox; g.step_h = g.hbox;
+    } else if (pool == 2) {
+        Wp = (Wo - 1) / 2 + 1;
+        g.pool = 2;
+        g.pool_q = Wp < 15 ? Wp : 15;
+        g.wbox = 32; g.hbox = Ho < 4 ? Ho : 4; g.nbox = 1;
+        g.step_w = 2 * g.pool_q; g.step_h = g.hbox; g.off_w = -1; g.off_h = 0;
+        g.tiles_w = (Wp + g.pool_q - 1) / g.pool_q; g.tiles_h = (Ho + g.hbox - 1) / g.hbox; g.tiles_n = N;
+        g.m_tiles = g.tiles_w * g.tiles_h * g.tiles_n;
     } else {
         Hp = (Ho + 2 - 3) / 2 + 1; Wp = (Wo + 2 - 3) / 2 + 1;
         long best = -1;
@@ -1744,6 +1787,11 @@
         cuuint32_t box[4] = {32, (cuuint32_t)g.wbox, (cuuint32_t)g.hbox, (cuuint32_t)g.nbox};
         cuuint32_t one[4] = {1, 1, 1, 1};
         if ((rc = encode_map(enc, &tmC, CU_TENSOR_MAP_DATA_TYPE_FLOAT32, 4, out, 4, odims, box, one, "stem output")) != TQ_OK) return rc;
+    } else if (pool == 2) {
+        cuuint64_t odims[4] = {(cuuint64_t)Cout, (cuuint64_t)Wp, (cuuint64_t)Ho, (cuuint64_t)N};
+        cuuint32_t box[4] = {32, (cuuint32_t)g.pool_q, (cuuint32_t)g.hbox, 1};
+        cuuint32_t one[4] = {1, 1, 1, 1};
+        if ((rc = encode_map(enc, &tmC, CU_TENSOR_MAP_DATA_TYPE_FLOAT32, 4, out, 4, odims, box, one, "stem row maxima")) != TQ_OK) return rc;
     } else {
         cuuint64_t odims[4] = {(cuuint64_t)Cout, (cuuint64_t)Wp, (cuuint64_t)Hp, (cuuint64_t)N};
         cuuint32_t box[4] = {32, (cuuint32_t)g.pool_q, (cuuint32_t)g.pool_p, 1};
@@ -1785,6 +1833,19 @@
                      mean3, std3);
 }
 
+extern "C" int tq_stem_conv7x7s2_rowmax(const void *x, int x_dtype, void *x2_scratch, const void *w2, float *out,
+                                        int N, int H, int W, int Cout, void *stream)
+{
+    return stem_impl(x, x_dtype, x2_scratch, w2, out, nullptr, nullptr, nullptr, 0, 2, 1.0f, 1, 0, N, H, W, Cout, stream);
+}
+
+extern "C" int tq_stem_conv7x7s2_u8_rowmax(const void *x_u8, const float *mean3, const float *std3, void *x2_scratch,
+                                           const void *w2, float *out, int N, int H, int W, int Cout, void *stream)
+{
+    return stem_impl(x_u8, STEM_U8, x2_scratch, w2, out, nullptr, nullptr, nullptr, 0, 2, 1.0f, 1, 0, N, H, W, Cout, stream,
+                     mean3, std3);
+}
+
 extern "C" int tq_stem_conv7x7s2(const float *x, void *x2_scratch, const void *w2, float *out,
                                  int N, int H, int W, int Cout, void *stream)
 {
diff --git a/term_quantization_b200/csrc/tq_pool.cu b/term_quantization_b200/csrc/tq_pool.cu
--- a/term_quantization_b200/csrc/tq_pool.cu
+++ b/term_quantization_b200/csrc/tq_pool.cu
@@ -72,16 +72,24 @@
     }
 }
 
-constexpr int PT_PR = 4, PT_PC = 7, PT_CB = 64, PT_IH = 2 * PT_PR + 1, PT_IW = 2 * PT_PC + 1;
-constexpr int PT_STAGE_BYTES = PT_IH * PT_IW * PT_CB * 4;
+constexpr int PT_PR = 4, PT_CB = 64, PT_IH = 2 * PT_PR + 1;
 constexpr int PT_STAGES = 3;
-constexpr int PT_THREADS = PT_PR * PT_PC * (PT_CB / 4);
-
+constexpr int PT_THREADS = PT_PR * 7 * (PT_CB / 4);
+template <int KW> struct PoolTile {
+    static constexpr int SW = KW == 3 ? 2 : 1, PAD = KW / 2;
+    static constexpr int PC = KW == 3 ? 7 : 14;
+    static constexpr int IW = SW * (PC - 1) + KW;
+    static constexpr int STAGE_BYTES = PT_IH * IW * PT_CB * 4;
+};
+
+template <int KW>
 __global__ void __launch_bounds__(PT_THREADS, 2)
 bn_relu_maxpool3x3s2_tiled_kernel(const __grid_constant__ CUtensorMap tmIn, const float *__restrict__ bn_a,
                                   const float *__restrict__ bn_b, float *__restrict__ out,
                                   __half *__restrict__ codes, PoolParams p)
 {
+    using T = PoolTile<KW>;
+    constexpr int PT_PC = T::PC, PT_IW = T::IW, PT_STAGE_BYTES = T::STAGE_BYTES;
     extern __shared__ __align__(128) uint8_t pool_smem[];
     uint8_t *base = reinterpret_cast<uint8_t *>((reinterpret_cast<uintptr_t>(pool_smem) + 127) & ~uintptr_t(127));
     __half *lut = reinterpret_cast<__half *>(base + PT_STAGES * PT_STAGE_BYTES);
@@ -100,7 +108,7 @@
     }
     __syncthreads();
     const Quant nq = make_quant(p.write_codes ? p.next_sf : 1.0f, (float)((1u << p.next_bits) - 1u));
-    const int cblocks = p.C / PT_CB, tiles_w = (p.Wo + PT_PC - 1) / PT_PC, tiles_h = (p.Ho + PT_PR - 1) / PT_PR;
+    const int cblocks = (p.C + PT_CB - 1) / PT_CB, tiles_w = (p.Wo + PT_PC - 1) / PT_PC, tiles_h = (p.Ho + PT_PR - 1) / PT_PR;
     const int64_t total = (int64_t)p.N * tiles_h * tiles_w * cblocks;
     const int C4 = p.C >> 2;
     constexpr int c4n = PT_CB / 4;
@@ -112,7 +120,7 @@
         asm volatile("mbarrier.arrive.expect_tx.shared::cta.b64 _, [%0], %1;" ::"r"(bar), "r"((uint32_t)PT_STAGE_BYTES) : "memory");
         asm volatile(
             "cp.async.bulk.tensor.4d.shared::cluster.global.mbarrier::complete_tx::bytes [%0], [%1, {%3, %4, %5, %6}], [%2];"
-            ::"r"(s32(base + stage * PT_STAGE_BYTES)), "l"(&tmIn), "r"(bar), "r"(cb * PT_CB), "r"(tw * PT_PC * 2 - 1),
+            ::"r"(s32(base + stage * PT_STAGE_BYTES)), "l"(&tmIn), "r"(bar), "r"(cb * PT_CB), "r"(tw * PT_PC * T::SW - T::PAD),
               "r"(th * PT_PR * 2 - 1), "r"(n) : "memory");
     };
     int stage = 0;
@@ -139,13 +147,13 @@
         const int cb = (int)(t % cblocks);
         const int64_t r = t / cblocks;
         const int tw = (int)(r % tiles_w), th = (int)((r / tiles_w) % tiles_h), n = (int)(r / ((int64_t)tiles_w * tiles_h));
-        const int h0 = th * PT_PR * 2 - 1, w0 = tw * PT_PC * 2 - 1;
+        const int h0 = th * PT_PR * 2 - 1, w0 = tw * PT_PC * T::SW - T::PAD;
         const float4 *tile = reinterpret_cast<const float4 *>(base + stage * PT_STAGE_BYTES);
         for (int o = threadIdx.x; o < PT_PR * PT_PC * c4n; o += blockDim.x) {
             const int c4 = o % c4n, pw = (o / c4n) % PT_PC, ph = o / (c4n * PT_PC);
             const int ho = th * PT_PR + ph, wo = tw * PT_PC + pw;
-            if (ho >= p.Ho || wo >= p.Wo) continue;
             const int cg = cb * c4n + c4;
+            if (ho >= p.Ho || wo >= p.Wo || cg >= C4) continue;
             const float4 a = __ldg(reinterpret_cast<const float4 *>(bn_a) + cg);
             const float4 b = __ldg(reinterpret_cast<const float4 *>(bn_b) + cg);
             const float ninf = -INFINITY;
@@ -155,10 +163,10 @@
                 const int h = h0 + 2 * ph + dy;
                 if (h < 0 || h >= p.H) continue;
 #pragma unroll
-                for (int dx = 0; dx < 3; ++dx) {
-                    const int w = w0 + 2 * pw + dx;
+                for (int dx = 0; dx < KW; ++dx) {
+                    const int w = w0 + T::SW * pw + dx;
                     if (w < 0 || w >= p.W) continue;
-                    const float4 v = tile[((2 * ph + dy) * PT_IW + 2 * pw + dx) * c4n + c4];
+                    const float4 v = tile[((2 * ph + dy) * PT_IW + T::SW * pw + dx) * c4n + c4];
                     m.x = fmaxf(m.x, __fmaf_rn(v.x, a.x, b.x));
                     m.y = fmaxf(m.y, __fmaf_rn(v.y, a.y, b.y));
                     m.z = fmaxf(m.z, __fmaf_rn(v.z, a.z, b.z));
@@ -189,18 +197,19 @@
 
 using namespace tq;
 
-extern "C" int tq_bn_relu_maxpool_encode(const float *x, const float *bn_a, const float *bn_b, float *out,
-                                         void *out_codes, int N, int H, int W, int C, int relu,
-                                         float next_sf, int next_bits, int next_terms, void *stream)
+namespace {
+
+int pool_params(PoolParams &p, const float *x, const float *bn_a, const float *bn_b, float *out, void *out_codes, int N,
+                int H, int W, int C, int Wo, int relu, float next_sf, int next_bits, int next_terms)
 {
     if (!x || !bn_a || !bn_b || !out) return fail(TQ_ERR_INVALID, "NULL pointer");
     if (N < 1 || H < 1 || W < 1 || C < 4 || C % 4) return fail(TQ_ERR_INVALID, "bad shape (C must be a multiple of 4)");
     if ((((uintptr_t)x | (uintptr_t)bn_a | (uintptr_t)bn_b | (uintptr_t)out | (uintptr_t)out_codes) & 15u) != 0)
         return fail(TQ_ERR_INVALID, "pointers must be 16-byte aligned");
-    PoolParams p{};
+    p = PoolParams{};
     p.N = N; p.H = H; p.W = W; p.C = C;
     p.Ho = (H + 2 - 3) / 2 + 1;
-    p.Wo = (W + 2 - 3) / 2 + 1;
+    p.Wo = Wo;
     p.relu = relu ? 1 : 0;
     p.write_codes = out_codes ? 1 : 0;
     p.next_sf = out_codes ? next_sf : 1.0f;
@@ -211,35 +220,54 @@
         if (next_bits < 1 || next_bits > 11 || next_terms < 0) return fail(TQ_ERR_UNSUPPORTED, "fused encode supports 1..11 bits");
     }
     p.next_fastdiv = (p.next_sf >= 9.313225746154785e-10f && p.next_sf <= 1073741824.0f) ? 1 : 0;
+    return TQ_OK;
+}
+
+template <int KW>
+int launch_tiled(EncodeTiledFn enc, const float *x, const float *bn_a, const float *bn_b, float *out, void *out_codes,
+                 const PoolParams &p, void *stream)
+{
+    using T = PoolTile<KW>;
+    const int N = p.N, H = p.H, W = p.W, C = p.C;
+    CUtensorMap tm;
+    cuuint64_t dims[4] = {(cuuint64_t)C, (cuuint64_t)W, (cuuint64_t)H, (cuuint64_t)N};
+    cuuint64_t strides[3] = {(cuuint64_t)C * 4, (cuuint64_t)W * C * 4, (cuuint64_t)H * W * C * 4};
+    cuuint32_t box[4] = {(cuuint32_t)PT_CB, (cuuint32_t)T::IW, (cuuint32_t)PT_IH, 1};
+    cuuint32_t one[4] = {1, 1, 1, 1};
+    CUresult r = enc(&tm, CU_TENSOR_MAP_DATA_TYPE_FLOAT32, 4, const_cast<float *>(x), dims, strides, box, one,
+                     CU_TENSOR_MAP_INTERLEAVE_NONE, CU_TENSOR_MAP_SWIZZLE_NONE, CU_TENSOR_MAP_L2_PROMOTION_L2_256B,
+                     CU_TENSOR_MAP_FLOAT_OOB_FILL_NONE);
+    if (r != CUDA_SUCCESS) return fail(TQ_ERR_CUDA, "cuTensorMapEncodeTiled(pool input) failed: %d", (int)r);
+    const size_t smem_t = PT_STAGES * (size_t)T::STAGE_BYTES + (((size_t)(2u << p.next_bits) * 2 + 15) & ~(size_t)15) + 64 + 128;
+    static bool attr_done[64] = {false};
+    int dev = 0;
+    cudaGetDevice(&dev);
+    if (dev >= 0 && dev < 64 && !attr_done[dev]) {
+        if (cudaFuncSetAttribute(bn_relu_maxpool3x3s2_tiled_kernel<KW>, cudaFuncAttributeMaxDynamicSharedMemorySize, 112 * 1024) != cudaSuccess)
+            return check_launch("cudaFuncSetAttribute(bn_relu_maxpool3x3s2_tiled_kernel)");
+        attr_done[dev] = true;
+    }
+    const int64_t tiles = (int64_t)N * ((p.Ho + PT_PR - 1) / PT_PR) * ((p.Wo + T::PC - 1) / T::PC) * ((C + PT_CB - 1) / PT_CB);
+    const int64_t capt = (int64_t)num_sms() * 2;
+    bn_relu_maxpool3x3s2_tiled_kernel<KW><<<(int)(tiles < capt ? tiles : capt), PT_THREADS, smem_t, (cudaStream_t)stream>>>(
+        tm, bn_a, bn_b, out, (__half *)out_codes, p);
+    count_launch();
+    return check_launch("bn_relu_maxpool3x3s2_tiled_kernel");
+}
+
+}
+
+extern "C" int tq_bn_relu_maxpool_encode(const float *x, const float *bn_a, const float *bn_b, float *out,
+                                         void *out_codes, int N, int H, int W, int C, int relu,
+                                         float next_sf, int next_bits, int next_terms, void *stream)
+{
+    PoolParams p;
+    int rc = pool_params(p, x, bn_a, bn_b, out, out_codes, N, H, W, C, (W + 2 - 3) / 2 + 1, relu, next_sf, next_bits, next_terms);
+    if (rc != TQ_OK) return rc;
     static const int tiled_env = getenv("TQ_POOL_TILED") ? atoi(getenv("TQ_POOL_TILED")) : 1;
-    if (tiled_env && C % PT_CB == 0 && p.Ho >= PT_PR && p.Wo >= PT_PC) {
+    if (tiled_env && C % PT_CB == 0 && p.Ho >= PT_PR && p.Wo >= PoolTile<3>::PC) {
         EncodeTiledFn enc = encode_tiled();
-        if (enc) {
-            CUtensorMap tm;
-            cuuint64_t dims[4] = {(cuuint64_t)C, (cuuint64_t)W, (cuuint64_t)H, (cuuint64_t)N};
-            cuuint64_t strides[3] = {(cuuint64_t)C * 4, (cuuint64_t)W * C * 4, (cuuint64_t)H * W * C * 4};
-            cuuint32_t box[4] = {(cuuint32_t)PT_CB, (cuuint32_t)PT_IW, (cuuint32_t)PT_IH, 1};
-            cuuint32_t one[4] = {1, 1, 1, 1};
-            CUresult r = enc(&tm, CU_TENSOR_MAP_DATA_TYPE_FLOAT32, 4, const_cast<float *>(x), dims, strides, box, one,
-                             CU_TENSOR_MAP_INTERLEAVE_NONE, CU_TENSOR_MAP_SWIZZLE_NONE, CU_TENSOR_MAP_L2_PROMOTION_L2_256B,
-                             CU_TENSOR_MAP_FLOAT_OOB_FILL_NONE);
-            if (r != CUDA_SUCCESS) return fail(TQ_ERR_CUDA, "cuTensorMapEncodeTiled(pool input) failed: %d", (int)r);
-            const size_t smem_t = PT_STAGES * (size_t)PT_STAGE_BYTES + (((size_t)(2u << p.next_bits) * 2 + 15) & ~(size_t)15) + 64 + 128;
-            static bool attr_done[64] = {false};
-            int dev = 0;
-            cudaGetDevice(&dev);
-            if (dev >= 0 && dev < 64 && !attr_done[dev]) {
-                if (cudaFuncSetAttribute(bn_relu_maxpool3x3s2_tiled_kernel, cudaFuncAttributeMaxDynamicSharedMemorySize, 112 * 1024) != cudaSuccess)
-                    return check_launch("cudaFuncSetAttribute(bn_relu_maxpool3x3s2_tiled_kernel)");
-                attr_done[dev] = true;
-            }
-            const int64_t tiles = (int64_t)N * ((p.Ho + PT_PR - 1) / PT_PR) * ((p.Wo + PT_PC - 1) / PT_PC) * (C / PT_CB);
-            const int64_t capt = (int64_t)num_sms() * 2;
-            bn_relu_maxpool3x3s2_tiled_kernel<<<(int)(tiles < capt ? tiles : capt), PT_THREADS, smem_t, (cudaStream_t)stream>>>(
-                tm, bn_a, bn_b, out, (__half *)out_codes, p);
-            count_launch();
-            return check_launch("bn_relu_maxpool3x3s2_tiled_kernel");
-        }
+        if (enc) return launch_tiled<3>(enc, x, bn_a, bn_b, out, out_codes, p, stream);
     }
     const int64_t total = (int64_t)N * p.Ho * p.Wo * (C / 4);
     int64_t blocks = (total + 255) / 256;
@@ -250,6 +278,18 @@
         x, bn_a, bn_b, out, (__half *)out_codes, p);
     count_launch();
     return check_launch("bn_relu_maxpool3x3s2_kernel");
+}
+
+extern "C" int tq_bn_relu_maxpool_encode_rowmax(const float *x, const float *bn_a, const float *bn_b, float *out,
+                                                void *out_codes, int N, int H, int W, int C, int relu,
+                                                float next_sf, int next_bits, int next_terms, void *stream)
+{
+    PoolParams p;
+    int rc = pool_params(p, x, bn_a, bn_b, out, out_codes, N, H, W, C, W, relu, next_sf, next_bits, next_terms);
+    if (rc != TQ_OK) return rc;
+    EncodeTiledFn enc = encode_tiled();
+    if (!enc) return fail(TQ_ERR_CUDA, "cuTensorMapEncodeTiled is not available from this driver");
+    return launch_tiled<1>(enc, x, bn_a, bn_b, out, out_codes, p, stream);
 }
 
 
diff --git a/term_quantization_b200/fused.py b/term_quantization_b200/fused.py
--- a/term_quantization_b200/fused.py
+++ b/term_quantization_b200/fused.py
@@ -81,9 +81,7 @@
         if (stem != "cudnn" and self.fuse_stem and tuple(c1.weight.shape[1:]) == (3, 7, 7) and c1.stride == (2, 2)
                 and c1.padding == (3, 3) and c1.dilation == (1, 1) and c1.groups == 1 and c1.bias is None
                 and c1.out_channels <= 64):
-            self.stem_w = conv_codes.pack_stem_weight(c1.weight)
-            if stem == "tcgen05_pool":
-                self.stem_w_pool, self.stem_bn_pool = conv_codes.stem_pool_operands(c1.weight, self.stem_bn)
+            self.stem_w, self.stem_bn_pool = conv_codes.stem_pool_operands(c1.weight, self.stem_bn)
         self._stem_scratch = None
 
     @staticmethod
@@ -121,8 +119,8 @@
         if u8_norm is not None:
             q0 = self.blocks[0][0].quant
             y, self._stem_scratch = conv_codes.stem_conv7x7s2_u8(x, u8_norm[0], u8_norm[1], self.stem_w, self._stem_scratch,
-                                                                 cout=m.conv1.out_channels)
-            cur, c0 = conv_codes.bn_relu_maxpool_encode(y, self.stem_bn, relu=True, next_quant=q0)
+                                                                 cout=m.conv1.out_channels, rowmax=True)
+            cur, c0 = conv_codes.bn_relu_maxpool_encode(y, self.stem_bn_pool, relu=True, next_quant=q0, rowmax=True)
             codes = {q0: c0}
         elif self.fuse_stem:
             x = x.contiguous(memory_format=torch.channels_last)
@@ -131,12 +129,12 @@
                     and (x.shape[2] // 2) * (x.shape[3] // 2) >= 128:
                 if self.stem_mode == "tcgen05_pool":
                     cur, c0, self._stem_scratch = conv_codes.stem_conv_pool(
-                        x.permute(0, 2, 3, 1), self.stem_w_pool, self.stem_bn_pool, relu=True, next_quant=q0,
+                        x.permute(0, 2, 3, 1), self.stem_w, self.stem_bn_pool, relu=True, next_quant=q0,
                         scratch=self._stem_scratch)
                 else:
-                    y, self._stem_scratch = conv_codes.stem_conv7x7s2(x.permute(0, 2, 3, 1), self.stem_w,
-                                                                      self._stem_scratch, cout=m.conv1.out_channels)
-                    cur, c0 = conv_codes.bn_relu_maxpool_encode(y, self.stem_bn, relu=True, next_quant=q0)
+                    y, self._stem_scratch = conv_codes.stem_conv7x7s2(x.permute(0, 2, 3, 1), self.stem_w, self._stem_scratch,
+                                                                      cout=m.conv1.out_channels, rowmax=True)
+                    cur, c0 = conv_codes.bn_relu_maxpool_encode(y, self.stem_bn_pool, relu=True, next_quant=q0, rowmax=True)
             else:
                 y = m.conv1(x.float()).permute(0, 2, 3, 1)
                 cur, c0 = conv_codes.bn_relu_maxpool_encode(y, self.stem_bn, relu=True, next_quant=q0)
```

New measurement: 152,500 (median of 6 runs). 1.04x the previous value.
